# AechPro/rlgym-ppo

Measured on NVIDIA B200. Metric: learner_timesteps_per_sec, higher is better.
Workload: dtype bf16

## Files before the change

include/rlppo.h:

```cpp
#ifndef RLPPO_H_
#define RLPPO_H_

#include <stddef.h>
#include <stdint.h>

#ifdef __cplusplus
extern "C" {
#endif

#define RLPPO_OK 0
#define RLPPO_ERR_ARG (-1)
#define RLPPO_ERR_CUDA (-2)
#define RLPPO_ERR_DEVICE (-3)
#define RLPPO_ERR_WORKSPACE (-4)

int rlppo_version(void);
const char* rlppo_last_error(void);
int rlppo_device_check(void);

size_t rlppo_gae_workspace_bytes(int64_t n);
int rlppo_gae_f32(const float* rew, const float* done, const void* trunc, int trunc_is_f64,
                  const float* values, int64_t n, double gamma, double lambda, const float* ret_std,
                  float* adv, float* vtarget, float* ret, double* ret_head64, int64_t n_head,
                  const double* carry_in, void* ws, size_t ws_bytes, void* stream);
// ... 41 lines not shown
                         uint16_t* wt, int64_t wt_ld, int in_pad, void* stream);

int rlppo_linear_fwd(const uint16_t* x, int64_t ldx, const uint16_t* w, int64_t ldw, const float* bias,
                     uint16_t* y, int64_t ldy, int64_t M, int N, int K, int relu, void* stream);
int rlppo_linear_dgrad(const uint16_t* dy, int64_t lddy, const uint16_t* wt, int64_t ldwt,
                       const uint16_t* hprev, int64_t ldh, uint16_t* dx, int64_t lddx, int64_t M, int N,
                       int K, void* stream);
int rlppo_linear_dgrad_db(const uint16_t* dy, int64_t lddy, const uint16_t* wt, int64_t ldwt,
                          const uint16_t* hprev, int64_t ldh, uint16_t* dx, int64_t lddx, float* db_below,
                          int64_t M, int N, int K, void* stream);
int rlppo_linear_wgrad(const uint16_t* dy, int64_t lddy, const uint16_t* x, int64_t ldx, float* dw,
                       int64_t lddw, float* db, int64_t M, int N, int K, void* stream);

typedef struct rlppo_wgrad_item {
    const uint16_t* dy;
    int64_t lddy;
    const uint16_t* x;
    int64_t ldx;
    float* dw;
    int64_t lddw;
    int64_t M;
    int32_t N, K;
    float* db;
} rlppo_wgrad_item;
int rlppo_wgrad_multi(const rlppo_wgrad_item* h_items, int n_items, void* stream);

int rlppo_policy_head_sample(const uint16_t* h, int64_t ldh, const uint16_t* w, int64_t ldw,
                             const float* bias, int64_t M, int n_actions, int K, const float* u_inject,
                             uint64_t seed, uint64_t offset, int deterministic, float* actions_out,
                             int64_t* actions_i64_out, float* logp_out, float* probs_out, void* stream);

int rlppo_policy_head_train(const uint16_t* h, int64_t ldh, const uint16_t* w, int64_t ldw,
                            const float* bias, int64_t M, int n_actions, int K, const float* actions,
                            const float* old_logp, const float* adv, float inv_batch, float clip,
                            float ent_coef, uint16_t* dz, int64_t lddz, float* logp_out, float* metrics,
                            void* stream);

int rlppo_value_head(const uint16_t* h, int64_t ldh, const float* w, const float* bias, int64_t M, int K,
                     float* values_out, const float* targets, float inv_batch, uint16_t* dh, int64_t lddh,
                     float* dw, float* db, float* metrics, void* stream);

typedef struct rlppo_split {
    int32_t a_parts;
    int32_t b_parts;
    int32_t order;
    int32_t out_parts;
    int64_t a_pstride;
    int64_t b_pstride;
    int64_t out_pstride;
} rlppo_split;
int rlppo_rows_split_bf16(const float* src, int64_t src_ld, int64_t n_rows, int width, const float* mean,
                          const float* std, float clip, uint16_t* dst, int64_t dst_ld, int parts, int64_t pstride,
                          void* stream);
int rlppo_weight_split_bf16(const float* w, int out_f, int in_f, uint16_t* wq, int64_t wq_ld, int q_parts,
                            int64_t q_pstride, int out_rows, uint16_t* wt, int64_t wt_ld, int t_parts,
                            int64_t t_pstride, int in_rows, void* stream);
int rlppo_linear_fwd_split(const uint16_t* x, int64_t ldx, const uint16_t* w, int64_t ldw, const float* bias,
                           int bias_n, uint16_t* y, int64_t ldy, int64_t M, int N, int K, int relu,
                           const rlppo_split* sp, void* stream);
int rlppo_linear_dgrad_split(const uint16_t* dy, int64_t lddy, const uint16_t* wt, int64_t ldwt,
                             const uint16_t* hprev, int64_t ldh, uint16_t* dx, int64_t lddx, float* db_below,
                             int64_t M, int N, int K, const rlppo_split* sp, void* stream);
int rlppo_linear_wgrad_split(const uint16_t* dy, int64_t lddy, const uint16_t* x, int64_t ldx, float* dw,
                             int64_t lddw, float* db, int64_t M, int N, int K, const rlppo_split* sp, void* stream);
int rlppo_policy_head_sample_split(const uint16_t* h, int64_t ldh, const uint16_t* w, int64_t ldw,
                                   const float* bias, int64_t M, int n_actions, int K, const float* u_inject,
                                   uint64_t seed, uint64_t offset, int deterministic, float* actions_out,
                                   int64_t* actions_i64_out, float* logp_out, float* probs_out,
                                   const rlppo_split* sp, void* stream);
int rlppo_policy_head_train_split(const uint16_t* h, int64_t ldh, const uint16_t* w, int64_t ldw,
                                  const float* bias, int64_t M, int n_actions, int K, const float* actions,
                                  const float* old_logp, const float* adv, float inv_batch, float clip,
                                  float ent_coef, uint16_t* dz, int64_t lddz, float* logp_out, float* metrics,
                                  const rlppo_split* sp, void* stream);
int rlppo_value_head_split(const uint16_t* h, int64_t ldh, const float* w, const float* bias, int64_t M, int K,
                           float* values_out, const float* targets, float inv_batch, uint16_t* dh, int64_t lddh,
                           float* dw, float* db, float* metrics, int h_parts, int64_t h_pstride, int dh_parts,
                           int64_t dh_pstride, void* stream);

int rlppo_head_multi_discrete_train(const uint16_t* z, int64_t ldz, int z_parts, int64_t z_pstride, int64_t M,
                                    const float* actions, int64_t ld_act, const float* old_logp, const float* adv,
                                    float inv_batch, float clip, float ent_coef, uint16_t* dz, int64_t lddz,
                                    int dz_parts, int64_t dz_pstride, int dz_cols, float* logp_out, float* metrics,
                                    void* stream);
int rlppo_head_multi_discrete_sample(const uint16_t* z, int64_t ldz, int z_parts, int64_t z_pstride, int64_t M,
                                     const float* u_inject, uint64_t seed, uint64_t offset, int deterministic,
                                     float* actions_out, int64_t ld_aout, float* logp_out, void* stream);
int rlppo_head_continuous_train(const uint16_t* z, int64_t ldz, int z_parts, int64_t z_pstride, int64_t M, int n_act,
                                float var_min, float var_max, const float* actions, int64_t ld_act,
                                const float* old_logp, const float* adv, float inv_batch, float clip, float ent_coef,
                                uint16_t* dz, int64_t lddz, int dz_parts, int64_t dz_pstride, int dz_cols,
                                float* logp_out, float* metrics, void* stream);
int rlppo_head_continuous_sample(const uint16_t* z, int64_t ldz, int z_parts, int64_t z_pstride, int64_t M, int n_act,
                                 float var_min, float var_max, const float* n_inject, uint64_t seed, uint64_t offset,
                                 int deterministic, float* actions_out, int64_t ld_aout, float* logp_out, void* stream);

int rlppo_policy_head_backward(const uint16_t* h, int64_t ldh, const uint16_t* w, int64_t ldw, const float* bias,
                               int64_t M, int n_actions, int K, const float* actions, const float* d_logp,
                               const float* d_ent, const float* d_probs, uint16_t* dz, int64_t lddz, void* stream);
int rlppo_policy_head_backward_split(const uint16_t* h, int64_t ldh, const uint16_t* w, int64_t ldw, const float* bias,
                                     int64_t M, int n_actions, int K, const float* actions, const float* d_logp,
                                     const float* d_ent, const float* d_probs, uint16_t* dz, int64_t lddz,
                                     const rlppo_split* sp, void* stream);
int rlppo_head_multi_discrete_backward(const uint16_t* z, int64_t ldz, int z_parts, int64_t z_pstride, int64_t M,
                                       const float* actions, int64_t ld_act, const float* d_logp, const float* d_ent,
                                       uint16_t* dz, int64_t lddz, int dz_parts, int64_t dz_pstride, int dz_cols,
                                       void* stream);
int rlppo_head_continuous_backward(const uint16_t* z, int64_t ldz, int z_parts, int64_t z_pstride, int64_t M, int n_act,
                                   float var_min, float var_max, const float* actions, int64_t ld_act,
                                   const float* d_logp, const float* d_ent, const float* d_mean, const float* d_std,
                                   uint16_t* dz, int64_t lddz, int dz_parts, int64_t dz_pstride, int dz_cols,
                                   void* stream);
int rlppo_value_head_backward(const uint16_t* h, int64_t ldh, const float* w, int64_t M, int K,
                              const float* d_values, uint16_t* dh, int64_t lddh, float* dw, float* db, void* stream);
int rlppo_value_head_backward_split(const uint16_t* h, int64_t ldh, const float* w, int64_t M, int K,
                                    const float* d_values, uint16_t* dh, int64_t lddh, float* dw, float* db,
                                    int h_parts, int64_t h_pstride, int dh_parts, int64_t dh_pstride, void* stream);

typedef struct rlppo_fused_net {
    int n_hidden;
    int in_dim;
    int64_t in_ld;
    int hidden[4];
    const uint16_t* wq[5];
    int64_t wq_ld[5];
    const uint16_t* wt[5];
    int64_t wt_ld[5];
    const float* bias[5];
    float* gbias[5];
    uint16_t* h[4];
    int64_t h_ld[4];
    uint16_t* dh[4];
    int64_t dh_ld[4];
    uint16_t* dz;
    int64_t dz_ld;
} rlppo_fused_net;

int rlppo_policy_train_fused(const rlppo_fused_net* net, const uint16_t* x, int64_t M, int n_actions,
                             const float* actions, const float* old_logp, const float* adv, float inv_batch,
                             float clip, float ent_coef, float* logp_out, float* metrics, void* stream);
int rlppo_policy_infer_fused(const rlppo_fused_net* net, const uint16_t* x, int64_t M, int n_actions,
                             const float* u_inject, uint64_t seed, uint64_t offset, const uint64_t* d_offset,
                             int deterministic, float* actions_out, int64_t* actions_i64_out, float* logp_out,
                             void* stream);
int rlppo_u64_add(uint64_t* d_counter, uint64_t inc, void* stream);
int rlppo_value_train_fused(const rlppo_fused_net* net, const uint16_t* x, int64_t M, const float* w_head,
                            const float* targets, float inv_batch, float* gw_head, float* values_out,
                            float* metrics, void* stream);
int rlppo_policy_value_train_fused(const rlppo_fused_net* policy_net, const rlppo_fused_net* value_net,
                                   const uint16_t* x, int64_t M, int n_actions, const float* actions,
                                   const float* old_logp, const float* adv, float inv_batch, float clip, float ent_coef,
                                   float* logp_out, const float* w_head, const float* targets, float* gw_head,
                                   float* values_out, float* metrics, void* stream);
int rlppo_value_infer_fused(const rlppo_fused_net* net, const uint16_t* x, int64_t M, const float* w_head,
                            float* values_out, void* stream);

int rlppo_grad_sqnorm(const float* grads, const int64_t* h_seg_off, int n_seg, float* sqnorm, void* stream);
typedef struct rlppo_bf16_view {
    int64_t offset;
    int32_t out_f, in_f;
    uint16_t* wq;
    int64_t wq_ld;
    uint16_t* wt;
    int64_t wt_ld;
} rlppo_bf16_view;
int rlppo_clip_adam(float* params, const float* grads, float* m, float* v, const int64_t* h_seg_off,
                    int n_seg, const float* sqnorm, const float* lr, int64_t* step_count, double max_norm,
                    double beta1, double beta2, double eps, const rlppo_bf16_view* h_views, int n_views,
                    void* stream);
size_t rlppo_norm_clip_adam_workspace_bytes(void);
int rlppo_norm_clip_adam(float* params, const float* grads, float* m, float* v, const int64_t* h_seg_off,
                         int n_seg, float* sqnorm_out, const float* lr, int64_t* step_count, double max_norm,
                         double beta1, double beta2, double eps, const rlppo_bf16_view* h_views, int n_views,
                         void* ws, size_t ws_bytes, void* stream);
size_t rlppo_peer_flag_bytes(void);
int rlppo_norm_clip_adam_peers(float* params, const float* const* h_peer_grads, void* const* h_peer_flags, int rank,
                               int world, float* gsum, float* m, float* v, const int64_t* h_seg_off, int n_seg,
                               float* sqnorm_out, const float* lr, int64_t* step_count, double max_norm, double beta1,
                               double beta2, double eps, const rlppo_bf16_view* h_views, int n_views, void* ws,
                               size_t ws_bytes, void* stream);
int rlppo_norm_clip_adam_peers2(float* params, const float* const* h_peer_grads, void* const* h_peer_flags,
                                const float* const* h_peer_red, int rank, int world, float* m, float* v,
                                const int64_t* h_seg_off, int n_seg, float* sqnorm_out, const float* lr,
                                int64_t* step_count, double max_norm, double beta1, double beta2, double eps,
                                const rlppo_bf16_view* h_views, int n_views, void* ws, size_t ws_bytes, void* stream);
int rlppo_sqdiff(const float* a, const float* b, const int64_t* h_seg_off, int n_seg, float* out,
                 void* stream);

#ifdef __cplusplus
}
#endif
#endif
```

rlgym_ppo_b200/_lib.py:

```python
import ctypes
import os

import torch

_HERE = os.path.dirname(os.path.abspath(__file__))
LIB_PATH = os.environ.get("RLPPO_LIB_PATH") or os.path.join(_HERE, "librlppo_b200.so")

if not os.path.exists(LIB_PATH):
    raise ImportError(
        f"{LIB_PATH} is missing: build it with `python -m rlgym_ppo_b200.build` (nvcc, sm_100a). "
        "rlgym_ppo_b200 has no CPU or PyTorch fallback for its kernels."
    )

_lib = ctypes.CDLL(LIB_PATH)

_P = ctypes.c_void_p
_I = ctypes.c_int
_L = ctypes.c_int64
_D = ctypes.c_double
_F = ctypes.c_float
_U64 = ctypes.c_uint64
_SZ = ctypes.c_size_t

_SIGS = {
    "rlppo_version": ([], _I),
    "rlppo_last_error": ([], ctypes.c_char_p),
    "rlppo_device_check": ([], _I),
    "rlppo_gae_workspace_bytes": ([_L], _SZ),
    "rlppo_gae_f32": ([_P, _P, _P, _I, _P, _L, _D, _D, _P, _P, _P, _P, _P, _L, _P, _P, _SZ, _P], _I),
    "rlppo_gae_chunk_summary": ([_P, _P, _P, _I, _P, _L, _D, _D, _P, _P, _P, _SZ, _P], _I),
    "rlppo_gae_compose_carry": ([_P, _I, _I, _P, _P], _I),
    "rlppo_welford_update": ([_P, _P, _P, _P, _I, _L, _I, _P, _P, _P], _I),
    "rlppo_ring_append": ([_P, _L, _P, _L, _L, _L, _P, _I, _L, _L, _I, _P], _I),
    "rlppo_ring_append_fields": ([_P, _I, _L, _L, _L, _P], _I),
    "rlppo_ring_append_fields_dev": ([_P, _I, _L, _P, _L, _P], _I),
    "rlppo_gather_batch": ([_P, _P, _P, _P, _P, _L, _P, _L, _I, _L, _L, _P, _P, _L, _P, _P, _P, _P, _P, _P, _P], _I),
    "rlppo_host_permutation": ([_P, _P, _L, _P], _I),
    "rlppo_rows_to_bf16": ([_P, _L, _L, _I, _P, _L, _P], _I),
    "rlppo_rows_standardize_to_bf16": ([_P, _L, _L, _I, _P, _P, _F, _P, _L, _P, _L, _P], _I),
    "rlppo_weight_to_bf16": ([_P, _I, _I, _P, _L, _I, _P, _L, _I, _P], _I),
    "rlppo_linear_fwd": ([_P, _L, _P, _L, _P, _P, _L, _L, _I, _I, _I, _P], _I),
    "rlppo_linear_dgrad": ([_P, _L, _P, _L, _P, _L, _P, _L, _L, _I, _I, _P], _I),
    "rlppo_linear_dgrad_db": ([_P, _L, _P, _L, _P, _L, _P, _L, _P, _L, _I, _I, _P], _I),
    "rlppo_linear_wgrad": ([_P, _L, _P, _L, _P, _L, _P, _L, _I, _I, _P], _I),
    "rlppo_wgrad_multi": ([_P, _I, _P], _I),
    "rlppo_policy_head_sample": ([_P, _L, _P, _L, _P, _L, _I, _I, _P, _U64, _U64, _I, _P, _P, _P, _P, _P], _I),
    "rlppo_policy_head_train": ([_P, _L, _P, _L, _P, _L, _I, _I, _P, _P, _P, _F, _F, _F, _P, _L, _P, _P, _P], _I),
    "rlppo_value_head": ([_P, _L, _P, _P, _L, _I, _P, _P, _F, _P, _L, _P, _P, _P, _P], _I),
    "rlppo_rows_split_bf16": ([_P, _L, _L, _I, _P, _P, _F, _P, _L, _I, _L, _P], _I),
    "rlppo_weight_split_bf16": ([_P, _I, _I, _P, _L, _I, _L, _I, _P, _L, _I, _L, _I, _P], _I),
    "rlppo_linear_fwd_split": ([_P, _L, _P, _L, _P, _I, _P, _L, _L, _I, _I, _I, _P, _P], _I),
    "rlppo_linear_dgrad_split": ([_P, _L, _P, _L, _P, _L, _P, _L, _P, _L, _I, _I, _P, _P], _I),
    "rlppo_linear_wgrad_split": ([_P, _L, _P, _L, _P, _L, _P, _L, _I, _I, _P, _P], _I),
    "rlppo_policy_head_sample_split": ([_P, _L, _P, _L, _P, _L, _I, _I, _P, _U64, _U64, _I, _P, _P, _P, _P, _P, _P], _I),
    "rlppo_policy_head_train_split": ([_P, _L, _P, _L, _P, _L, _I, _I, _P, _P, _P, _F, _F, _F, _P, _L, _P, _P, _P, _P], _I),
    "rlppo_value_head_split": ([_P, _L, _P, _P, _L, _I, _P, _P, _F, _P, _L, _P, _P, _P, _I, _L, _I, _L, _P], _I),
    "rlppo_head_multi_discrete_train": ([_P, _L, _I, _L, _L, _P, _L, _P, _P, _F, _F, _F, _P, _L, _I, _L, _I, _P, _P, _P], _I),
    "rlppo_head_multi_discrete_sample": ([_P, _L, _I, _L, _L, _P, _U64, _U64, _I, _P, _L, _P, _P], _I),
    "rlppo_head_continuous_train": ([_P, _L, _I, _L, _L, _I, _F, _F, _P, _L, _P, _P, _F, _F, _F, _P, _L, _I, _L, _I, _P,
                                     _P, _P], _I),
    "rlppo_head_continuous_sample": ([_P, _L, _I, _L, _L, _I, _F, _F, _P, _U64, _U64, _I, _P, _L, _P, _P], _I),
    "rlppo_policy_head_backward": ([_P, _L, _P, _L, _P, _L, _I, _I, _P, _P, _P, _P, _P, _L, _P], _I),
    "rlppo_policy_head_backward_split": ([_P, _L, _P, _L, _P, _L, _I, _I, _P, _P, _P, _P, _P, _L, _P, _P], _I),
    "rlppo_head_multi_discrete_backward": ([_P, _L, _I, _L, _L, _P, _L, _P, _P, _P, _L, _I, _L, _I, _P], _I),
    "rlppo_head_continuous_backward": ([_P, _L, _I, _L, _L, _I, _F, _F, _P, _L, _P, _P, _P, _P, _P, _L, _I, _L, _I, _P],
                                       _I),
    "rlppo_value_head_backward": ([_P, _L, _P, _L, _I, _P, _P, _L, _P, _P, _P], _I),
    "rlppo_value_head_backward_split": ([_P, _L, _P, _L, _I, _P, _P, _L, _P, _P, _I, _L, _I, _L, _P], _I),
    "rlppo_policy_train_fused": ([_P, _P, _L, _I, _P, _P, _P, _F, _F, _F, _P, _P, _P], _I),
    "rlppo_policy_infer_fused": ([_P, _P, _L, _I, _P, _U64, _U64, _P, _I, _P, _P, _P, _P], _I),
    "rlppo_u64_add": ([_P, _U64, _P], _I),
    "rlppo_value_train_fused": ([_P, _P, _L, _P, _P, _F, _P, _P, _P, _P], _I),
    "rlppo_policy_value_train_fused": ([_P, _P, _P, _L, _I, _P, _P, _P, _F, _F, _F, _P, _P, _P, _P, _P, _P, _P], _I),
    "rlppo_value_infer_fused": ([_P, _P, _L, _P, _P, _P], _I),
    "rlppo_grad_sqnorm": ([_P, _P, _I, _P, _P], _I),
    "rlppo_clip_adam": ([_P, _P, _P, _P, _P, _I, _P, _P, _P, _D, _D, _D, _D, _P, _I, _P], _I),
    "rlppo_norm_clip_adam_workspace_bytes": ([], ctypes.c_size_t),
    "rlppo_norm_clip_adam": ([_P, _P, _P, _P, _P, _I, _P, _P, _P, _D, _D, _D, _D, _P, _I, _P, ctypes.c_size_t, _P], _I),
    "rlppo_peer_flag_bytes": ([], ctypes.c_size_t),
    "rlppo_norm_clip_adam_peers": ([_P, _P, _P, _I, _I, _P, _P, _P, _P, _I, _P, _P, _P, _D, _D, _D, _D, _P, _I, _P,
                                    ctypes.c_size_t, _P], _I),
    "rlppo_norm_clip_adam_peers2": ([_P, _P, _P, _P, _I, _I, _P, _P, _P, _I, _P, _P, _P, _D, _D, _D, _D, _P, _I, _P,
                                     ctypes.c_size_t, _P], _I),
    "rlppo_sqdiff": ([_P, _P, _P, _I, _P, _P], _I),
}

EXPORTED = tuple(_SIGS)


class AppendField(ctypes.Structure):
    _fields_ = [("ring", _P), ("ring_ld", _L), ("ring_bf16", _P), ("bf16_ld", _L), ("src", _P), ("src_ld", _L),
                ("src_is_f64", ctypes.c_int32), ("width", ctypes.c_int32)]


class Split(ctypes.Structure):
    _fields_ = [("a_parts", ctypes.c_int32), ("b_parts", ctypes.c_int32), ("order", ctypes.c_int32),
                ("out_parts", ctypes.c_int32), ("a_pstride", _L), ("b_pstride", _L), ("out_pstride", _L)]


class WgradItem(ctypes.Structure):
    _fields_ = [("dy", _P), ("lddy", _L), ("x", _P), ("ldx", _L), ("dw", _P), ("lddw", _L), ("M", _L),
                ("N", ctypes.c_int32), ("K", ctypes.c_int32), ("db", _P)]


class Bf16View(ctypes.Structure):
    _fields_ = [("offset", _L), ("out_f", ctypes.c_int32), ("in_f", ctypes.c_int32), ("wq", _P), ("wq_ld", _L),
                ("wt", _P), ("wt_ld", _L)]


class FusedNet(ctypes.Structure):
    _fields_ = [("n_hidden", _I), ("in_dim", _I), ("in_ld", _L), ("hidden", _I * 4),
                ("wq", _P * 5), ("wq_ld", _L * 5), ("wt", _P * 5), ("wt_ld", _L * 5),
                ("bias", _P * 5), ("gbias", _P * 5), ("h", _P * 4), ("h_ld", _L * 4),
                ("dh", _P * 4), ("dh_ld", _L * 4), ("dz", _P), ("dz_ld", _L)]

for _name, (_args, _res) in _SIGS.items():
    _fn = getattr(_lib, _name)
    _fn.argtypes = _args
    _fn.restype = _res


class RlppoError(RuntimeError):
    pass


def last_error():
    return _lib.rlppo_last_error().decode("utf-8", "replace")


def _check(rc, name):
    if rc != 0:
        raise RlppoError(f"{name} failed ({rc}): {last_error()}")


def ptr(t):
    if t is None:
        return None
    return ctypes.c_void_p(t.data_ptr())


def stream_ptr():
    return ctypes.c_void_p(torch.cuda.current_stream().cuda_stream)


CALLS = 0
_TIMING = None


def call(name, *args, work=None):
    global CALLS
    CALLS += 1
    if _TIMING is None:
        _check(getattr(_lib, name)(*args), name)
        return
    e0, e1 = torch.cuda.Event(enable_timing=True), torch.cuda.Event(enable_timing=True)
    torch.cuda._sleep(300_000)
    e0.record()
    rc = getattr(_lib, name)(*args)
    e1.record()
    _check(rc, name)
    _TIMING.append((name, work, e0, e1))


def timing_begin():
    global _TIMING
    _TIMING = []


def timing_end():
    global _TIMING
    rec, _TIMING = _TIMING, None
    torch.cuda.synchronize()
    out = {}
    for name, work, e0, e1 in rec:
        d = out.setdefault(name, {"calls": 0, "ms": 0.0, "flop": 0.0, "byte": 0.0})
        d["calls"] += 1
        d["ms"] += e0.elapsed_time(e1)
        if work is not None:
            for i in range(0, len(work), 2):
                d[work[i]] = d.get(work[i], 0.0) + float(work[i + 1])
    return out


def require_device():
    if not torch.cuda.is_available():
        raise RlppoError("rlgym_ppo_b200 needs a CUDA device (B200, sm_100); there is no CPU fallback")
    _check(_lib.rlppo_device_check(), "rlppo_device_check")


def version():
    return _lib.rlppo_version()


def gae_workspace_bytes(n):
    return int(_lib.rlppo_gae_workspace_bytes(int(n)))


def host_permutation_raw(key, pos, n, out=None):
    import numpy as np

    key = np.ascontiguousarray(key, dtype=np.uint32).copy()
    p = np.asarray([pos], dtype=np.int32)
    if out is None:
        out = np.empty(int(n), dtype=np.int64)
    rc = _lib.rlppo_host_permutation(key.ctypes.data_as(_P), p.ctypes.data_as(_P), int(n), out.ctypes.data_as(_P))
    _check(rc, "rlppo_host_permutation")
    return out, key, int(p[0])


def host_permutation(rng, n):
    import numpy as np

    st = rng.get_state()
    key = np.ascontiguousarray(st[1], dtype=np.uint32).copy()
    pos = np.asarray([st[2]], dtype=np.int32)
    out = np.empty(int(n), dtype=np.int64)
    rc = _lib.rlppo_host_permutation(key.ctypes.data_as(_P), pos.ctypes.data_as(_P), int(n), out.ctypes.data_as(_P))
    _check(rc, "rlppo_host_permutation")
    rng.set_state((st[0], key, int(pos[0]), st[3], st[4]))
    return out
```

rlgym_ppo_b200/csrc/common.cuh:

```cuda
#pragma once
#include <cuda_runtime.h>
#include <cuda_bf16.h>
#include <stdint.h>
#include <stdio.h>
#include <string.h>

#include "../../include/rlppo.h"

namespace rlppo {

void set_error(const char* fmt, ...);
int check_device();
int num_sms();

#define RLPPO_CHECK_ARG(cond, ...)                 \
    do {                                           \
        if (!(cond)) {                             \
            rlppo::set_error(__VA_ARGS__);         \
            return RLPPO_ERR_ARG;                  \
        }                                          \
    } while (0)

#define RLPPO_CUDA(expr)                                                                      \
    do {                                                                                      \
        cudaError_t _e = (expr);                                                              \
        if (_e != cudaSuccess) {                                                              \
            rlppo::set_error("%s failed: %s (%s:%d)", #expr, cudaGetErrorString(_e), __FILE__, \
                             __LINE__);                                                       \
            return RLPPO_ERR_CUDA;                                                            \
        }                                                                                     \
    } while (0)

#define RLPPO_REQUIRE_DEVICE()                    \
    do {                                          \
        int _d = rlppo::check_device();           \
        if (_d != RLPPO_OK) return _d;            \
    } while (0)

#define RLPPO_LAUNCH_CHECK() RLPPO_CUDA(cudaGetLastError())

__device__ __forceinline__ void pdl_wait() { asm volatile("griddepcontrol.wait;" ::: "memory"); }
__device__ __forceinline__ void pdl_trigger() { asm volatile("griddepcontrol.launch_dependents;" ::: "memory"); }
int pdl_mode();

template <class... KArgs, class... Args>
cudaError_t launch_pdl_cluster(void (*kernel)(KArgs...), dim3 grid, dim3 block, size_t smem, cudaStream_t s, int cluster_x,
                               Args&&... args) {
    cudaLaunchConfig_t cfg = {};
    cfg.gridDim = grid;
    cfg.blockDim = block;
    cfg.dynamicSmemBytes = smem;
    cfg.stream = s;
    cudaLaunchAttribute attr[2];
    int n = 0;
    if (pdl_mode()) {
        attr[n].id = cudaLaunchAttributeProgrammaticStreamSerialization;
        attr[n].val.programmaticStreamSerializationAllowed = 1;
        ++n;
    }
    if (cluster_x > 1) {
        attr[n].id = cudaLaunchAttributeClusterDimension;
        attr[n].val.clusterDim.x = (unsigned)cluster_x;
        attr[n].val.clusterDim.y = 1;
        attr[n].val.clusterDim.z = 1;
        ++n;
    }
    cfg.attrs = attr;
    cfg.numAttrs = n;
    return cudaLaunchKernelEx(&cfg, kernel, static_cast<KArgs>(args)...);
}
template <class... KArgs, class... Args>
cudaError_t launch_pdl(void (*kernel)(KArgs...), dim3 grid, dim3 block, size_t smem, cudaStream_t s, Args&&... args) {
    return launch_pdl_cluster(kernel, grid, block, smem, s, 1, static_cast<Args&&>(args)...);
}

__device__ __forceinline__ int ld_acquire_s32(const int* p) {
    int v;
    asm volatile("ld.acquire.gpu.global.s32 %0, [%1];" : "=r"(v) : "l"(p) : "memory");
    return v;
}
__device__ __forceinline__ void st_release_s32(int* p, int v) {
    asm volatile("st.release.gpu.global.s32 [%0], %1;" ::"l"(p), "r"(v) : "memory");
}

__device__ __forceinline__ float warp_sum(float v) {
#pragma unroll
    for (int o = 16; o > 0; o >>= 1) v += __shfl_xor_sync(0xffffffffu, v, o);
    return v;
}
__device__ __forceinline__ double warp_sum(double v) {
#pragma unroll
    for (int o = 16; o > 0; o >>= 1) v += __shfl_xor_sync(0xffffffffu, v, o);
    return v;
}

__device__ __forceinline__ uint16_t f32_to_bf16_bits(float f) {
    return __bfloat16_as_ushort(__float2bfloat16_rn(f));
}
__device__ __forceinline__ float bf16_bits_to_f32(uint16_t b) { return __uint_as_float(((uint32_t)b) << 16); }
__device__ __forceinline__ uint32_t pack_bf16x2(float lo, float hi) {
    return (uint32_t)f32_to_bf16_bits(lo) | ((uint32_t)f32_to_bf16_bits(hi) << 16);
}

}
```

rlgym_ppo_b200/csrc/mlp_fused.cu:

```cuda
#include <type_traits>
#include <math.h>
#include <stdlib.h>

#include "tc_common.cuh"

namespace {

using namespace rlppo;
using namespace rlppo::tc;

constexpr int MAXL = 4;
constexpr int TILE_M = 128;
constexpr int KBLK = 64;
constexpr uint32_t KB_BYTES = TILE_M * KBLK * 2;
constexpr uint32_t ACT_BYTES = 4 * KB_BYTES;
constexpr uint32_t WST_BYTES = 256 * KBLK * 2;
constexpr uint32_t MN_CHUNK = 64 * KBLK * 2;
constexpr int MAX_NWST = 6;
constexpr int kThreads = 352;
constexpr int kEpiThreads = 256;
constexpr int MAXPH = 2 * MAXL + 1;

constexpr uint32_t OFF_ACT = 0;
constexpr uint32_t OFF_XST = ACT_BYTES;
constexpr uint32_t BIAS_FLOATS = (MAXL + 1) * 256;
constexpr uint32_t MISC_BIAS = 0;
constexpr uint32_t MISC_ROWX = MISC_BIAS + 2 * BIAS_FLOATS * 4;
constexpr uint32_t ROWX_FLOATS = 1280;
constexpr uint32_t MISC_DB = MISC_ROWX + ROWX_FLOATS * 4;
constexpr uint32_t MISC_MASK = MISC_DB + 256 * 4;
constexpr uint32_t MISC_BARS = MISC_MASK + MAXL * 4 * kEpiThreads * 4;
constexpr uint32_t MISC_BYTES = MISC_BARS + 384;
constexpr uint32_t SMEM_LIMIT = 232448;
static_assert(ACT_BYTES + 2 * KB_BYTES + MISC_BYTES + 1024 + 3 * WST_BYTES <= SMEM_LIMIT,
              "an observation of <= 128 columns must leave room for a 3-stage weight ring (2 stages starve the MMA)");

enum { PH_FWD = 0, PH_FWD_VALUE = 1, PH_HEAD = 2, PH_DGRAD = 3, PH_VALUE_BWD = 4 };
constexpr uint8_t NO_STORE = 0xFF;

struct alignas(16) PhaseDesc {
    uint8_t kind;
    uint8_t layer;
    uint8_t n_kb;
    uint8_t wmap;
    uint16_t N;
    uint8_t out;
    uint8_t smem;
    uint8_t wait_kb;
    uint8_t rel_kb;
    uint8_t b_mn;
};

constexpr int MAXNET = 2;

struct alignas(64) Maps {
    CUtensorMap x;
    CUtensorMap w[MAXNET][MAXPH];
    CUtensorMap out[MAXNET][MAXPH];
};

struct NetP {
    int policy;
    int n_ph, L;
    int H[MAXL];
    PhaseDesc ph[MAXPH];
    int tail_rel_kb;
    const float* bias[MAXL + 1];
    float* gbias[MAXL + 1];
    int n_actions, out_kb;
    const float *actions, *old_logp, *adv;
    float inv_batch, clip, ent_coef;
    const float* u_inject;
    uint64_t seed, offset;
    const unsigned long long* d_offset;
    int deterministic;
    float* actions_out;
    int64_t* actions_i64_out;
    float* logp_out;
    const float* w_head;
    const float* targets;
    float* gw_head;
    float* values_out;
    float* metrics;
};

struct Params {
    int64_t M;
    int num_tiles, in_kb, nwst;
    int pair;
    int n_units;
    uint32_t wst_bytes;
    int n_nets;
    NetP net[MAXNET];
    unsigned int* sched;
    uint32_t* mask_scratch;
    int dbg_nostore;
    int dbg;
    unsigned long long* trace;
};

__device__ __forceinline__ void tma_store_2d(const CUtensorMap* m, const void* smem_src, int c0, int c1) {
    asm volatile("cp.async.bulk.tensor.2d.global.shared::cta.bulk_group [%0, {%2, %3}], [%1];" ::"l"(
                     reinterpret_cast<uint64_t>(m)),
                 "r"(smem_u32(smem_src)), "r"(c0), "r"(c1)
                 : "memory");
}
__device__ __forceinline__ void bulk_commit() { asm volatile("cp.async.bulk.commit_group;" ::: "memory"); }
__device__ __forceinline__ void bulk_wait_read_all() { asm volatile("cp.async.bulk.wait_group.read 0;" ::: "memory"); }
__device__ __forceinline__ void epi_bar_sync() { asm volatile("bar.sync 1, 256;" ::: "memory"); }

__device__ __forceinline__ uint4 philox4x32_10(uint4 c, uint2 k) {
#pragma unroll
    for (int i = 0; i < 10; ++i) {
        const uint32_t hi0 = __umulhi(0xD2511F53u, c.x), lo0 = 0xD2511F53u * c.x;
        const uint32_t hi1 = __umulhi(0xCD9E8D57u, c.z), lo1 = 0xCD9E8D57u * c.z;
        c = make_uint4(hi1 ^ c.y ^ k.x, lo1, hi0 ^ c.w ^ k.y, lo0);
        k.x += 0x9E3779B9u;
        k.y += 0xBB67AE85u;
    }
    return c;
}

__device__ __forceinline__ float warp_colsum32(float (&v)[32], int lane) {
#pragma unroll
    for (int w = 16; w >= 1; w >>= 1) {
        const bool up = (lane & w) != 0;
#pragma unroll
        for (int i = 0; i < w; ++i) {
            const float send = up ? v[i] : v[i + w];
            const float keep = up ? v[i + w] : v[i];
            v[i] = keep + __shfl_xor_sync(0xffffffffu, send, w);
        }
    }
    return v[0];
}

__device__ __forceinline__ float warp_colsum16(float (&v)[16], int lane) {
#pragma unroll
    for (int w = 8; w >= 1; w >>= 1) {
        const bool up = (lane & w) != 0;
#pragma unroll
        for (int i = 0; i < w; ++i) {
            const float send = up ? v[i] : v[i + w];
            const float keep = up ? v[i + w] : v[i];
            v[i] = keep + __shfl_xor_sync(0xffffffffu, send, w);
        }
    }
    return v[0] + __shfl_xor_sync(0xffffffffu, v[0], 16);
}

__device__ __forceinline__ float bf16_round(float x) { return bf16_bits_to_f32(f32_to_bf16_bits(x)); }
__device__ __forceinline__ uint32_t cvt_bf16x2(float lo, float hi) {
    uint32_t r;
    asm("cvt.rn.bf16x2.f32 %0, %1, %2;" : "=r"(r) : "f"(hi), "f"(lo));
    return r;
}

__device__ __forceinline__ uint32_t cvt_relu_bf16x2(float lo, float hi) {
    uint32_t r;
    asm("cvt.rn.relu.bf16x2.f32 %0, %1, %2;" : "=r"(r) : "f"(hi), "f"(lo));
    return r;
}

__device__ __forceinline__ void pack32(const float (&v)[32], uint32_t (&w)[16]) {
#pragma unroll
    for (int i = 0; i < 16; ++i) w[i] = cvt_bf16x2(v[2 * i], v[2 * i + 1]);
}
__device__ __forceinline__ void pack32_relu(const float (&v)[32], uint32_t (&w)[16]) {
#pragma unroll
    for (int i = 0; i < 16; ++i) w[i] = cvt_relu_bf16x2(v[2 * i], v[2 * i + 1]);
}
__device__ __forceinline__ uint32_t prmt_b32(uint32_t a, uint32_t b, uint32_t sel) {
    uint32_t r;
    asm("prmt.b32 %0, %1, %2, %3;" : "=r"(r) : "r"(a), "r"(b), "r"(sel));
    return r;
}
__device__ __forceinline__ uint32_t relu_mask32(const uint32_t (&w)[16]) {
    uint32_t m[4] = {0u, 0u, 0u, 0u};
#pragma unroll
    for (int q = 0; q < 8; ++q) {
        uint32_t f0, f1;
        asm("set.gt.u32.bf16x2 %0, %1, %2;" : "=r"(f0) : "r"(w[2 * q]), "r"(0u));
        asm("set.gt.u32.bf16x2 %0, %1, %2;" : "=r"(f1) : "r"(w[2 * q + 1]), "r"(0u));
        m[q & 3] |= prmt_b32(f0, f1, 0x7531u) & (0x80808080u >> q);
    }
    return (m[0] | m[1]) | (m[2] | m[3]);
}
__device__ __forceinline__ void apply_relu_mask32(uint32_t (&w)[16], uint32_t bits) {
#pragma unroll
    for (int q = 0; q < 8; ++q) {
        const uint32_t t = bits << q;
        w[2 * q] &= prmt_b32(t, 0u, 0x9988u);
        w[2 * q + 1] &= prmt_b32(t, 0u, 0xBBAAu);
    }
}
__device__ __forceinline__ constexpr int relu_mask_bit(int i) { return 8 * (i & 3) + 7 - (i >> 2); }
__device__ __forceinline__ void sts_chunk_sw128(uint8_t* buf, int row, int chunk32, const uint32_t (&w)[16]) {
    uint8_t* kb = buf + (chunk32 >> 1) * KB_BYTES + row * 128;
    const int base16 = (chunk32 & 1) * 4;
#pragma unroll
    for (int t = 0; t < 4; ++t)
        *reinterpret_cast<uint4*>(kb + (((base16 + t) ^ (row & 7)) << 4)) = make_uint4(w[4 * t], w[4 * t + 1], w[4 * t + 2], w[4 * t + 3]);
}
__device__ __forceinline__ void sts_chunk16_sw128(uint8_t* buf, int row, int chunk16, const uint32_t (&w)[8]) {
    uint8_t* kb = buf + (chunk16 >> 2) * KB_BYTES + row * 128;
    const int base16 = (chunk16 & 3) * 2;
#pragma unroll
    for (int t = 0; t < 2; ++t)
        *reinterpret_cast<uint4*>(kb + (((base16 + t) ^ (row & 7)) << 4)) = make_uint4(w[4 * t], w[4 * t + 1], w[4 * t + 2], w[4 * t + 3]);
}

#define RLPPO_TRACE(role, idx)                                                                  \
    do {                                                                                        \
        const int _i = (idx);                                                                   \
        if (p.trace != nullptr && blockIdx.x == 0 && _i < 512) p.trace[(role) * 512 + _i] = clock64(); \
    } while (0)

#ifdef RLPPO_FINE_TRACE
#define EPI_T()                                                                                  \
    do {                                                                                         \
        if (p.trace != nullptr && blockIdx.x == 0 && it == 0 && warp == 2 && lane == 0 && tr5 < 500) p.trace[5 * 512 + tr5++] = clock64(); \
    } while (0)
#else
#define EPI_T() do { } while (0)
#endif

struct EpiCtx {
    uint8_t* act;
    float* s_bias;
    float* s_rowx;
    uint32_t* s_mask;
    uint64_t* a_ready;
    uint64_t* a_mma;
    uint32_t rank;
    int lane, quarter, half, row_in_tile;
};

template <bool PAIR>
__device__ __forceinline__ void release_kb(const EpiCtx& e, int kb) {
    tc_fence_before();
    fence_proxy_async();
    __syncwarp();
    if (e.lane == 0) {
        mbar_arrive(e.a_ready + kb);
        if (PAIR) mbar_arrive_cta(e.a_mma + kb, 0);
    }
}

template <bool TRAIN, bool PAIR>
__global__ void __launch_bounds__(kThreads, 1) fused_mlp_kernel(const __grid_constant__ Maps maps, const Params p) {
    extern __shared__ uint8_t smem_raw[];
    uint8_t* smem = smem_raw + ((1024u - (smem_u32(smem_raw) & 1023u)) & 1023u);
    uint8_t* act = smem + OFF_ACT;
    uint8_t* xst = smem + OFF_XST;
    uint8_t* wring = xst + p.in_kb * KB_BYTES;
    uint8_t* misc = wring + p.nwst * p.wst_bytes;
    const uint32_t rank = PAIR ? cluster_ctarank() : 0u;
    const bool leader = rank == 0;
    float* s_bias = reinterpret_cast<float*>(misc + MISC_BIAS);
    float* s_rowx = reinterpret_cast<float*>(misc + MISC_ROWX);
    float* s_db = reinterpret_cast<float*>(misc + MISC_DB);
// ... 455 lines not shown
            mbar_init(&a_done[s], 16);
            mbar_init(&acc_full[s], 1);
            mbar_init(&st_done[s], 1);
        }
        fence_barrier_init();
    }
    if (warp == 1) tmem_alloc_pair(tmem_slot, 512);
    pdl_wait();
    pdl_trigger();
    if (p.trace != nullptr && threadIdx.x == 0) {
        unsigned long long t;
        asm volatile("mov.u64 %0, %%globaltimer;" : "=l"(t));
        p.trace[2048 + 2 * blockIdx.x] = t;
    }
    for (int i = threadIdx.x; i < p.n_nets * (int)BIAS_FLOATS; i += kThreads) {
        const int ni = i >= (int)BIAS_FLOATS ? 1 : 0;
        const NetP& np = p.net[ni];
        const int j = i - ni * (int)BIAS_FLOATS;
        const int l = j >> 8, c = j & 255;
        float b = 0.f;
        if (l < np.L) {
            if (c < np.H[l]) b = __ldg(np.bias[l] + c);
        } else if (l == MAXL) {
            if (np.policy) b = c < np.n_actions ? (np.bias[MAXL] != nullptr ? __ldg(np.bias[MAXL] + c) : 0.f) : -1e30f;
            else if (c < np.H[np.L - 1]) b = __ldg(np.w_head + c);
        }
        s_bias[i] = b;
    }
    for (int i = threadIdx.x; i < 256; i += kThreads) s_db[i] = 0.f;
    for (int i = threadIdx.x; i < p.n_nets * MAXPH; i += kThreads)
        const_cast<PhaseDesc*>(s_ph)[i] = p.net[i / MAXPH].ph[i % MAXPH];
    tc_fence_before();
    __syncthreads();
    cluster_sync_all();
    tc_fence_after();
    const uint32_t tmem_base = *tmem_slot;

    const int cluster_id = (int)(blockIdx.x >> 1), n_clusters = (int)(gridDim.x >> 1);
    const int total_items = p.n_nets * p.n_units;
    const int nph_net0 = p.net[0].n_ph, nph_net1 = p.net[1].n_ph;
    auto next_item = [&](DuoWalk& w, int s) -> bool {
        const int q = cluster_id + (w.fetches++) * n_clusters;
        if (q >= total_items) {
            DUO_SET(w, alive, s, false);
            return false;
        }
        const int ni = q >= p.n_units ? 1 : 0;
        DUO_SET(w, ni, s, ni);
        DUO_SET(w, tile, s, 2 * (q - ni * p.n_units) + (int)rank);
        DUO_SET(w, ph, s, 0);
        DUO_SET(w, nph, s, ni ? nph_net1 : nph_net0);
        DUO_SET(w, items, s, DUO_SEL(w, items, s) + 1);
        return true;
    };
#define DUO_WALK_BEGIN(w, traced)                                             \
    for (int n = 0;; ++n) {                                                   \
        const int s = n & 1;                                                  \
        if ((traced) && warp == 2 && lane == 0) RLPPO_TRACE(3, 4 * n);        \
        if (!DUO_SEL(w, alive, s)) {                                          \
            if (!DUO_SEL(w, alive, s ^ 1)) break;                             \
            continue;                                                         \
        }                                                                     \
        if (DUO_SEL(w, ph, s) == DUO_SEL(w, nph, s) && !next_item(w, s)) {    \
            if (!DUO_SEL(w, alive, s ^ 1)) break;                             \
            continue;                                                         \
        }                                                                     \
        const int ph = DUO_SEL(w, ph, s);                                     \
        DUO_SET(w, ph, s, ph + 1);                                            \
        const int ni = DUO_SEL(w, ni, s);                                     \
        const int tile_s = DUO_SEL(w, tile, s);                               \
        const int items_s = DUO_SEL(w, items, s);                             \
        const bool last_ph = ph + 1 == DUO_SEL(w, nph, s);                    \
        const NetP& np = p.net[ni];                                           \
        const PhaseDesc d = s_ph[ni * MAXPH + ph];                            \
        (void)d; (void)np; (void)tile_s; (void)items_s; (void)last_ph;
#define DUO_WALK_END }

    if (warp == 0) {
        if (lane == 0) {
            DuoWalk w;
            uint32_t ws = 0, wpar = 0;
            DUO_WALK_BEGIN(w, false)
                if (ph == 0) {
                    mbar_wait(&x_free[s], (uint32_t)(items_s & 1));
                    if (leader) mbar_expect_tx(&x_full[s], 2u * p.in_kb * KB_BYTES);
                    for (int kb = 0; kb < p.in_kb; ++kb)
                        tma_load_2d_leaderbar(&maps.x, &x_full[s], smem + s * ACT_BYTES + kb * KB_BYTES, kb * KBLK, tile_s * TILE_M);
                }
                const int nh = d.N >> 1;
                for (int kb = 0; kb < d.n_kb; ++kb) {
                    mbar_wait(&wempty[ws], wpar ^ 1);
                    if (leader) mbar_expect_tx(&wfull[ws], (uint32_t)d.N * 128u);
                    uint8_t* dst = ring + ws * DUO_STAGE;
                    if (d.b_mn) {
                        for (int c = 0; c < (nh >> 6); ++c)
                            tma_load_2d_leaderbar(&maps.w[ni][d.wmap], &wfull[ws], dst + c * MN_CHUNK, (int)rank * nh + c * 64,
                                                  kb * KBLK);
                    } else {
                        tma_load_2d_leaderbar(&maps.w[ni][d.wmap], &wfull[ws], dst, kb * KBLK, (int)rank * nh);
                    }
                    if (++ws == DUO_NST) {
                        ws = 0;
                        wpar ^= 1;
                    }
                }
            DUO_WALK_END
        }
    } else if (warp == 1) {
        if (lane == 0 && leader) {
            DuoWalk w;
            uint32_t ws = 0, wpar = 0;
            uint32_t epi_cnt[2] = {0u, 0u};
            int tr0 = 0;
            DUO_WALK_BEGIN(w, false)
                RLPPO_TRACE(0, tr0++);
                const uint32_t d_tmem = tmem_base + (uint32_t)s * 256u;
                uint8_t* act = smem + s * ACT_BYTES;
                if (epi_cnt[s] > 0u) mbar_wait(&a_done[s], (epi_cnt[s] - 1u) & 1u);
                if (ph == 0) mbar_wait(&x_full[s], (items_s - 1) & 1);
                tc_fence_after();
                if (d.n_kb > 0) {
                    const uint32_t idesc = umma_idesc_bf16(2 * TILE_M, d.N, 0, d.b_mn);
                    for (int kb = 0; kb < d.n_kb; ++kb) {
                        mbar_wait(&wfull[ws], wpar);
                        tc_fence_after();
                        const uint32_t a_addr = smem_u32(act + kb * KB_BYTES);
                        const uint32_t b_addr = smem_u32(ring + ws * DUO_STAGE);
#pragma unroll
                        for (int k = 0; k < KBLK / 16; ++k) {
                            const uint64_t ad = umma_smem_desc(a_addr + k * 32, 16, 1024);
                            const uint64_t bd = d.b_mn ? umma_smem_desc(b_addr + k * (16 * 128), MN_CHUNK, 1024)
                                                       : umma_smem_desc(b_addr + k * 32, 16, 1024);
                            if (!(p.dbg & 1)) umma_bf16_pair(d_tmem, ad, bd, idesc, (kb | k) != 0 ? 1u : 0u);
                        }
                        umma_commit_pair(&wempty[ws]);
                        if (++ws == DUO_NST) {
                            ws = 0;
                            wpar ^= 1;
                        }
                    }
                    umma_commit_pair(&acc_full[s]);
                } else {
                    mbar_arrive(&acc_full[s]);
                    mbar_arrive_cta(&acc_full[s], 1);
                }
                ++epi_cnt[s];
                RLPPO_TRACE(0, tr0++);
            DUO_WALK_END
        }
    } else if (warp == 10) {
        if (lane == 0) {
            DuoWalk w;
            uint32_t kpar = 0;
            DUO_WALK_BEGIN(w, false)
                uint8_t* act = smem + s * ACT_BYTES;
                for (int kb = 0; kb < d.rel_kb; ++kb) {
                    const int b = 4 * s + kb;
                    mbar_wait(&a_kb[b], (kpar >> b) & 1u);
                    kpar ^= 1u << b;
                    if (d.out != NO_STORE) {
                        if (!p.dbg_nostore) tma_store_2d(&maps.out[ni][d.out], act + kb * KB_BYTES, kb * KBLK, tile_s * TILE_M);
                        bulk_commit();
                    }
                }
                if (d.out != NO_STORE && d.rel_kb > 0) bulk_wait_read_all();
                mbar_arrive(&st_done[s]);
                if (last_ph) mbar_arrive(&x_free[s]);
            DUO_WALK_END
            asm volatile("cp.async.bulk.wait_group 0;" ::: "memory");
        }
    } else {
        EpiCtx e;
        e.s_bias = s_bias;
        e.s_rowx = s_rowx;
        e.a_ready = nullptr;
        e.a_mma = nullptr;
        e.rank = rank;
        e.lane = lane;
        e.quarter = warp & 3;
        e.half = (warp - 2) >> 2;
        e.row_in_tile = e.quarter * 32 + lane;
        float dv_slot0 = 0.f, dv_slot1 = 0.f;
        float m0 = 0.f, m1 = 0.f, m2 = 0.f, m3 = 0.f, mrows = 0.f;
        float vm0 = 0.f, vm1 = 0.f, vrows = 0.f;
        auto db_add = [&](int c, float v) { atomicAdd(&s_db[c * 32 + e.lane], v); };
        uint32_t cnt[2] = {0u, 0u};
        uint32_t pend = 0, scnt = 0;
        uint32_t* mask_g = p.mask_scratch + (size_t)blockIdx.x * (2 * DUO_MAXL * 4 * kEpiThreads) + (threadIdx.x - 64);
        int tr1 = 0;
        DuoWalk w;
        DUO_WALK_BEGIN(w, true)
            uint8_t* act = smem + s * ACT_BYTES;
            e.act = act;
            e.s_mask = nullptr;
            const float* s_bias_n = s_bias + ni * (int)BIAS_FLOATS;
            const int64_t row = (int64_t)tile_s * TILE_M + e.row_in_tile;
            const bool row_ok = row < p.M;
            float dv_keep = s ? dv_slot1 : dv_slot0;
            if (warp == 2 && lane == 0) RLPPO_TRACE(2, tr1);
            uint32_t mpre0 = 0u, mpre1 = 0u, mpre2 = 0u, mpre3 = 0u;
            if (d.kind == PH_DGRAD || d.kind == PH_VALUE_BWD) {
                const uint32_t* mp = mask_g + (s * DUO_MAXL + d.layer) * 4 * kEpiThreads;
                mpre0 = __ldcg(mp);
                mpre1 = __ldcg(mp + kEpiThreads);
                mpre2 = __ldcg(mp + 2 * kEpiThreads);
                mpre3 = __ldcg(mp + 3 * kEpiThreads);
            }
            mbar_wait(&acc_full[s], cnt[s] & 1u);
            ++cnt[s];
            tc_fence_after();
            if (warp == 2 && lane == 0) RLPPO_TRACE(1, tr1++);
            if ((pend >> s) & 1u) {
                mbar_wait(&st_done[s], (scnt >> s) & 1u);
                scnt ^= 1u << s;
                pend &= ~(1u << s);
            }
            const uint32_t trow = tmem_base + ((uint32_t)(e.quarter * 32) << 16) + (uint32_t)s * 256u;
            uint8_t* dst = act;
            const int li = d.layer;
            const int it = 1;
            int tr5 = 0;
            (void)it;
            (void)tr5;
#define RLPPO_RELEASE_KB(j)                                                  \
    do {                                                                      \
        if (((j) & 1) || (j) + 1 >= (int)d.rel_kb) {                          \
            fence_proxy_async();                                              \
            __syncwarp();                                                     \
            if (lane == 0) {                                                  \
                if ((j) & 1) mbar_arrive(&a_kb[4 * s + (j) - 1]);             \
                mbar_arrive(&a_kb[4 * s + (j)]);                              \
            }                                                                 \
        }                                                                     \
    } while (0)
#define RLPPO_MASK_ST(l, kb, v) __stcg(mask_g + ((s * DUO_MAXL + (l)) * 4 + (kb)) * kEpiThreads, (v))
#define RLPPO_MASK_LD(l, kb) ((kb) == 0 ? mpre0 : (kb) == 1 ? mpre1 : (kb) == 2 ? mpre2 : mpre3)
#include "fused_epilogue.inc"
#undef RLPPO_MASK_ST
#undef RLPPO_MASK_LD
#undef RLPPO_RELEASE_KB
            if (s) dv_slot1 = dv_keep;
            else dv_slot0 = dv_keep;
            pend |= 1u << s;
            if (warp == 2 && lane == 0) RLPPO_TRACE(3, 4 * n + 1);
            tc_fence_before();
            __syncwarp();
            if (warp == 2 && lane == 0) RLPPO_TRACE(3, 4 * n + 2);
            if (lane == 0) {
                if (leader) mbar_arrive(&a_done[s]);
                else mbar_arrive_cta(&a_done[s], 0);
            }
            if (warp == 2 && lane == 0) RLPPO_TRACE(1, tr1++);
        DUO_WALK_END
        if (e.half == 0) {
            for (int ni = 0; ni < p.n_nets; ++ni) {
                const NetP& np = p.net[ni];
                if (np.metrics == nullptr) continue;
                if (np.policy) {
                    const float r0 = warp_sum(m0), r1 = warp_sum(m1), r2 = warp_sum(m2), r3 = warp_sum(m3),
                                rr = warp_sum(mrows);
                    if (e.lane == 0 && rr > 0.f) {
                        atomicAdd(np.metrics + 0, r0);
                        atomicAdd(np.metrics + 1, r1);
                        atomicAdd(np.metrics + 2, r2);
                        atomicAdd(np.metrics + 3, r3);
                        atomicAdd(np.metrics + 4, rr);
                    }
                } else {
                    const float r0 = warp_sum(vm0), r1 = warp_sum(vm1), rr = warp_sum(vrows);
                    if (e.lane == 0 && rr > 0.f) {
                        atomicAdd(np.metrics + 5, r0);
                        atomicAdd(np.metrics + 6, rr);
                        if (np.gbias[MAXL] != nullptr) atomicAdd(np.gbias[MAXL], r1);
                    }
                }
            }
        }
    }
#undef DUO_WALK_BEGIN
#undef DUO_WALK_END
#undef DUO_SEL
#undef DUO_SET
    tc_fence_before();
    __syncthreads();
    if (p.trace != nullptr && threadIdx.x == 0) {
        unsigned long long t;
        asm volatile("mov.u64 %0, %%globaltimer;" : "=l"(t));
        p.trace[2048 + 2 * blockIdx.x + 1] = t;
    }
    cluster_sync_all();
    if (warp == 1) {
        tc_fence_after();
        tmem_dealloc_pair(tmem_base, 512);
    }
    for (int ni = 0; ni < p.n_nets; ++ni) {
        const NetP& np = p.net[ni];
        if (np.policy || np.gw_head == nullptr) continue;
        for (int c = threadIdx.x; c < np.H[np.L - 1]; c += kThreads) atomicAdd(np.gw_head + c, s_db[c]);
    }
}

int check_net(const rlppo_fused_net* net) {
    RLPPO_CHECK_ARG(net != nullptr, "null net descriptor");
    RLPPO_CHECK_ARG(net->n_hidden >= 1 && net->n_hidden <= MAXL, "fused path: 1..%d hidden layers", MAXL);
    RLPPO_CHECK_ARG(net->in_dim >= 1 && net->in_dim <= 256 && net->in_ld % 8 == 0 && net->in_ld >= net->in_dim,
                    "fused path: input width <= 256, row stride a multiple of 8");
    for (int l = 0; l < net->n_hidden; ++l)
        RLPPO_CHECK_ARG(net->hidden[l] >= 64 && net->hidden[l] <= 256 && net->hidden[l] % 64 == 0,
                        "fused path: hidden widths must be 64, 128, 192 or 256 (got %d)", net->hidden[l]);
    return RLPPO_OK;
}

template <bool TRAIN>
int build_net(bool POLICY, const rlppo_fused_net* net, int64_t M, int ni, Maps& maps, NetP& p, bool pair) {
    int rc = check_net(net);
    if (rc) return rc;
    const int L = net->n_hidden;
    p.policy = POLICY ? 1 : 0;
    p.L = L;
    for (int l = 0; l < MAXL; ++l) p.H[l] = l < L ? net->hidden[l] : 0;
    for (int l = 0; l < L; ++l) {
        p.bias[l] = net->bias[l];
// ... 197 lines not shown
    }
    return true;
}

int launch_duo(const rlppo_fused_net* const* nets, const bool* is_policy, int n_nets, const uint16_t* x, int64_t M, Params& p,
               cudaStream_t s) {
    Maps maps;
    p.M = M;
    p.num_tiles = (int)((M + TILE_M - 1) / TILE_M);
    p.pair = 1;
    p.n_units = (p.num_tiles + 1) / 2;
    p.n_nets = n_nets;
    p.in_kb = (nets[0]->in_dim + KBLK - 1) / KBLK;
    p.nwst = DUO_NST;
    p.wst_bytes = DUO_STAGE;
    for (int ni = 0; ni < n_nets; ++ni) {
        RLPPO_CHECK_ARG(nets[ni]->in_dim == nets[0]->in_dim && nets[ni]->in_ld == nets[0]->in_ld,
                        "nets of one launch read the same x");
        int rc = build_net<true>(is_policy[ni], nets[ni], M, ni, maps, p.net[ni], true);
        if (rc) return rc;
    }
    int rc = make_tmap_bf16_2d(&maps.x, x, (uint64_t)M, (uint64_t)nets[0]->in_dim, (uint64_t)nets[0]->in_ld, TILE_M);
    if (rc) return rc;
    static bool configured = false;
    if (!configured) {
        RLPPO_CUDA(cudaFuncSetAttribute(fused_duo_kernel, cudaFuncAttributeMaxDynamicSharedMemorySize, (int)SMEM_LIMIT));
        configured = true;
    }
    const int items = p.n_units * n_nets;
    const int pairs = num_sms() / 2;
    const int want = (items + 1) / 2;
    const int grid = 2 * (want < pairs ? want : pairs);
    for (int ni = 0; ni < n_nets; ++ni)
        for (int i = 0; i < p.net[ni].n_ph; ++i)
            RLPPO_CHECK_ARG(p.net[ni].ph[i].rel_kb > 0, "duo kernel: every phase must release at least one k-block");
    p.sched = nullptr;
    {
        static uint32_t* d_mask[16] = {};
        static unsigned int next_area[16] = {};
        int dev = 0;
        RLPPO_CUDA(cudaGetDevice(&dev));
        const size_t area = (size_t)num_sms() * 2 * DUO_MAXL * 4 * kEpiThreads;
        if (d_mask[dev] == nullptr) RLPPO_CUDA(cudaMalloc(&d_mask[dev], 4 * area * sizeof(uint32_t)));
        p.mask_scratch = d_mask[dev] + (next_area[dev]++ % 4) * area;
    }
    p.dbg_nostore = getenv("RLPPO_FUSED_NOSTORE") != nullptr ? 1 : 0;
    p.dbg = getenv("RLPPO_DUO_DBG") != nullptr ? atoi(getenv("RLPPO_DUO_DBG")) : 0;
    static unsigned long long* d_trace = nullptr;
    const bool tracing = getenv("RLPPO_FUSED_TRACE") != nullptr;
    if (tracing) {
        if (d_trace == nullptr) RLPPO_CUDA(cudaMalloc(&d_trace, 3072 * sizeof(unsigned long long)));
        RLPPO_CUDA(cudaMemsetAsync(d_trace, 0, 3072 * sizeof(unsigned long long), s));
        p.trace = d_trace;
    }
    RLPPO_CUDA(launch_pdl_cluster(fused_duo_kernel, dim3(grid), dim3(kThreads), (size_t)DUO_SMEM, s, 2, maps, p));
    if (tracing) {
        static unsigned long long h[3072];
        RLPPO_CUDA(cudaMemcpyAsync(h, d_trace, sizeof(h), cudaMemcpyDeviceToHost, s));
        RLPPO_CUDA(cudaStreamSynchronize(s));
        const unsigned long long t0 = h[0];
        fprintf(stderr, "[duo trace] items=%d (steps alternate slots 0/1)\n", items);
        for (int i = 0; i + 1 < 100 && h[i + 1] != 0; i += 2)
            fprintf(stderr, "  mma  step %d start=%llu issued=+%llu\n", i / 2, h[i] - t0, h[i + 1] - h[i]);
        {
            unsigned long long g0 = ~0ull, g1 = 0;
            for (int b = 0; b < grid; ++b) {
                if (h[2048 + 2 * b] < g0) g0 = h[2048 + 2 * b];
                if (h[2048 + 2 * b + 1] > g1) g1 = h[2048 + 2 * b + 1];
            }
            fprintf(stderr, "  CTA spans (ns from the first start; start..end), kernel body %llu ns:\n", g1 - g0);
            for (int b = 0; b < grid; b += 2)
                fprintf(stderr, "   cluster %d: %llu..%llu%s", b / 2, h[2048 + 2 * b] - g0, h[2048 + 2 * b + 1] - g0, (b / 2) % 4 == 3 ? "\n" : "");
            fprintf(stderr, "\n");
        }
        for (int i = 0; i + 1 < 100 && h[512 + i] != 0; i += 2)
            fprintf(stderr, "  epi  step %d top=%llu arrive=%llu acc_full=%llu dur=%llu body_end=+%llu fences=+%llu arrives=+%llu\n", i / 2,
                    h[1536 + 2 * i] - t0, h[1024 + i] - t0, h[512 + i] - t0, h[512 + i + 1] - h[512 + i],
                    h[1536 + 2 * i + 1] - h[512 + i], h[1536 + 2 * i + 2] - h[1536 + 2 * i + 1], h[512 + i + 1] - h[1536 + 2 * i + 2]);
    }
    return RLPPO_OK;
}

template <bool TRAIN>
int launch_nets(const rlppo_fused_net* const* nets, const bool* is_policy, int n_nets, const uint16_t* x, int64_t M, Params& p,
                cudaStream_t s) {
    RLPPO_CHECK_ARG(n_nets >= 1 && n_nets <= MAXNET && nets[0] != nullptr, "1..%d nets per launch", MAXNET);
    RLPPO_CHECK_ARG(M >= 1 && M < (1ll << 30) - TILE_M, "bad row count");
    for (int ni = 0; ni < n_nets; ++ni) {
        int rc = check_net(nets[ni]);
        if (rc) return rc;
    }
    if (TRAIN && duo_ok(nets, n_nets)) return launch_duo(nets, is_policy, n_nets, x, M, p, s);
    if (TRAIN && pair_ok(nets, n_nets)) return launch_nets_t<TRAIN, TRAIN>(nets, is_policy, n_nets, x, M, p, s);
    return launch_nets_t<TRAIN, false>(nets, is_policy, n_nets, x, M, p, s);
}

void fill_policy_train(NetP& n, int n_actions, const float* actions, const float* old_logp, const float* adv,
                       float inv_batch, float clip, float ent_coef, float* logp_out, float* metrics) {
    n.n_actions = n_actions;
    n.actions = actions; n.old_logp = old_logp; n.adv = adv;
    n.inv_batch = inv_batch; n.clip = clip; n.ent_coef = ent_coef;
    n.logp_out = logp_out; n.metrics = metrics;
}
void fill_value_train(NetP& n, const float* w_head, const float* targets, float inv_batch, float* gw_head,
                      float* values_out, float* metrics) {
    n.w_head = w_head; n.targets = targets; n.inv_batch = inv_batch; n.gw_head = gw_head;
    n.values_out = values_out; n.metrics = metrics;
}

__global__ void u64_add_kernel(unsigned long long* ctr, unsigned long long inc) { *ctr += inc; }

}

extern "C" {

int rlppo_policy_train_fused(const rlppo_fused_net* net, const uint16_t* x, int64_t M, int n_actions,
                             const float* actions, const float* old_logp, const float* adv, float inv_batch, float clip,
                             float ent_coef, float* logp_out, float* metrics, void* stream) {
    RLPPO_REQUIRE_DEVICE();
    RLPPO_CHECK_ARG(x && actions && old_logp && adv, "null pointer");
    RLPPO_CHECK_ARG(n_actions >= 1 && n_actions <= 128, "fused path: n_actions must be in [1,128]");
    Params p{};
    fill_policy_train(p.net[0], n_actions, actions, old_logp, adv, inv_batch, clip, ent_coef, logp_out, metrics);
    const bool pol[1] = {true};
    return launch_nets<true>(&net, pol, 1, x, M, p, static_cast<cudaStream_t>(stream));
}

int rlppo_value_train_fused(const rlppo_fused_net* net, const uint16_t* x, int64_t M, const float* w_head,
                            const float* targets, float inv_batch, float* gw_head, float* values_out, float* metrics,
                            void* stream) {
    RLPPO_REQUIRE_DEVICE();
    RLPPO_CHECK_ARG(x && w_head && targets && gw_head, "null pointer");
    Params p{};
    fill_value_train(p.net[0], w_head, targets, inv_batch, gw_head, values_out, metrics);
    const bool pol[1] = {false};
    return launch_nets<true>(&net, pol, 1, x, M, p, static_cast<cudaStream_t>(stream));
}

int rlppo_policy_value_train_fused(const rlppo_fused_net* policy_net, const rlppo_fused_net* value_net, const uint16_t* x,
                                   int64_t M, int n_actions, const float* actions, const float* old_logp, const float* adv,
                                   float inv_batch, float clip, float ent_coef, float* logp_out, const float* w_head,
                                   const float* targets, float* gw_head, float* values_out, float* metrics, void* stream) {
    RLPPO_REQUIRE_DEVICE();
    RLPPO_CHECK_ARG(policy_net && value_net && x && actions && old_logp && adv && w_head && targets && gw_head, "null pointer");
    RLPPO_CHECK_ARG(n_actions >= 1 && n_actions <= 128, "fused path: n_actions must be in [1,128]");
    Params p{};
    fill_policy_train(p.net[0], n_actions, actions, old_logp, adv, inv_batch, clip, ent_coef, logp_out, metrics);
    fill_value_train(p.net[1], w_head, targets, inv_batch, gw_head, values_out, metrics);
    const rlppo_fused_net* nets[2] = {policy_net, value_net};
    const bool pol[2] = {true, false};
    return launch_nets<true>(nets, pol, 2, x, M, p, static_cast<cudaStream_t>(stream));
}

int rlppo_u64_add(uint64_t* d_counter, uint64_t inc, void* stream) {
    RLPPO_REQUIRE_DEVICE();
    RLPPO_CHECK_ARG(d_counter != nullptr, "null pointer");
    u64_add_kernel<<<1, 1, 0, static_cast<cudaStream_t>(stream)>>>(reinterpret_cast<unsigned long long*>(d_counter), inc);
    RLPPO_LAUNCH_CHECK();
    return RLPPO_OK;
}

int rlppo_policy_infer_fused(const rlppo_fused_net* net, const uint16_t* x, int64_t M, int n_actions,
                             const float* u_inject, uint64_t seed, uint64_t offset, const uint64_t* d_offset,
                             int deterministic, float* actions_out, int64_t* actions_i64_out, float* logp_out,
                             void* stream) {
    RLPPO_REQUIRE_DEVICE();
    RLPPO_CHECK_ARG(x != nullptr, "null pointer");
    RLPPO_CHECK_ARG(n_actions >= 1 && n_actions <= 128, "fused path: n_actions must be in [1,128]");
    Params p{};
    NetP& n = p.net[0];
    n.n_actions = n_actions;
    n.u_inject = u_inject; n.seed = seed; n.offset = offset; n.deterministic = deterministic;
    n.d_offset = reinterpret_cast<const unsigned long long*>(d_offset);
    n.actions_out = actions_out; n.actions_i64_out = actions_i64_out; n.logp_out = logp_out;
    const bool pol[1] = {true};
    return launch_nets<false>(&net, pol, 1, x, M, p, static_cast<cudaStream_t>(stream));
}

int rlppo_value_infer_fused(const rlppo_fused_net* net, const uint16_t* x, int64_t M, const float* w_head,
                            float* values_out, void* stream) {
    RLPPO_REQUIRE_DEVICE();
    RLPPO_CHECK_ARG(x && w_head && values_out, "null pointer");
    Params p{};
    p.net[0].w_head = w_head; p.net[0].values_out = values_out;
    const bool pol[1] = {false};
    return launch_nets<false>(&net, pol, 1, x, M, p, static_cast<cudaStream_t>(stream));
}
}
```

rlgym_ppo_b200/csrc/mlp_tcgen05.cu:

```cuda
#include <mutex>
#include <unordered_map>
#include <math.h>

#include <stdlib.h>

#include "tc_common.cuh"

namespace rlppo {
namespace tc {

typedef CUresult (*EncodeTiledFn)(CUtensorMap*, CUtensorMapDataType, cuuint32_t, void*, const cuuint64_t*,
                                  const cuuint64_t*, const cuuint32_t*, const cuuint32_t*, CUtensorMapInterleave,
                                  CUtensorMapSwizzle, CUtensorMapL2promotion, CUtensorMapFloatOOBfill);

static EncodeTiledFn get_encode_fn() {
    static EncodeTiledFn fn = nullptr;
    if (fn == nullptr) {
        void* p = nullptr;
        cudaDriverEntryPointQueryResult q;
        if (cudaGetDriverEntryPoint("cuTensorMapEncodeTiled", &p, cudaEnableDefault, &q) == cudaSuccess &&
            q == cudaDriverEntryPointSuccess)
            fn = reinterpret_cast<EncodeTiledFn>(p);
    }
    return fn;
}

int make_tmap_bf16_2d(CUtensorMap* out, const void* base, uint64_t rows, uint64_t cols, uint64_t ld,
                      uint32_t box_rows) {
    EncodeTiledFn fn = get_encode_fn();
    if (fn == nullptr) {
        set_error("cuTensorMapEncodeTiled not available from the driver");
        return RLPPO_ERR_CUDA;
    }
    RLPPO_CHECK_ARG((reinterpret_cast<uintptr_t>(base) & 15) == 0, "TMA operand must be 16-byte aligned");
    RLPPO_CHECK_ARG((ld * 2) % 16 == 0 && cols <= ld && cols >= 1 && rows >= 1, "TMA operand: ld must be a multiple of 8");
    RLPPO_CHECK_ARG(box_rows >= 1 && box_rows <= 256, "TMA box rows out of range");
    struct Key {
        const void* base;
        uint64_t rows, cols, ld;
        uint32_t box_rows;
        bool operator==(const Key& o) const {
            return base == o.base && rows == o.rows && cols == o.cols && ld == o.ld && box_rows == o.box_rows;
        }
    };
    struct KeyHash {
        size_t operator()(const Key& k) const {
            uint64_t h = reinterpret_cast<uintptr_t>(k.base) * 0x9E3779B97F4A7C15ull;
            h ^= (k.rows + 0x9E3779B97F4A7C15ull + (h << 6) + (h >> 2));
            h ^= (k.cols * 0xC2B2AE3D27D4EB4Full + (h << 6) + (h >> 2));
            h ^= (k.ld * 0x165667B19E3779F9ull + (h << 6) + (h >> 2));
            return (size_t)(h ^ k.box_rows);
        }
    };
    static std::mutex mu;
    static std::unordered_map<Key, CUtensorMap, KeyHash> cache;
    const Key key{base, rows, cols, ld, box_rows};
    {
        std::lock_guard<std::mutex> lock(mu);
        auto it = cache.find(key);
        if (it != cache.end()) {
            *out = it->second;
            return RLPPO_OK;
        }
    }
    cuuint64_t gdim[2] = {cols, rows};
    cuuint64_t gstride[1] = {ld * 2};
    cuuint32_t box[2] = {64, box_rows};
    cuuint32_t estr[2] = {1, 1};
    CUresult r = fn(out, CU_TENSOR_MAP_DATA_TYPE_BFLOAT16, 2, const_cast<void*>(base), gdim, gstride, box, estr,
                    CU_TENSOR_MAP_INTERLEAVE_NONE, CU_TENSOR_MAP_SWIZZLE_128B, CU_TENSOR_MAP_L2_PROMOTION_L2_256B,
                    CU_TENSOR_MAP_FLOAT_OOB_FILL_NONE);
    if (r != CUDA_SUCCESS) {
        set_error("cuTensorMapEncodeTiled failed with CUresult %d (rows=%llu cols=%llu ld=%llu box_rows=%u)", (int)r,
                  (unsigned long long)rows, (unsigned long long)cols, (unsigned long long)ld, box_rows);
        return RLPPO_ERR_CUDA;
    }
    {
        std::lock_guard<std::mutex> lock(mu);
        if (cache.size() >= 4096) cache.clear();
        cache.emplace(key, *out);
    }
    return RLPPO_OK;
}

}
}

namespace {

using namespace rlppo;
using namespace rlppo::tc;

constexpr int BLOCK_M = 128;
constexpr int BLOCK_K = 64;
constexpr int UMMA_K = 16;
constexpr int kStages = 4;
constexpr int kThreads = 192;
constexpr uint32_t A_BYTES = BLOCK_M * BLOCK_K * 2;

enum { EPI_BIAS_ACT = 0, EPI_RELU_MASK = 1, EPI_HEAD_SAMPLE = 2, EPI_HEAD_TRAIN = 3, EPI_HEAD_BWD = 4 };

constexpr int MAX_SCHED = 6;
struct KSched {
    int n;
    int kpp;
    int a_off[MAX_SCHED];
    int b_off[MAX_SCHED];
};

struct RowGemmParams {
    int64_t M;
    int N, K;
    int num_m_tiles, num_n_tiles, num_k_blocks;
    KSched sched;
    int out_parts;
    int64_t out_pstride;
    int out_cols;
    uint16_t* out;
    int64_t ldo;
    const float* bias;
    int bias_n;
    int relu;
    const uint16_t* mask;
    int64_t ldmask;
    float* colsum;
    int n_actions;
    const float* actions;
    const float* old_logp;
    const float* adv;
    float inv_batch, clip, ent_coef;
    float* logp_out;
    float* metrics;
    const float* u_inject;
    uint64_t seed, offset;
    int deterministic;
    float* actions_out;
    int64_t* actions_i64_out;
    float* probs_out;
    const float* d_logp;
    const float* d_ent;
    const float* d_probs;
};

__device__ __forceinline__ uint4 philox4x32_10(uint4 c, uint2 k) {
#pragma unroll
    for (int i = 0; i < 10; ++i) {
        const uint32_t hi0 = __umulhi(0xD2511F53u, c.x), lo0 = 0xD2511F53u * c.x;
        const uint32_t hi1 = __umulhi(0xCD9E8D57u, c.z), lo1 = 0xCD9E8D57u * c.z;
        c = make_uint4(hi1 ^ c.y ^ k.x, lo1, hi0 ^ c.w ^ k.y, lo0);
        k.x += 0x9E3779B9u;
        k.y += 0xBB67AE85u;
    }
// ... 509 lines not shown
            } else if (EPI == EPI_HEAD_SAMPLE) {
                epilogue_head_sample(p, trow, row, s_bias);
            } else {
                epilogue_head_train<EPI == EPI_HEAD_BWD>(p, trow, row, s_bias, lane);
            }
            tc_fence_before();
            __syncwarp();
            if (lane == 0) mbar_arrive(&tempty[acc]);
        }
    }
    tc_fence_before();
    __syncthreads();
    if (warp == 1) {
        tc_fence_after();
        tmem_dealloc(tmem_base, TMEM_COLS);
    }
}

struct WgradParams {
    int64_t M;
    int N, K;
    float* dw;
    int64_t lddw;
    int64_t m_per_split;
    int splits, n_tiles_n, n_tiles_k;
    int n_sched;
    int x_off[MAX_SCHED], dy_off[MAX_SCHED];
};

template <int BN>
__global__ void __launch_bounds__(kThreads, 1)
wgrad_kernel(const __grid_constant__ CUtensorMap tmX, const __grid_constant__ CUtensorMap tmDY, WgradParams p) {
    constexpr uint32_t CHUNK = 64 * BLOCK_K * 2;
    constexpr uint32_t XA_BYTES = 2 * CHUNK;
    constexpr uint32_t DY_BYTES = (BN / 64) * CHUNK;
    constexpr uint32_t STAGE = XA_BYTES + DY_BYTES;
    constexpr uint32_t TMEM_COLS = BN < 32 ? 32 : BN;
    static_assert(BN % 64 == 0 && BN <= 256, "wgrad n tile");

    extern __shared__ uint8_t smem_raw[];
    uint8_t* smem = smem_raw + ((1024u - (smem_u32(smem_raw) & 1023u)) & 1023u);
    uint64_t* full = reinterpret_cast<uint64_t*>(smem + kStages * STAGE);
    uint64_t* empty = full + kStages;
    uint64_t* tfull = empty + kStages;
    uint32_t* tmem_slot = reinterpret_cast<uint32_t*>(tfull + 1);

    const int warp = threadIdx.x >> 5, lane = threadIdx.x & 31;
    if (threadIdx.x == 0) {
        tma_prefetch_desc(&tmX);
        tma_prefetch_desc(&tmDY);
        for (int i = 0; i < kStages; ++i) {
            mbar_init(&full[i], 1);
            mbar_init(&empty[i], 1);
        }
        mbar_init(tfull, 1);
        fence_barrier_init();
    }
    if (warp == 1) tmem_alloc(tmem_slot, TMEM_COLS);
    tc_fence_before();
    __syncthreads();
    tc_fence_after();
    const uint32_t tmem_base = *tmem_slot;

    const int split = blockIdx.x % p.splits;
    const int tile = blockIdx.x / p.splits;
    const int k_tile = tile % p.n_tiles_k, n_tile = tile / p.n_tiles_k;
    const int64_t m0 = (int64_t)split * p.m_per_split;
    const int64_t m1 = min(p.M, m0 + p.m_per_split);
    const int nkb = m1 > m0 ? (int)((m1 - m0 + BLOCK_K - 1) / BLOCK_K) : 0;

    const int nsch = p.n_sched > 0 ? p.n_sched : 1;
    if (warp == 0) {
        if (lane == 0) {
            uint32_t stage = 0, phase = 0;
            for (int kb = 0; kb < nkb; ++kb) {
              const int mrow = (int)(m0 + (int64_t)kb * BLOCK_K);
              for (int se = 0; se < nsch; ++se) {
                mbar_wait(&empty[stage], phase ^ 1);
                mbar_expect_tx(&full[stage], STAGE);
                uint8_t* sx = smem + stage * STAGE;
                const int xo = p.n_sched > 0 ? p.x_off[se] : 0, yo = p.n_sched > 0 ? p.dy_off[se] : 0;
#pragma unroll
                for (int c = 0; c < 2; ++c)
                    tma_load_2d(&tmX, &full[stage], sx + c * CHUNK, xo + k_tile * 128 + c * 64, mrow);
#pragma unroll
                for (int c = 0; c < BN / 64; ++c)
                    tma_load_2d(&tmDY, &full[stage], sx + XA_BYTES + c * CHUNK, yo + n_tile * BN + c * 64, mrow);
                if (++stage == kStages) {
                    stage = 0;
                    phase ^= 1;
                }
              }
            }
        }
    } else if (warp == 1) {
        if (lane == 0 && nkb > 0) {
            constexpr uint32_t idesc = umma_idesc_bf16(128, BN, 1, 1);
            uint32_t stage = 0, phase = 0;
            for (int kb = 0; kb < nkb * nsch; ++kb) {
                mbar_wait(&full[stage], phase);
                tc_fence_after();
                const uint32_t a_addr = smem_u32(smem + stage * STAGE);
                const uint32_t b_addr = a_addr + XA_BYTES;
#pragma unroll
                for (int ks = 0; ks < BLOCK_K / UMMA_K; ++ks) {
                    const uint64_t ad = umma_smem_desc(a_addr + ks * (UMMA_K * 128), CHUNK, 1024);
                    const uint64_t bd = umma_smem_desc(b_addr + ks * (UMMA_K * 128), CHUNK, 1024);
                    umma_bf16(tmem_base, ad, bd, idesc, (kb | ks) != 0 ? 1u : 0u);
                }
                umma_commit(&empty[stage]);
                if (++stage == kStages) {
                    stage = 0;
                    phase ^= 1;
                }
            }
            umma_commit(tfull);
        }
    } else if (nkb > 0) {
        const int ew = warp & 3;
        mbar_wait(tfull, 0);
        tc_fence_after();
        const uint32_t trow = tmem_base + ((uint32_t)(ew * 32) << 16);
        const int k = k_tile * 128 + ew * 32 + lane;
        const int n0 = n_tile * BN;
        const int nch = (min(BN, p.N - n0) + 31) >> 5;
        for (int c = 0; c < nch; ++c) {
            float v[32];
            tmem_ld32(trow + c * 32, v);
            if (k < p.K) {
#pragma unroll
                for (int j = 0; j < 32; ++j) {
                    const int n = n0 + c * 32 + j;
                    if (n < p.N) atomicAdd(p.dw + (int64_t)n * p.lddw + k, v[j]);
                }
            }
        }
    }
    tc_fence_before();
    __syncthreads();
    if (warp == 1) {
        tc_fence_after();
        tmem_dealloc(tmem_base, TMEM_COLS);
    }
}

constexpr int MAXW = 8;
struct alignas(64) WMaps {
    CUtensorMap x[MAXW];
    CUtensorMap dy[MAXW];
};
struct WLayer {
    float* dw;
    float* db;
    int64_t lddw, M, m_per_split;
    int N, K, n_tiles_n, n_kpairs, splits, first_item;
};
struct WMultiParams {
    WLayer L[MAXW];
    int n_layers, total_items;
    int dbg_nodrain;
    int dbg_nomma;
};

__global__ void __launch_bounds__(kThreads, 1)
wgrad_multi_kernel(const __grid_constant__ WMaps maps, const WMultiParams p) {
    constexpr uint32_t CHUNK = 64 * BLOCK_K * 2;
    constexpr uint32_t STAGE = 8 * CHUNK;
    constexpr int NST = 3;

    extern __shared__ uint8_t smem_raw[];
    uint8_t* smem = smem_raw + ((1024u - (smem_u32(smem_raw) & 1023u)) & 1023u);
    uint64_t* full = reinterpret_cast<uint64_t*>(smem + NST * STAGE);
    uint64_t* empty = full + NST;
    uint64_t* tfull = empty + NST;
    uint64_t* tempty = tfull + 1;
    uint32_t* tmem_slot = reinterpret_cast<uint32_t*>(tempty + 1);

    const int warp = threadIdx.x >> 5, lane = threadIdx.x & 31;
    if (threadIdx.x == 0) {
        for (int i = 0; i < NST; ++i) {
            mbar_init(&full[i], 1);
            mbar_init(&empty[i], 1 + 4);
        }
        mbar_init(tfull, 1);
        mbar_init(tempty, 4);
        fence_barrier_init();
    }
    if (warp == 1) tmem_alloc(tmem_slot, 512);
    tc_fence_before();
    __syncthreads();
    tc_fence_after();
    const uint32_t tmem_base = *tmem_slot;
    pdl_wait();
    pdl_trigger();

    struct Item {
        int layer, n0, k0, nkb, n_x, n_y, bn;
        int64_t m0;
    };
    auto decode = [&](int w) {
        Item it;
        int l = 0;
        while (l + 1 < p.n_layers && w >= p.L[l + 1].first_item) ++l;
        const WLayer& L = p.L[l];
        const int local = w - L.first_item;
        const int split = local % L.splits, tile = local / L.splits;
        const int kp = tile % L.n_kpairs, nt = tile / L.n_kpairs;
        it.layer = l;
        it.n0 = nt * 256;
        it.k0 = kp * 256;
        it.m0 = (int64_t)split * L.m_per_split;
        const int64_t m1 = min(L.M, it.m0 + L.m_per_split);
        it.nkb = m1 > it.m0 ? (int)((m1 - it.m0 + BLOCK_K - 1) / BLOCK_K) : 0;
        it.n_x = (min(256, L.K - it.k0) + 63) / 64;
        it.n_y = (min(256, L.N - it.n0) + 63) / 64;
        it.bn = (min(256, L.N - it.n0) + 15) / 16 * 16;
        return it;
    };

    if (warp == 0) {
        if (lane == 0) {
            uint32_t stage = 0, phase = 0;
            for (int w = blockIdx.x; w < p.total_items; w += gridDim.x) {
                const Item it = decode(w);
                for (int kb = 0; kb < it.nkb; ++kb) {
                    mbar_wait(&empty[stage], phase ^ 1);
                    mbar_expect_tx(&full[stage], (uint32_t)(it.n_x + it.n_y) * CHUNK);
                    uint8_t* sx = smem + stage * STAGE;
                    const int mrow = (int)(it.m0 + (int64_t)kb * BLOCK_K);
                    for (int c = 0; c < it.n_x; ++c)
                        tma_load_2d_hint(&maps.x[it.layer], &full[stage], sx + c * CHUNK, it.k0 + c * 64, mrow, L2_EVICT_FIRST);
                    for (int c = 0; c < it.n_y; ++c)
                        tma_load_2d_hint(&maps.dy[it.layer], &full[stage], sx + (4 + c) * CHUNK, it.n0 + c * 64, mrow, L2_EVICT_FIRST);
                    if (++stage == NST) {
                        stage = 0;
                        phase ^= 1;
                    }
                }
            }
        }
    } else if (warp == 1) {
        if (lane == 0) {
            uint32_t stage = 0, phase = 0, n_done = 0;
            for (int w = blockIdx.x; w < p.total_items; w += gridDim.x) {
                const Item it = decode(w);
                if (it.nkb == 0) continue;
                mbar_wait(tempty, (n_done & 1) ^ 1);
                tc_fence_after();
                const uint32_t idesc = umma_idesc_bf16(128, it.bn, 1, 1);
                const int n_kt = (it.n_x + 1) / 2;
                for (int kb = 0; kb < it.nkb; ++kb) {
                    mbar_wait(&full[stage], phase);
                    tc_fence_after();
                    const uint32_t x_addr = smem_u32(smem + stage * STAGE);
                    const uint32_t b_addr = x_addr + 4 * CHUNK;
                    for (int kt = 0; kt < (p.dbg_nomma ? 0 : n_kt); ++kt) {
#pragma unroll
                        for (int ks = 0; ks < BLOCK_K / UMMA_K; ++ks) {
                            const uint64_t ad = umma_smem_desc(x_addr + kt * 2 * CHUNK + ks * (UMMA_K * 128), CHUNK, 1024);
                            const uint64_t bd = umma_smem_desc(b_addr + ks * (UMMA_K * 128), CHUNK, 1024);
                            umma_bf16(tmem_base + kt * 256, ad, bd, idesc, (kb | ks) != 0 ? 1u : 0u);
                        }
                    }
                    umma_commit(&empty[stage]);
                    if (++stage == NST) {
                        stage = 0;
                        phase ^= 1;
                    }
                }
                umma_commit(tfull);
                ++n_done;
            }
        }
    } else {
        const int ew = warp & 3;
        uint32_t n_done = 0, stage = 0, phase = 0;
        for (int w = blockIdx.x; w < p.total_items; w += gridDim.x) {
            const Item it = decode(w);
            if (it.nkb == 0) continue;
            const WLayer& L = p.L[it.layer];
            const bool want_db = L.db != nullptr && it.k0 == 0 && ew < it.n_y;
            float s0 = 0.f, s1 = 0.f, s2 = 0.f, s3 = 0.f;
            for (int kb = 0; kb < it.nkb; ++kb) {
                mbar_wait(&full[stage], phase);
                if (want_db) {
                    const uint8_t* tile = smem + stage * STAGE + (4 + ew) * CHUNK;
                    const uint32_t sub = (uint32_t)(lane & 3) * 4u, c16 = (uint32_t)lane >> 2;
#pragma unroll 8
                    for (int r = 0; r < BLOCK_K; r += 2) {
                        const uint32_t w0 = *reinterpret_cast<const uint32_t*>(tile + r * 128 + ((c16 ^ (uint32_t)(r & 7)) << 4) + sub);
                        const uint32_t w1 = *reinterpret_cast<const uint32_t*>(tile + (r + 1) * 128 + ((c16 ^ (uint32_t)((r + 1) & 7)) << 4) + sub);
                        s0 += __uint_as_float(w0 << 16);
                        s1 += __uint_as_float(w0 & 0xFFFF0000u);
                        s2 += __uint_as_float(w1 << 16);
                        s3 += __uint_as_float(w1 & 0xFFFF0000u);
                    }
                }
                __syncwarp();
                if (lane == 0) mbar_arrive(&empty[stage]);
                if (++stage == NST) {
                    stage = 0;
                    phase ^= 1;
                }
            }
            if (want_db && !p.dbg_nodrain) {
                const int n = it.n0 + ew * 64 + 2 * lane;
                if (n < L.N) atomicAdd(L.db + n, s0 + s2);
                if (n + 1 < L.N) atomicAdd(L.db + n + 1, s1 + s3);
            }
            mbar_wait(tfull, n_done & 1);
            tc_fence_after();
            const int n_kt = (it.n_x + 1) / 2;
            const int nch = (min(256, L.N - it.n0) + 31) >> 5;
            for (int kt = 0; kt < n_kt; ++kt) {
                const uint32_t trow = tmem_base + ((uint32_t)(ew * 32) << 16) + kt * 256;
                const int k = it.k0 + kt * 128 + ew * 32 + lane;
                for (int c = 0; c < nch; ++c) {
                    float v[32];
                    tmem_ld32(trow + c * 32, v);
                    if (k < L.K) {
#pragma unroll
                        for (int j = 0; j < 32; ++j) {
                            const int n = it.n0 + c * 32 + j;
                            if (n < L.N && !p.dbg_nodrain) atomicAdd(L.dw + (int64_t)n * L.lddw + k, v[j]);
                        }
                    }
                }
            }
            tc_fence_before();
            __syncwarp();
            if (lane == 0) mbar_arrive(tempty);
            ++n_done;
        }
    }
    tc_fence_before();
    __syncthreads();
    if (warp == 1) {
        tc_fence_after();
        tmem_dealloc(tmem_base, 512);
    }
}

__global__ void colsum_kernel(const uint16_t* __restrict__ dy, int64_t ld, int64_t M, int N, int n8,
                              float* __restrict__ db, int64_t rows_per_block) {
    extern __shared__ float s_acc[];
    for (int i = threadIdx.x; i < n8; i += blockDim.x) s_acc[i] = 0.f;
    __syncthreads();
    const int groups = n8 >> 3;
    const int g = threadIdx.x % groups;
    const int rlane = threadIdx.x / groups;
    const int rstride = blockDim.x / groups;
    const int64_t r0 = (int64_t)blockIdx.x * rows_per_block;
    const int64_t r1 = min(M, r0 + rows_per_block);
    float acc[8] = {0, 0, 0, 0, 0, 0, 0, 0};
    if (rlane < rstride) {
#pragma unroll 4
        for (int64_t r = r0 + rlane; r < r1; r += rstride) {
            const uint4 q = __ldg(reinterpret_cast<const uint4*>(dy + r * ld + g * 8));
            const uint32_t w[4] = {q.x, q.y, q.z, q.w};
#pragma unroll
            for (int j = 0; j < 4; ++j) {
                acc[2 * j] += __uint_as_float(w[j] << 16);
                acc[2 * j + 1] += __uint_as_float(w[j] & 0xFFFF0000u);
            }
        }
#pragma unroll
        for (int j = 0; j < 8; ++j) atomicAdd(&s_acc[g * 8 + j], acc[j]);
    }
    __syncthreads();
    for (int i = threadIdx.x; i < N; i += blockDim.x) atomicAdd(db + i, s_acc[i]);
}

template <int BLOCK_N, int EPI>
int launch_rowgemm_t(const CUtensorMap& tmA, const CUtensorMap& tmB, RowGemmParams& p, cudaStream_t s) {
    using L = SmemLayout<BLOCK_N>;
    static bool configured = false;
    auto kfn = rowgemm_kernel<BLOCK_N, EPI>;
    if (!configured) {
        RLPPO_CUDA(cudaFuncSetAttribute(kfn, cudaFuncAttributeMaxDynamicSharedMemorySize, (int)L::TOTAL));
        configured = true;
    }
    p.num_m_tiles = (int)((p.M + BLOCK_M - 1) / BLOCK_M);
    p.num_n_tiles = (p.N + BLOCK_N - 1) / BLOCK_N;
    p.num_k_blocks = (p.K + BLOCK_K - 1) / BLOCK_K * (p.sched.n > 0 ? p.sched.n : 1);
    const int tiles = p.num_m_tiles * p.num_n_tiles;
    const int grid = tiles < num_sms() ? tiles : num_sms();
    kfn<<<grid, kThreads, L::TOTAL, s>>>(tmA, tmB, p);
    RLPPO_LAUNCH_CHECK();
    return RLPPO_OK;
}

int fill_sched(const rlppo_split* sp, int K, int* n, int* a_off, int* b_off) {
    *n = 0;
    if (sp == nullptr) return RLPPO_OK;
    RLPPO_CHECK_ARG(sp->a_parts >= 1 && sp->a_parts <= 3 && sp->b_parts >= 1 && sp->b_parts <= 3 && sp->order >= 1 &&
                        sp->order <= 3 && sp->out_parts >= 1 && sp->out_parts <= 3,
                    "split: parts and order must be in [1,3]");
    const int Kp = (K + 63) / 64 * 64;
    RLPPO_CHECK_ARG((sp->a_parts == 1 || (sp->a_pstride % 64 == 0 && sp->a_pstride >= Kp)) &&
                        (sp->b_parts == 1 || (sp->b_pstride % 64 == 0 && sp->b_pstride >= Kp)),
                    "split: part strides must be multiples of 64 columns and cover the contraction width");
    for (int sum = sp->order - 1; sum >= 0; --sum)
        for (int i = 0; i < sp->a_parts; ++i) {
            const int j = sum - i;
            if (j < 0 || j >= sp->b_parts) continue;
            RLPPO_CHECK_ARG(*n < MAX_SCHED, "split: too many products");
            a_off[*n] = (int)(i * sp->a_pstride);
            b_off[*n] = (int)(j * sp->b_pstride);
            ++*n;
        }
    return RLPPO_OK;
}

template <int EPI>
int launch_rowgemm(const uint16_t* a, int64_t lda, const uint16_t* b, int64_t ldb, int64_t b_rows,
                   RowGemmParams& p, int min_block_n, const rlppo_split* sp, cudaStream_t s) {
    RLPPO_CHECK_ARG(p.M >= 1 && p.N >= 1 && p.K >= 1, "empty GEMM");
    RLPPO_CHECK_ARG(p.M < (1ll << 31), "M too large for TMA coordinates");
    int bn = p.N <= 64 ? 64 : (p.N <= 128 ? 128 : 256);
    if (bn < min_block_n) bn = min_block_n;
    int rc = fill_sched(sp, p.K, &p.sched.n, p.sched.a_off, p.sched.b_off);
    if (rc) return rc;
    p.sched.kpp = (p.K + BLOCK_K - 1) / BLOCK_K;
    p.out_parts = sp ? sp->out_parts : 1;
    p.out_pstride = sp ? sp->out_pstride : 0;
    RLPPO_CHECK_ARG(p.out_parts == 1 || p.out_pstride % 8 == 0, "split: output part stride must be a multiple of 8");
    const uint64_t a_cols = sp && sp->a_parts > 1 ? (uint64_t)lda : (uint64_t)p.K;
    const uint64_t b_cols = sp && sp->b_parts > 1 ? (uint64_t)ldb : (uint64_t)p.K;
    CUtensorMap tmA, tmB;
    rc = make_tmap_bf16_2d(&tmA, a, (uint64_t)p.M, a_cols, (uint64_t)lda, BLOCK_M);
    if (rc) return rc;
    rc = make_tmap_bf16_2d(&tmB, b, (uint64_t)b_rows, b_cols, (uint64_t)ldb, (uint32_t)bn);
    if (rc) return rc;
    if (EPI == EPI_HEAD_SAMPLE || EPI == EPI_HEAD_TRAIN || EPI == EPI_HEAD_BWD) {
        if (bn <= 128) return launch_rowgemm_t<128, EPI>(tmA, tmB, p, s);
        return launch_rowgemm_t<256, EPI>(tmA, tmB, p, s);
    }
    if (bn == 64) return launch_rowgemm_t<64, EPI>(tmA, tmB, p, s);
    if (bn == 128) return launch_rowgemm_t<128, EPI>(tmA, tmB, p, s);
    return launch_rowgemm_t<256, EPI>(tmA, tmB, p, s);
}

template <int BN>
int launch_wgrad_t(const CUtensorMap& tmX, const CUtensorMap& tmDY, const WgradParams& p, cudaStream_t s) {
    constexpr uint32_t SMEM = kStages * (2 * 8192 + (BN / 64) * 8192) + 256 + 1024;
    static bool configured = false;
    auto kfn = wgrad_kernel<BN>;
    if (!configured) {
        RLPPO_CUDA(cudaFuncSetAttribute(kfn, cudaFuncAttributeMaxDynamicSharedMemorySize, (int)SMEM));
        configured = true;
    }
    const int grid = p.n_tiles_n * p.n_tiles_k * p.splits;
    kfn<<<grid, kThreads, SMEM, s>>>(tmX, tmDY, p);
    RLPPO_LAUNCH_CHECK();
    return RLPPO_OK;
}

}

extern "C" {

int rlppo_linear_fwd_split(const uint16_t* x, int64_t ldx, const uint16_t* w, int64_t ldw, const float* bias,
                           int bias_n, uint16_t* y, int64_t ldy, int64_t M, int N, int K, int relu,
                           const rlppo_split* sp, void* stream) {
    RLPPO_REQUIRE_DEVICE();
    RLPPO_CHECK_ARG(x && w && y, "null pointer");
    RLPPO_CHECK_ARG(N % 8 == 0 && ldy >= N && ldy % 8 == 0, "N and ldy must be multiples of 8");
    RLPPO_CHECK_ARG(bias_n >= 0 && bias_n <= N, "bias_n must be in [0, N]");
    RowGemmParams p{};
    p.M = M; p.N = N; p.K = K;
    p.out = y; p.ldo = ldy; p.bias = bias; p.bias_n = bias_n > 0 ? bias_n : N; p.relu = relu;
    return launch_rowgemm<EPI_BIAS_ACT>(x, ldx, w, ldw, N, p, 0, sp, static_cast<cudaStream_t>(stream));
}

int rlppo_linear_fwd(const uint16_t* x, int64_t ldx, const uint16_t* w, int64_t ldw, const float* bias, uint16_t* y,
                     int64_t ldy, int64_t M, int N, int K, int relu, void* stream) {
    return rlppo_linear_fwd_split(x, ldx, w, ldw, bias, 0, y, ldy, M, N, K, relu, nullptr, stream);
}

int rlppo_linear_dgrad_split(const uint16_t* dy, int64_t lddy, const uint16_t* wt, int64_t ldwt, const uint16_t* hprev,
                             int64_t ldh, uint16_t* dx, int64_t lddx, float* db_below, int64_t M, int N, int K,
                             const rlppo_split* sp, void* stream) {
    RLPPO_REQUIRE_DEVICE();
    RLPPO_CHECK_ARG(dy && wt && dx, "null pointer");
    RLPPO_CHECK_ARG(K % 8 == 0 && lddx >= K && lddx % 8 == 0, "K and lddx must be multiples of 8");
    RLPPO_CHECK_ARG(!hprev || ldh % 8 == 0, "ldh must be a multiple of 8");
    RowGemmParams p{};
// ... 3 lines not shown
}

int rlppo_linear_dgrad(const uint16_t* dy, int64_t lddy, const uint16_t* wt, int64_t ldwt, const uint16_t* hprev,
                       int64_t ldh, uint16_t* dx, int64_t lddx, int64_t M, int N, int K, void* stream) {
    return rlppo_linear_dgrad_split(dy, lddy, wt, ldwt, hprev, ldh, dx, lddx, nullptr, M, N, K, nullptr, stream);
}

int rlppo_linear_dgrad_db(const uint16_t* dy, int64_t lddy, const uint16_t* wt, int64_t ldwt, const uint16_t* hprev,
                          int64_t ldh, uint16_t* dx, int64_t lddx, float* db_below, int64_t M, int N, int K,
                          void* stream) {
    return rlppo_linear_dgrad_split(dy, lddy, wt, ldwt, hprev, ldh, dx, lddx, db_below, M, N, K, nullptr, stream);
}

int rlppo_policy_head_sample_split(const uint16_t* h, int64_t ldh, const uint16_t* w, int64_t ldw, const float* bias,
                                   int64_t M, int n_actions, int K, const float* u_inject, uint64_t seed,
                                   uint64_t offset, int deterministic, float* actions_out, int64_t* actions_i64_out,
                                   float* logp_out, float* probs_out, const rlppo_split* sp, void* stream) {
    RLPPO_REQUIRE_DEVICE();
    RLPPO_CHECK_ARG(h && w, "null pointer");
    RLPPO_CHECK_ARG(n_actions >= 1 && n_actions <= 256, "n_actions must be in [1,256]");
    RowGemmParams p{};
    p.M = M; p.N = (n_actions + 7) / 8 * 8; p.K = K;
    p.bias = bias; p.n_actions = n_actions;
    p.u_inject = u_inject; p.seed = seed; p.offset = offset; p.deterministic = deterministic;
    p.actions_out = actions_out; p.actions_i64_out = actions_i64_out; p.logp_out = logp_out; p.probs_out = probs_out;
    return launch_rowgemm<EPI_HEAD_SAMPLE>(h, ldh, w, ldw, n_actions, p, 128, sp, static_cast<cudaStream_t>(stream));
}

int rlppo_policy_head_sample(const uint16_t* h, int64_t ldh, const uint16_t* w, int64_t ldw, const float* bias,
                             int64_t M, int n_actions, int K, const float* u_inject, uint64_t seed, uint64_t offset,
                             int deterministic, float* actions_out, int64_t* actions_i64_out, float* logp_out,
                             float* probs_out, void* stream) {
    return rlppo_policy_head_sample_split(h, ldh, w, ldw, bias, M, n_actions, K, u_inject, seed, offset, deterministic,
                                          actions_out, actions_i64_out, logp_out, probs_out, nullptr, stream);
}

int rlppo_policy_head_train_split(const uint16_t* h, int64_t ldh, const uint16_t* w, int64_t ldw, const float* bias,
                                  int64_t M, int n_actions, int K, const float* actions, const float* old_logp,
                                  const float* adv, float inv_batch, float clip, float ent_coef, uint16_t* dz,
                                  int64_t lddz, float* logp_out, float* metrics, const rlppo_split* sp, void* stream) {
    RLPPO_REQUIRE_DEVICE();
    RLPPO_CHECK_ARG(h && w && actions && old_logp && adv && dz, "null pointer");
    RLPPO_CHECK_ARG(n_actions >= 1 && n_actions <= 256, "n_actions must be in [1,256]");
    const int64_t cols = sp && sp->out_parts > 1 ? sp->out_pstride : lddz;
    RLPPO_CHECK_ARG(cols >= n_actions && cols % 8 == 0 && cols <= 256 && lddz >= cols && lddz % 8 == 0,
                    "d(logits) row width must be a multiple of 8 in [n_actions,256]");
    RowGemmParams p{};
    p.M = M; p.N = (n_actions + 7) / 8 * 8; p.K = K;
    p.bias = bias; p.n_actions = n_actions;
    p.actions = actions; p.old_logp = old_logp; p.adv = adv;
    p.inv_batch = inv_batch; p.clip = clip; p.ent_coef = ent_coef;
    p.out = dz; p.ldo = lddz; p.out_cols = (int)cols; p.logp_out = logp_out; p.metrics = metrics;
    const int min_bn = cols > 128 ? 256 : 128;
    return launch_rowgemm<EPI_HEAD_TRAIN>(h, ldh, w, ldw, n_actions, p, min_bn, sp, static_cast<cudaStream_t>(stream));
}

int rlppo_policy_head_train(const uint16_t* h, int64_t ldh, const uint16_t* w, int64_t ldw, const float* bias,
                            int64_t M, int n_actions, int K, const float* actions, const float* old_logp,
                            const float* adv, float inv_batch, float clip, float ent_coef, uint16_t* dz, int64_t lddz,
                            float* logp_out, float* metrics, void* stream) {
    return rlppo_policy_head_train_split(h, ldh, w, ldw, bias, M, n_actions, K, actions, old_logp, adv, inv_batch, clip,
                                         ent_coef, dz, lddz, logp_out, metrics, nullptr, stream);
}

int rlppo_policy_head_backward_split(const uint16_t* h, int64_t ldh, const uint16_t* w, int64_t ldw, const float* bias,
                                     int64_t M, int n_actions, int K, const float* actions, const float* d_logp,
                                     const float* d_ent, const float* d_probs, uint16_t* dz, int64_t lddz,
                                     const rlppo_split* sp, void* stream) {
    RLPPO_REQUIRE_DEVICE();
    RLPPO_CHECK_ARG(h && w && dz && (d_logp == nullptr || actions != nullptr), "null pointer");
    RLPPO_CHECK_ARG(n_actions >= 1 && n_actions <= 256, "n_actions must be in [1,256]");
    const int64_t cols = sp && sp->out_parts > 1 ? sp->out_pstride : lddz;
    RLPPO_CHECK_ARG(cols >= n_actions && cols % 8 == 0 && cols <= 256 && lddz >= cols && lddz % 8 == 0,
                    "d(logits) row width must be a multiple of 8 in [n_actions,256]");
    RowGemmParams p{};
    p.M = M; p.N = (n_actions + 7) / 8 * 8; p.K = K;
    p.bias = bias; p.n_actions = n_actions; p.actions = actions;
    p.d_logp = d_logp; p.d_ent = d_ent; p.d_probs = d_probs;
    p.out = dz; p.ldo = lddz; p.out_cols = (int)cols;
    const int min_bn = cols > 128 ? 256 : 128;
    return launch_rowgemm<EPI_HEAD_BWD>(h, ldh, w, ldw, n_actions, p, min_bn, sp, static_cast<cudaStream_t>(stream));
}

int rlppo_policy_head_backward(const uint16_t* h, int64_t ldh, const uint16_t* w, int64_t ldw, const float* bias,
                               int64_t M, int n_actions, int K, const float* actions, const float* d_logp,
                               const float* d_ent, const float* d_probs, uint16_t* dz, int64_t lddz, void* stream) {
    return rlppo_policy_head_backward_split(h, ldh, w, ldw, bias, M, n_actions, K, actions, d_logp, d_ent, d_probs, dz,
                                            lddz, nullptr, stream);
}

int rlppo_linear_wgrad_split(const uint16_t* dy, int64_t lddy, const uint16_t* x, int64_t ldx, float* dw, int64_t lddw,
                             float* db, int64_t M, int N, int K, const rlppo_split* sp, void* stream) {
    RLPPO_REQUIRE_DEVICE();
    RLPPO_CHECK_ARG(dy && x && dw && M >= 1 && N >= 1 && K >= 1, "bad argument");
    RLPPO_CHECK_ARG(M < (1ll << 31), "M too large for TMA coordinates");
    RLPPO_CHECK_ARG(lddy % 8 == 0 && ldx % 8 == 0, "lddy and ldx must be multiples of 8");
    cudaStream_t s = static_cast<cudaStream_t>(stream);
    const int bn = N <= 64 ? 64 : (N <= 128 ? 128 : 256);
    WgradParams p{};
    p.M = M; p.N = N; p.K = K; p.dw = dw; p.lddw = lddw;
    p.n_tiles_n = (N + bn - 1) / bn;
    p.n_tiles_k = (K + 127) / 128;
    if (sp != nullptr) {
        rlppo_split t = *sp;
        const int Np = (N + 63) / 64 * 64, Kp = (K + 63) / 64 * 64;
        RLPPO_CHECK_ARG((t.a_parts == 1 || t.a_pstride >= Np) && (t.b_parts == 1 || t.b_pstride >= Kp),
                        "split: part strides must cover the operand widths");
        int rc0 = fill_sched(&t, 1, &p.n_sched, p.dy_off, p.x_off);
        if (rc0) return rc0;
    }
    const int tiles = p.n_tiles_n * p.n_tiles_k;
    const int64_t kblocks = (M + BLOCK_K - 1) / BLOCK_K;
    int64_t splits = num_sms() / tiles;
    if (splits < 1) splits = 1;
    if (splits > kblocks) splits = kblocks;
    p.m_per_split = ((kblocks + splits - 1) / splits) * BLOCK_K;
    p.splits = (int)((M + p.m_per_split - 1) / p.m_per_split);
    const bool xs = sp && sp->b_parts > 1, ys = sp && sp->a_parts > 1;
    const uint64_t x_cols = xs ? (uint64_t)ldx : (uint64_t)min((int64_t)((K + 7) / 8 * 8), ldx);
    const uint64_t dy_cols = ys ? (uint64_t)lddy : (uint64_t)min((int64_t)((N + 7) / 8 * 8), lddy);
    CUtensorMap tmX, tmDY;
    int rc = make_tmap_bf16_2d(&tmX, x, (uint64_t)M, x_cols, (uint64_t)ldx, 64);
    if (rc) return rc;
    rc = make_tmap_bf16_2d(&tmDY, dy, (uint64_t)M, dy_cols, (uint64_t)lddy, 64);
    if (rc) return rc;
    if (bn == 64) rc = launch_wgrad_t<64>(tmX, tmDY, p, s);
    else if (bn == 128) rc = launch_wgrad_t<128>(tmX, tmDY, p, s);
    else rc = launch_wgrad_t<256>(tmX, tmDY, p, s);
    if (rc) return rc;
    if (db != nullptr) {
        const int n8 = (N + 7) / 8 * 8;
        RLPPO_CHECK_ARG(n8 <= lddy && n8 / 8 <= 256, "bias-gradient pass needs N padded to 8 within lddy");
        int64_t rows_per_block = (M + (int64_t)num_sms() * 8 - 1) / ((int64_t)num_sms() * 8);
        rows_per_block = (rows_per_block + 7) / 8 * 8;
        if (rows_per_block < 32) rows_per_block = 32;
        const unsigned blocks = (unsigned)((M + rows_per_block - 1) / rows_per_block);
        int threads = 256;
        if (threads < n8 / 8) threads = n8 / 8;
        const int dy_parts = sp ? sp->a_parts : 1;
        for (int q = 0; q < dy_parts; ++q) {
            colsum_kernel<<<blocks, threads, n8 * sizeof(float), s>>>(dy + (sp ? q * sp->a_pstride : 0), lddy, M, N, n8, db,
                                                                      rows_per_block);
            RLPPO_LAUNCH_CHECK();
        }
    }
    return RLPPO_OK;
}

int rlppo_linear_wgrad(const uint16_t* dy, int64_t lddy, const uint16_t* x, int64_t ldx, float* dw, int64_t lddw,
                       float* db, int64_t M, int N, int K, void* stream) {
    return rlppo_linear_wgrad_split(dy, lddy, x, ldx, dw, lddw, db, M, N, K, nullptr, stream);
}

int rlppo_wgrad_multi(const rlppo_wgrad_item* h_items, int n_items, void* stream) {
    RLPPO_REQUIRE_DEVICE();
    RLPPO_CHECK_ARG(h_items && n_items >= 1 && n_items <= MAXW, "1..%d weight-gradient items per launch", MAXW);
    WMaps maps;
    WMultiParams p{};
    p.n_layers = n_items;
    double bytes[MAXW], total_bytes = 0.0;
    for (int i = 0; i < n_items; ++i) {
        const rlppo_wgrad_item& it = h_items[i];
        RLPPO_CHECK_ARG(it.dy && it.x && it.dw && it.M >= 1 && it.N >= 1 && it.K >= 1, "bad item %d", i);
        RLPPO_CHECK_ARG(it.M < (1ll << 31) && it.lddy % 8 == 0 && it.ldx % 8 == 0, "item %d: ld must be a multiple of 8", i);
        WLayer& L = p.L[i];
        L.dw = it.dw; L.db = it.db; L.lddw = it.lddw; L.M = it.M; L.N = it.N; L.K = it.K;
        L.n_tiles_n = (it.N + 255) / 256;
        L.n_kpairs = (it.K + 255) / 256;
        const uint64_t x_cols = (uint64_t)min((int64_t)((it.K + 7) / 8 * 8), it.ldx);
        const uint64_t dy_cols = (uint64_t)min((int64_t)((it.N + 7) / 8 * 8), it.lddy);
        int rc = make_tmap_bf16_2d(&maps.x[i], it.x, (uint64_t)it.M, x_cols, (uint64_t)it.ldx, 64);
        if (rc) return rc;
        rc = make_tmap_bf16_2d(&maps.dy[i], it.dy, (uint64_t)it.M, dy_cols, (uint64_t)it.lddy, 64);
        if (rc) return rc;
        bytes[i] = (double)it.M * 2.0 * ((double)L.n_tiles_n * min(it.K, 256 * L.n_kpairs) + (double)L.n_kpairs * min(it.N, 256 * L.n_tiles_n));
        total_bytes += bytes[i];
    }
    const int ctas = num_sms();
    int64_t splits[MAXW], kblocks[MAXW];
    double ideal[MAXW];
    int used = 0;
    for (int i = 0; i < n_items; ++i) {
        const WLayer& L = p.L[i];
        const int tiles = L.n_tiles_n * L.n_kpairs;
        kblocks[i] = (L.M + BLOCK_K - 1) / BLOCK_K;
        ideal[i] = ctas * (bytes[i] / total_bytes) / tiles;
        splits[i] = (int64_t)ideal[i];
        if (splits[i] < 1) splits[i] = 1;
        if (splits[i] > kblocks[i]) splits[i] = kblocks[i];
        used += tiles * (int)splits[i];
    }
    for (;;) {
        int best = -1;
        double best_gap = 0.0;
        for (int i = 0; i < n_items; ++i) {
            const int tiles = p.L[i].n_tiles_n * p.L[i].n_kpairs;
            const double gap = ideal[i] - (double)splits[i];
            if (splits[i] < kblocks[i] && used + tiles <= ctas && gap > best_gap) {
                best = i;
                best_gap = gap;
            }
        }
        if (best < 0) break;
        ++splits[best];
        used += p.L[best].n_tiles_n * p.L[best].n_kpairs;
    }
    int first = 0;
    for (int i = 0; i < n_items; ++i) {
        WLayer& L = p.L[i];
        const int tiles = L.n_tiles_n * L.n_kpairs;
        L.m_per_split = ((kblocks[i] + splits[i] - 1) / splits[i]) * BLOCK_K;
        L.splits = (int)((L.M + L.m_per_split - 1) / L.m_per_split);
        L.first_item = first;
        first += tiles * L.splits;
    }
    p.total_items = first;
    static const bool nodrain = getenv("RLPPO_WGRAD_NODRAIN") != nullptr;
    p.dbg_nodrain = nodrain ? 1 : 0;
    static const bool nomma = getenv("RLPPO_WGRAD_NOMMA") != nullptr;
    p.dbg_nomma = nomma ? 1 : 0;
    constexpr uint32_t SMEM = 3 * 8 * 8192 + 256 + 1024;
    static bool configured = false;
    if (!configured) {
        RLPPO_CUDA(cudaFuncSetAttribute(wgrad_multi_kernel, cudaFuncAttributeMaxDynamicSharedMemorySize, (int)SMEM));
        configured = true;
    }
    const int grid = p.total_items < ctas ? p.total_items : ctas;
    RLPPO_CUDA(launch_pdl(wgrad_multi_kernel, dim3(grid), dim3(kThreads), SMEM, static_cast<cudaStream_t>(stream), maps, p));
    return RLPPO_OK;
}
}
```

rlgym_ppo_b200/ops.py:

```python
import ctypes

import numpy as np
import torch

from . import _lib
from ._lib import call, ptr, stream_ptr

BF16 = torch.bfloat16


def _cuda(t, dtype=None):
    assert t.is_cuda, "device tensor expected (no CPU fallback)"
    if dtype is not None:
        assert t.dtype == dtype, f"expected {dtype}, got {t.dtype}"
    return t


def pad8(n):
    return (int(n) + 7) // 8 * 8


_gae_ws = {}


# ... 53 lines not shown
    return out


def welford_update(mean, m2, count, samples, n, std_out=None, mean_out=None):
    dim = mean.numel()
    assert samples.dtype in (torch.float32, torch.float64) and count.dtype == torch.int64
    call("rlppo_welford_update", ptr(mean), ptr(m2), ptr(count), ptr(samples), int(samples.dtype == torch.float64),
         int(n), dim, ptr(std_out), ptr(mean_out), stream_ptr())


def ring_append(ring, phys_first, src, n_rows, ring_bf16=None):
    cap = ring.shape[0]
    width = 1 if ring.dim() == 1 else ring.shape[1]
    ring_ld = 1 if ring.dim() == 1 else ring.stride(0)
    src_ld = 1 if src.dim() == 1 else src.stride(0)
    assert src.dtype in (torch.float32, torch.float64)
    call("rlppo_ring_append", ptr(ring), ring_ld, ptr(ring_bf16), 0 if ring_bf16 is None else ring_bf16.stride(0),
         cap, int(phys_first), ptr(src), int(src.dtype == torch.float64), src_ld, int(n_rows), width, stream_ptr(),
         work=("byte", int(n_rows) * width * (src.element_size() + 4 + (2 if ring_bf16 is not None else 0))))


def ring_append_fields(fields, capacity, phys_first, n_rows, state_dev=None):
    arr = (_lib.AppendField * len(fields))()
    nbytes = 0
    for a, (ring, src, rb) in zip(arr, fields):
        assert src.dtype in (torch.float32, torch.float64) and src.is_cuda
        a.ring, a.ring_ld = ring.data_ptr(), (1 if ring.dim() == 1 else ring.stride(0))
        a.ring_bf16, a.bf16_ld = (None, 0) if rb is None else (rb.data_ptr(), rb.stride(0))
        a.src, a.src_ld = src.data_ptr(), (1 if src.dim() == 1 else src.stride(0))
        a.src_is_f64 = int(src.dtype == torch.float64)
        a.width = 1 if ring.dim() == 1 else ring.shape[1]
        nbytes += int(n_rows) * (a.width * (src.element_size() + 4) + (0 if rb is None else 2 * rb.stride(0)))
    if state_dev is not None:
        assert state_dev.dtype == torch.int64 and state_dev.numel() == 2 and state_dev.is_cuda
        call("rlppo_ring_append_fields_dev", ctypes.cast(arr, ctypes.c_void_p), len(fields), int(capacity),
             ptr(state_dev), int(n_rows), stream_ptr(), work=("byte", nbytes))
        return
    call("rlppo_ring_append_fields", ctypes.cast(arr, ctypes.c_void_p), len(fields), int(capacity), int(phys_first),
         int(n_rows), stream_ptr(), work=("byte", nbytes))


def gather_batch(buf, idx, out_actions=None, out_logp=None, out_values=None, out_adv=None, out_states=None,
                 out_states_bf16=None):
    B = idx.numel()
    sb = getattr(buf, "states_bf16", None)
    call("rlppo_gather_batch", ptr(buf.actions), ptr(buf.log_probs), ptr(buf.values), ptr(buf.advantages),
         ptr(buf.states), buf.states.stride(0) if buf.states is not None and buf.states.dim() == 2 else 1, ptr(sb),
         0 if sb is None else sb.stride(0), int(buf.obs_dim), int(buf.capacity), int(buf.start),
         ptr(getattr(buf, "start_dev", None)), ptr(idx), B,
         ptr(out_actions), ptr(out_logp), ptr(out_values), ptr(out_adv), ptr(out_states), ptr(out_states_bf16),
         stream_ptr(),
         work=("byte", 8 * B + 2 * B * (4 * sum(o is not None for o in (out_actions, out_logp, out_values, out_adv))
                                        + (4 * buf.obs_dim if out_states is not None else 0)
                                        + (2 * sb.stride(0) if out_states_bf16 is not None else 0))))


def rows_to_bf16(src, dst, mean=None, std=None, clip=5.0, dst_f32=None):
    n_rows, width = src.shape
    assert dst.dtype == BF16 and dst.shape[0] >= n_rows
    if mean is None:
        call("rlppo_rows_to_bf16", ptr(src), src.stride(0), n_rows, width, ptr(dst), dst.stride(0), stream_ptr(),
             work=("byte", n_rows * (4 * width + 2 * dst.stride(0))))
    else:
        call("rlppo_rows_standardize_to_bf16", ptr(src), src.stride(0), n_rows, width, ptr(mean), ptr(std),
             float(clip), ptr(dst), dst.stride(0), ptr(dst_f32), 0 if dst_f32 is None else dst_f32.stride(0),
             stream_ptr(), work=("byte", n_rows * (4 * width + 2 * dst.stride(0))))


def weight_to_bf16(w, wq, wt=None):
    out_f, in_f = w.shape
    assert w.is_contiguous() and wq.dtype == BF16
    call("rlppo_weight_to_bf16", ptr(w), out_f, in_f, ptr(wq), wq.stride(0), wq.shape[0], ptr(wt),
         0 if wt is None else wt.stride(0), 0 if wt is None else wt.shape[0], stream_ptr(),
         work=("byte", out_f * in_f * (4 + 2 + (2 if wt is not None else 0))))


def pad64(n):
    return (int(n) + 63) // 64 * 64


def make_split(a_parts, b_parts, order, out_parts, a_pstride, b_pstride, out_pstride=0):
    sp = _lib.Split()
    sp.a_parts, sp.b_parts, sp.order, sp.out_parts = int(a_parts), int(b_parts), int(order), int(out_parts)
    sp.a_pstride, sp.b_pstride, sp.out_pstride = int(a_pstride), int(b_pstride), int(out_pstride)
    return sp


def _n_products(sp):
    return sum(1 for i in range(sp.a_parts) for j in range(sp.b_parts) if i + j < sp.order)


def _sp(sp):
    return None if sp is None else ctypes.byref(sp)


def rows_split(src, dst, parts, pstride, mean=None, std=None, clip=5.0):
    n_rows, width = src.shape
    assert dst.dtype == BF16 and dst.shape[0] >= n_rows and src.dtype == torch.float32
    call("rlppo_rows_split_bf16", ptr(src), src.stride(0), n_rows, width, ptr(mean), ptr(std), float(clip), ptr(dst),
         dst.stride(0), int(parts), int(pstride), stream_ptr(), work=("byte", n_rows * (4 * width + 2 * parts * pstride)))


def weight_split(w, wq, q_parts, q_pstride, wt=None, t_parts=0, t_pstride=0):
    out_f, in_f = w.shape
    assert w.is_contiguous()
    call("rlppo_weight_split_bf16", ptr(w), out_f, in_f, ptr(wq), 0 if wq is None else wq.stride(0), int(q_parts),
         int(q_pstride), 0 if wq is None else wq.shape[0], ptr(wt), 0 if wt is None else wt.stride(0), int(t_parts),
         int(t_pstride), 0 if wt is None else wt.shape[0], stream_ptr(),
         work=("byte", out_f * in_f * (4 + 2 * q_parts + 2 * t_parts)))


def linear_fwd(x, wq, bias, y, N, K, relu, M=None, split=None, bias_n=0):
    M = x.shape[0] if M is None else M
    if split is not None:
        call("rlppo_linear_fwd_split", ptr(x), x.stride(0), ptr(wq), wq.stride(0), ptr(bias), int(bias_n), ptr(y),
             y.stride(0), int(M), int(N), int(K), int(bool(relu)), _sp(split), stream_ptr(),
             work=("flop", 2.0 * M * N * K, "mma_flop", 2.0 * M * N * K * _n_products(split),
                   "byte", 2.0 * (M * K * split.a_parts + N * K * split.b_parts + M * N * split.out_parts)))
        return
    call("rlppo_linear_fwd", ptr(x), x.stride(0), ptr(wq), wq.stride(0), ptr(bias), ptr(y), y.stride(0), int(M),
         int(N), int(K), int(bool(relu)), stream_ptr(),
         work=("flop", 2.0 * M * N * K, "byte", 2.0 * (M * K + N * K + M * N)))


def linear_dgrad(dy, wt, hprev, dx, N, K, M=None, db_below=None, split=None):
    M = dy.shape[0] if M is None else M
    work = ("flop", 2.0 * M * N * K, "byte", 2.0 * (M * N + N * K + M * K * (2 if hprev is not None else 1)))
    if split is not None:
        call("rlppo_linear_dgrad_split", ptr(dy), dy.stride(0), ptr(wt), wt.stride(0), ptr(hprev),
             0 if hprev is None else hprev.stride(0), ptr(dx), dx.stride(0), ptr(db_below), int(M), int(N), int(K),
             _sp(split), stream_ptr(), work=work)
        return
    if db_below is None:
        call("rlppo_linear_dgrad", ptr(dy), dy.stride(0), ptr(wt), wt.stride(0), ptr(hprev),
             0 if hprev is None else hprev.stride(0), ptr(dx), dx.stride(0), int(M), int(N), int(K), stream_ptr(),
             work=work)
    else:
        call("rlppo_linear_dgrad_db", ptr(dy), dy.stride(0), ptr(wt), wt.stride(0), ptr(hprev),
             0 if hprev is None else hprev.stride(0), ptr(dx), dx.stride(0), ptr(db_below), int(M), int(N), int(K),
             stream_ptr(), work=work)


def linear_wgrad(dy, x, dw, db, N, K, M=None, split=None):
    M = dy.shape[0] if M is None else M
    if split is not None:
        call("rlppo_linear_wgrad_split", ptr(dy), dy.stride(0), ptr(x), x.stride(0), ptr(dw), dw.stride(0), ptr(db),
             int(M), int(N), int(K), _sp(split), stream_ptr(),
             work=("flop", 2.0 * M * N * K, "byte", 2.0 * M * (N * split.a_parts + K * split.b_parts) + 4.0 * N * K))
        return
    call("rlppo_linear_wgrad", ptr(dy), dy.stride(0), ptr(x), x.stride(0), ptr(dw), dw.stride(0), ptr(db), int(M),
         int(N), int(K), stream_ptr(), work=("flop", 2.0 * M * N * K, "byte", 2.0 * M * (N + K) + 4.0 * N * K))


def wgrad_multi(items, M):
    for i0 in range(0, len(items), 8):
        part = items[i0:i0 + 8]
        arr = (_lib.WgradItem * len(part))()
        flop = nbytes = 0.0
        for a, item in zip(arr, part):
            dy, x, dw, N, K = item[:5]
            db = item[5] if len(item) > 5 else None
            a.dy, a.lddy, a.x, a.ldx = dy.data_ptr(), dy.stride(0), x.data_ptr(), x.stride(0)
            a.dw, a.lddw, a.M, a.N, a.K = dw.data_ptr(), dw.stride(0), int(M), int(N), int(K)
            a.db = db.data_ptr() if db is not None else None
            flop += 2.0 * M * N * K
            nbytes += 2.0 * M * (dy.stride(0) + x.stride(0)) + 4.0 * N * K
        call("rlppo_wgrad_multi", ctypes.cast(arr, ctypes.c_void_p), len(part), stream_ptr(),
             work=("flop", flop, "byte", nbytes))


def policy_head_sample(h, wq, bias, n_actions, K, M=None, u=None, seed=0, offset=0, deterministic=False,
                       actions_out=None, actions_i64_out=None, logp_out=None, probs_out=None, split=None):
    M = h.shape[0] if M is None else M
    if split is not None:
        call("rlppo_policy_head_sample_split", ptr(h), h.stride(0), ptr(wq), wq.stride(0), ptr(bias), int(M),
             int(n_actions), int(K), ptr(u), int(seed) & (2 ** 64 - 1), int(offset) & (2 ** 64 - 1),
             int(bool(deterministic)), ptr(actions_out), ptr(actions_i64_out), ptr(logp_out), ptr(probs_out),
             _sp(split), stream_ptr(), work=("flop", 2.0 * M * n_actions * K))
        return
    call("rlppo_policy_head_sample", ptr(h), h.stride(0), ptr(wq), wq.stride(0), ptr(bias), int(M), int(n_actions),
         int(K), ptr(u), int(seed) & (2 ** 64 - 1), int(offset) & (2 ** 64 - 1), int(bool(deterministic)),
         ptr(actions_out), ptr(actions_i64_out), ptr(logp_out), ptr(probs_out), stream_ptr(),
         work=("flop", 2.0 * M * n_actions * K))


def policy_head_train(h, wq, bias, n_actions, K, actions, old_logp, adv, inv_batch, clip, ent_coef, dz, metrics,
                      logp_out=None, M=None, split=None):
    M = h.shape[0] if M is None else M
    if split is not None:
        call("rlppo_policy_head_train_split", ptr(h), h.stride(0), ptr(wq), wq.stride(0), ptr(bias), int(M),
             int(n_actions), int(K), ptr(actions), ptr(old_logp), ptr(adv), float(inv_batch), float(clip),
             float(ent_coef), ptr(dz), dz.stride(0), ptr(logp_out), ptr(metrics), _sp(split), stream_ptr(),
             work=("flop", 2.0 * M * n_actions * K))
        return
    call("rlppo_policy_head_train", ptr(h), h.stride(0), ptr(wq), wq.stride(0), ptr(bias), int(M), int(n_actions),
         int(K), ptr(actions), ptr(old_logp), ptr(adv), float(inv_batch), float(clip), float(ent_coef), ptr(dz),
         dz.stride(0), ptr(logp_out), ptr(metrics), stream_ptr(), work=("flop", 2.0 * M * n_actions * K))


def value_head(h, w, bias, K, values_out=None, targets=None, inv_batch=0.0, dh=None, dw=None, db=None, metrics=None,
               M=None, h_parts=1, h_pstride=0, dh_parts=1, dh_pstride=0):
    M = h.shape[0] if M is None else M
    if h_parts > 1 or dh_parts > 1:
        call("rlppo_value_head_split", ptr(h), h.stride(0), ptr(w), ptr(bias), int(M), int(K), ptr(values_out),
             ptr(targets), float(inv_batch), ptr(dh), 0 if dh is None else dh.stride(0), ptr(dw), ptr(db), ptr(metrics),
             int(h_parts), int(h_pstride), int(dh_parts), int(dh_pstride), stream_ptr(),
             work=("byte", M * K * 2 * (h_parts + (dh_parts if targets is not None else 0)) + 8 * M))
        return
    call("rlppo_value_head", ptr(h), h.stride(0), ptr(w), ptr(bias), int(M), int(K), ptr(values_out), ptr(targets),
         float(inv_batch), ptr(dh), 0 if dh is None else dh.stride(0), ptr(dw), ptr(db), ptr(metrics), stream_ptr(),
         work=("byte", M * K * 2 * (2 if targets is not None else 1) + 4 * M * (2 if targets is not None else 1)))


def head_multi_discrete_train(z, z_parts, z_pstride, M, actions, old_logp, adv, inv_batch, clip, ent_coef, dz, dz_parts,
                              dz_pstride, dz_cols, metrics, logp_out=None):
    call("rlppo_head_multi_discrete_train", ptr(z), z.stride(0), int(z_parts), int(z_pstride), int(M), ptr(actions),
         actions.stride(0), ptr(old_logp), ptr(adv), float(inv_batch), float(clip), float(ent_coef), ptr(dz), dz.stride(0),
         int(dz_parts), int(dz_pstride), int(dz_cols), ptr(logp_out), ptr(metrics), stream_ptr(),
         work=("byte", M * (2 * 21 * z_parts + 2 * dz_cols * dz_parts + 4 * 11)))


def head_multi_discrete_sample(z, z_parts, z_pstride, M, actions_out, logp_out, u=None, seed=0, offset=0,
                               deterministic=False):
    call("rlppo_head_multi_discrete_sample", ptr(z), z.stride(0), int(z_parts), int(z_pstride), int(M), ptr(u),
         int(seed) & (2 ** 64 - 1), int(offset) & (2 ** 64 - 1), int(bool(deterministic)), ptr(actions_out),
         actions_out.stride(0), ptr(logp_out), stream_ptr(), work=("byte", M * (2 * 21 * z_parts + 4 * 9)))


def head_continuous_train(z, z_parts, z_pstride, M, n_act, var_min, var_max, actions, old_logp, adv, inv_batch, clip,
                          ent_coef, dz, dz_parts, dz_pstride, dz_cols, metrics, logp_out=None):
    call("rlppo_head_continuous_train", ptr(z), z.stride(0), int(z_parts), int(z_pstride), int(M), int(n_act),
         float(var_min), float(var_max), ptr(actions), actions.stride(0), ptr(old_logp), ptr(adv), float(inv_batch),
         float(clip), float(ent_coef), ptr(dz), dz.stride(0), int(dz_parts), int(dz_pstride), int(dz_cols), ptr(logp_out),
         ptr(metrics), stream_ptr(), work=("byte", M * (4 * n_act * z_parts + 2 * dz_cols * dz_parts + 4 * (n_act + 3))))


def head_continuous_sample(z, z_parts, z_pstride, M, n_act, var_min, var_max, actions_out, logp_out, normals=None, seed=0,
                           offset=0, deterministic=False):
    call("rlppo_head_continuous_sample", ptr(z), z.stride(0), int(z_parts), int(z_pstride), int(M), int(n_act),
         float(var_min), float(var_max), ptr(normals), int(seed) & (2 ** 64 - 1), int(offset) & (2 ** 64 - 1),
         int(bool(deterministic)), ptr(actions_out), actions_out.stride(0), ptr(logp_out), stream_ptr(),
         work=("byte", M * (4 * n_act * z_parts + 4 * (n_act + 1))))


def policy_head_backward(h, wq, bias, n_actions, K, actions, d_logp, d_ent, d_probs, dz, M=None, split=None):
    M = h.shape[0] if M is None else M
    args = (ptr(h), h.stride(0), ptr(wq), wq.stride(0), ptr(bias), int(M), int(n_actions), int(K), ptr(actions),
            ptr(d_logp), ptr(d_ent), ptr(d_probs), ptr(dz), dz.stride(0))
    if split is not None:
        call("rlppo_policy_head_backward_split", *args, _sp(split), stream_ptr(), work=("flop", 2.0 * M * n_actions * K))
        return
    call("rlppo_policy_head_backward", *args, stream_ptr(), work=("flop", 2.0 * M * n_actions * K))


def head_multi_discrete_backward(z, z_parts, z_pstride, M, actions, d_logp, d_ent, dz, dz_parts, dz_pstride, dz_cols):
    call("rlppo_head_multi_discrete_backward", ptr(z), z.stride(0), int(z_parts), int(z_pstride), int(M), ptr(actions),
         0 if actions is None else actions.stride(0), ptr(d_logp), ptr(d_ent), ptr(dz), dz.stride(0), int(dz_parts),
         int(dz_pstride), int(dz_cols), stream_ptr(), work=("byte", M * (2 * 21 * z_parts + 2 * dz_cols * dz_parts + 4 * 9)))


def head_continuous_backward(z, z_parts, z_pstride, M, n_act, var_min, var_max, actions, d_logp, d_ent, d_mean, d_std,
                             dz, dz_parts, dz_pstride, dz_cols):
    call("rlppo_head_continuous_backward", ptr(z), z.stride(0), int(z_parts), int(z_pstride), int(M), int(n_act),
         float(var_min), float(var_max), ptr(actions), 0 if actions is None else actions.stride(0), ptr(d_logp),
         ptr(d_ent), ptr(d_mean), ptr(d_std), ptr(dz), dz.stride(0), int(dz_parts), int(dz_pstride), int(dz_cols),
         stream_ptr(), work=("byte", M * (4 * n_act * z_parts + 2 * dz_cols * dz_parts + 4 * (3 * n_act + 1))))


def value_head_backward(h, w, K, d_values, dh, dw, db, M=None, h_parts=1, h_pstride=0, dh_parts=1, dh_pstride=0):
    M = h.shape[0] if M is None else M
    work = ("byte", M * K * 2 * (h_parts + dh_parts) + 4 * M)
    if h_parts > 1 or dh_parts > 1:
        call("rlppo_value_head_backward_split", ptr(h), h.stride(0), ptr(w), int(M), int(K), ptr(d_values), ptr(dh),
             dh.stride(0), ptr(dw), ptr(db), int(h_parts), int(h_pstride), int(dh_parts), int(dh_pstride), stream_ptr(),
             work=work)
        return
    call("rlppo_value_head_backward", ptr(h), h.stride(0), ptr(w), int(M), int(K), ptr(d_values), ptr(dh), dh.stride(0),
         ptr(dw), ptr(db), stream_ptr(), work=work)


def _net_flops(net, M, n_out, train):
    dims = [net.in_dim] + [net.hidden[i] for i in range(net.n_hidden)]
    f = sum(2.0 * M * dims[i] * dims[i + 1] for i in range(len(dims) - 1)) + 2.0 * M * dims[-1] * n_out
    if train:
        f += sum(2.0 * M * dims[i] * dims[i + 1] for i in range(1, len(dims) - 1)) + 2.0 * M * dims[-1] * n_out
    return f


def _net_bytes(net, M, n_out_pad, train, policy):
    hid = [net.hidden[i] for i in range(net.n_hidden)]
    b = 2.0 * M * ((net.in_dim + 7) // 8 * 8)
    if train:
        b += 2.0 * M * (2 * sum(hid) - (0 if policy else hid[-1])) + (2.0 * M * n_out_pad if policy else 0.0) + 16.0 * M
    else:
        b += 8.0 * M
    return b


def policy_train_fused(net, x, M, n_actions, actions, old_logp, adv, inv_batch, clip, ent_coef, metrics, logp_out=None):
    call("rlppo_policy_train_fused", ctypes.byref(net), ptr(x), int(M), int(n_actions), ptr(actions), ptr(old_logp),
         ptr(adv), float(inv_batch), float(clip), float(ent_coef), ptr(logp_out), ptr(metrics), stream_ptr(),
         work=("flop", _net_flops(net, M, n_actions, True), "byte", _net_bytes(net, M, (n_actions + 7) // 8 * 8, True, True)))


def policy_value_train_fused(pnet, vnet, x, M, n_actions, actions, old_logp, adv, inv_batch, clip, ent_coef, w_head, targets,
                             gw_head, metrics, logp_out=None, values_out=None):
    call("rlppo_policy_value_train_fused", ctypes.byref(pnet), ctypes.byref(vnet), ptr(x), int(M), int(n_actions),
         ptr(actions), ptr(old_logp), ptr(adv), float(inv_batch), float(clip), float(ent_coef), ptr(logp_out), ptr(w_head),
         ptr(targets), ptr(gw_head), ptr(values_out), ptr(metrics), stream_ptr(),
         work=("flop", _net_flops(pnet, M, n_actions, True) + _net_flops(vnet, M, 1, True),
               "byte", _net_bytes(pnet, M, (n_actions + 7) // 8 * 8, True, True) + _net_bytes(vnet, M, 0, True, False)))


def u64_add(counter, inc):
    call("rlppo_u64_add", ptr(counter), int(inc), stream_ptr())


def policy_infer_fused(net, x, M, n_actions, u=None, seed=0, offset=0, deterministic=False, actions_out=None,
                       actions_i64_out=None, logp_out=None, offset_dev=None):
    call("rlppo_policy_infer_fused", ctypes.byref(net), ptr(x), int(M), int(n_actions), ptr(u), int(seed) & (2 ** 64 - 1),
         int(offset) & (2 ** 64 - 1), ptr(offset_dev), int(bool(deterministic)), ptr(actions_out), ptr(actions_i64_out),
         ptr(logp_out),
         stream_ptr(), work=("flop", _net_flops(net, M, n_actions, False), "byte", _net_bytes(net, M, 0, False, True)))


def value_train_fused(net, x, M, w_head, targets, inv_batch, gw_head, metrics, values_out=None):
    call("rlppo_value_train_fused", ctypes.byref(net), ptr(x), int(M), ptr(w_head), ptr(targets), float(inv_batch),
         ptr(gw_head), ptr(values_out), ptr(metrics), stream_ptr(),
         work=("flop", _net_flops(net, M, 1, True), "byte", _net_bytes(net, M, 0, True, False)))


def value_infer_fused(net, x, M, w_head, values_out):
    call("rlppo_value_infer_fused", ctypes.byref(net), ptr(x), int(M), ptr(w_head), ptr(values_out), stream_ptr(),
         work=("flop", _net_flops(net, M, 1, False), "byte", _net_bytes(net, M, 0, False, False)))


def _seg(seg_off):
    return np.ascontiguousarray(seg_off, dtype=np.int64)


def grad_sqnorm(grads, seg_off, sqnorm):
    so = _seg(seg_off)
    call("rlppo_grad_sqnorm", ptr(grads), so.ctypes.data, len(so) - 1, ptr(sqnorm), stream_ptr(),
         work=("byte", 4 * int(so[-1])))


def clip_adam(params, grads, m, v, seg_off, sqnorm, lr, step_count, max_norm=0.5, beta1=0.9, beta2=0.999, eps=1e-8,
              views=None):
    so = _seg(seg_off)
    call("rlppo_clip_adam", ptr(params), ptr(grads), ptr(m), ptr(v), so.ctypes.data, len(so) - 1, ptr(sqnorm), ptr(lr),
         ptr(step_count), float(max_norm), float(beta1), float(beta2), float(eps),
         None if views is None else ctypes.cast(views, ctypes.c_void_p), 0 if views is None else len(views),
         stream_ptr(), work=("byte", 28 * int(so[-1])))


_nca_ws = {}


def norm_clip_adam(params, grads, m, v, seg_off, sqnorm_out, lr, step_count, max_norm=0.5, beta1=0.9, beta2=0.999,
                   eps=1e-8, views=None):
    so = _seg(seg_off)
    ws = _nca_ws.get(params.device)
    if ws is None:
        ws = torch.zeros(int(_lib._lib.rlppo_norm_clip_adam_workspace_bytes()), dtype=torch.uint8, device=params.device)
        _nca_ws[params.device] = ws
    call("rlppo_norm_clip_adam", ptr(params), ptr(grads), ptr(m), ptr(v), so.ctypes.data, len(so) - 1, ptr(sqnorm_out),
         ptr(lr), ptr(step_count), float(max_norm), float(beta1), float(beta2), float(eps),
         None if views is None else ctypes.cast(views, ctypes.c_void_p), 0 if views is None else len(views),
         ptr(ws), ws.numel(), stream_ptr(), work=("byte", 32 * int(so[-1])))


def norm_clip_adam_peers(params, peer_grad_ptrs, peer_flag_ptrs, rank, gsum, m, v, seg_off, sqnorm_out, lr, step_count,
                         max_norm=0.5, beta1=0.9, beta2=0.999, eps=1e-8, views=None):
    so = _seg(seg_off)
    ws = _nca_ws.get(params.device)
    if ws is None:
        ws = torch.zeros(int(_lib._lib.rlppo_norm_clip_adam_workspace_bytes()), dtype=torch.uint8, device=params.device)
        _nca_ws[params.device] = ws
    world = len(peer_grad_ptrs)
    gp = (ctypes.c_void_p * world)(*[int(x) for x in peer_grad_ptrs])
    fp = (ctypes.c_void_p * world)(*[int(x) for x in peer_flag_ptrs])
    call("rlppo_norm_clip_adam_peers", ptr(params), ctypes.cast(gp, ctypes.c_void_p), ctypes.cast(fp, ctypes.c_void_p),
         int(rank), world, ptr(gsum), ptr(m), ptr(v), so.ctypes.data, len(so) - 1, ptr(sqnorm_out), ptr(lr),
         ptr(step_count), float(max_norm), float(beta1), float(beta2), float(eps),
         None if views is None else ctypes.cast(views, ctypes.c_void_p), 0 if views is None else len(views),
         ptr(ws), ws.numel(), stream_ptr(), work=("byte", (32 + 4 * world) * int(so[-1])))


def norm_clip_adam_peers2(params, peer_grad_ptrs, peer_flag_ptrs, peer_red_ptrs, rank, m, v, seg_off, sqnorm_out, lr,
                          step_count, max_norm=0.5, beta1=0.9, beta2=0.999, eps=1e-8, views=None):
    so = _seg(seg_off)
    ws = _nca_ws.get(params.device)
    if ws is None:
        ws = torch.zeros(int(_lib._lib.rlppo_norm_clip_adam_workspace_bytes()), dtype=torch.uint8, device=params.device)
        _nca_ws[params.device] = ws
    world = len(peer_grad_ptrs)
    gp = (ctypes.c_void_p * world)(*[int(x) for x in peer_grad_ptrs])
    fp = (ctypes.c_void_p * world)(*[int(x) for x in peer_flag_ptrs])
    rp = (ctypes.c_void_p * world)(*[int(x) for x in peer_red_ptrs])
    call("rlppo_norm_clip_adam_peers2", ptr(params), ctypes.cast(gp, ctypes.c_void_p), ctypes.cast(fp, ctypes.c_void_p),
         ctypes.cast(rp, ctypes.c_void_p), int(rank), world, ptr(m), ptr(v), so.ctypes.data, len(so) - 1, ptr(sqnorm_out),
         ptr(lr), ptr(step_count), float(max_norm), float(beta1), float(beta2), float(eps),
         None if views is None else ctypes.cast(views, ctypes.c_void_p), 0 if views is None else len(views),
         ptr(ws), ws.numel(), stream_ptr(), work=("byte", 48 * int(so[-1])))


def sqdiff(a, b, seg_off, out):
    so = _seg(seg_off)
    call("rlppo_sqdiff", ptr(a), ptr(b), so.ctypes.data, len(so) - 1, ptr(out), stream_ptr(),
         work=("byte", 8 * int(so[-1])))
```

rlgym_ppo_b200/ppo/ppo_learner.py:

```python
import os
import sys
import time

import numpy as np
import torch

from .. import _lib, ops, parallel
from .continuous_policy import ContinuousPolicy
from .discrete_policy import DiscreteFF
from .fused_adam import FusedAdam
from .multi_discrete_policy import MultiDiscreteFF
from .value_estimator import ValueEstimator


class PPOLearner(object):
    def __init__(
        self,
        obs_space_size,
        act_space_size,
        policy_type,
        policy_layer_sizes,
        critic_layer_sizes,
        continuous_var_range,
        batch_size,
        n_epochs,
        policy_lr,
        critic_lr,
        clip_range,
        ent_coef,
        mini_batch_size,
        device,
        max_chunk_rows=131072,
        process_group=None,
        dp_mode="replicated",
        dp_collective=None,
        precision=None,
    ):
        _lib.require_device()
        if device in (None, "auto", "gpu"):
            device = "cuda:%d" % torch.cuda.current_device()
        if "cuda" not in str(device):
            raise _lib.RlppoError(f"PPOLearner device must be a CUDA device (got {device!r}); there is no CPU path")
        self.device = device
        dev = torch.device(device)

        assert (
            batch_size % mini_batch_size == 0
        ), "MINIBATCH SIZE MUST BE AN INTEGER MULTIPLE OF BATCH SIZE"
        obs_space_size = int(obs_space_size)
        self.policy_type = int(policy_type)
        if self.policy_type == 2:
            self.policy = ContinuousPolicy(obs_space_size, int(act_space_size) * 2, policy_layer_sizes, device,
                                           var_min=continuous_var_range[0], var_max=continuous_var_range[1],
                                           precision=precision)
        elif self.policy_type == 1:
            self.policy = MultiDiscreteFF(obs_space_size, policy_layer_sizes, device, precision=precision)
        else:
            self.policy = DiscreteFF(obs_space_size, act_space_size, policy_layer_sizes, device, precision)
        self._act_w = int(getattr(self.policy, "act_width", 1))
        self.value_net = ValueEstimator(obs_space_size, critic_layer_sizes, device, precision)
        self.precision = self.policy._stack.precision
        self.mini_batch_size = mini_batch_size

        ps, vs = self.policy._stack, self.value_net._stack
        n_p, n_v = ps.n_params, vs.n_params
        self._pg = process_group
        self.world_size, self.rank = parallel.world(process_group)
        n_x = 8 if self.world_size > 1 else 0
        self._n_net = n_p + n_v
        self._seg = np.asarray([0, n_p, n_p + n_v] + ([n_p + n_v + n_x] if n_x else []), dtype=np.int64)
        n_seg = len(self._seg) - 1
        self._params = torch.zeros(n_p + n_v + n_x, dtype=torch.float32, device=dev)
        self.dp_collective = "none"
        self._grads = None
        if self.world_size > 1:
            self.dp_collective = parallel.choose_collective(self.world_size, n_p + n_v, dp_collective,
                                                            os.environ.get("RLPPO_DP_COLLECTIVE"))
            if self.dp_collective in ("p2p", "p2p2"):
                import torch.distributed as dist
                err = None
                try:
                    self._setup_peers(dev, n_p + n_v + n_x)
                except Exception as e:
                    err = e
                ok = torch.tensor([0 if err is not None else 1], dtype=torch.int32, device=dev)
                dist.all_reduce(ok, op=dist.ReduceOp.MIN, group=self._pg)
                if int(ok.item()) == 0:
                    if dp_collective in ("p2p", "p2p2"):
                        raise _lib.RlppoError(f"dp_collective='p2p' requested but peer mappings are unavailable: {err}")
                    print(f"[rlgym_ppo_b200] rank {self.rank}: symmetric-memory peer mappings unavailable ({err}); "
                          "gradients go through NCCL all_reduce", file=sys.stderr, flush=True)
                    self.dp_collective = "nccl"
                    self._grads = None
        if self._grads is None:
            self._grads = torch.zeros_like(self._params)
        self._m = torch.zeros_like(self._params)
        self._v = torch.zeros_like(self._params)
        self._before = torch.zeros_like(self._params)
        ps.bind(self._params[:n_p], self._grads[:n_p])
        vs.bind(self._params[n_p:n_p + n_v], self._grads[n_p:n_p + n_v])
        self._steps = torch.zeros(n_seg, dtype=torch.int64, device=dev)
        self._lr_dev = torch.zeros(n_seg, dtype=torch.float32, device=dev)
        self._lr_host = None
        self._sqnorm = torch.zeros(n_seg, dtype=torch.float32, device=dev)
        self._tail = torch.zeros(12, dtype=torch.float32, device=dev)
        self._tail_host = torch.zeros(12, dtype=torch.float32).pin_memory()

        self.policy_optimizer = FusedAdam(ps, policy_lr, self._m[:n_p], self._v[:n_p], self._steps[0:1])
        self.value_optimizer = FusedAdam(vs, critic_lr, self._m[n_p:n_p + n_v], self._v[n_p:n_p + n_v], self._steps[1:2])

        policy_params_count, critic_params_count = n_p, n_v
        total_parameters = policy_params_count + critic_params_count
        print("Trainable Parameters:")
        print(f"{'Component':<10} {'Count':<10}")
        print("-" * 20)
        print(f"{'Policy':<10} {policy_params_count:<10}")
        print(f"{'Critic':<10} {critic_params_count:<10}")
        print("-" * 20)
        print(f"{'Total':<10} {total_parameters:<10}")
        print(f"Current Policy Learning Rate: {policy_lr}")
        print(f"Current Critic Learning Rate: {critic_lr}")

        self.n_epochs = n_epochs
        self.batch_size = batch_size
        self.clip_range = clip_range
        self.ent_coef = ent_coef
        self.cumulative_model_updates = 0
        self.max_chunk_rows = int(os.environ.get("RLPPO_MAX_CHUNK_ROWS", max_chunk_rows))

        assert dp_mode in ("replicated", "sharded")
        self.dp_mode = dp_mode
        if dp_mode == "replicated":
            assert batch_size % self.world_size == 0, "batch_size must be a multiple of the number of ranks"
        self._mb = None
        self.launches = 0
        self._views_sig = None
        self._sync_operand_views()
        self.use_cuda_graph = True
        self._nb_final = None
        self._graphs = {}
        self.max_graphs = 16
        self._graph_warm = set()
        self._idx_cur = None
        self._perm_dev = None
        self.graph_collectives = os.environ.get("RLPPO_GRAPH_COLLECTIVES", "0") == "1"
        self.two_streams = os.environ.get("RLPPO_TWO_STREAMS", "1") == "1"
        self.one_launch = os.environ.get("RLPPO_ONE_LAUNCH", "1") == "1"
        self._side_stream = None
        self.gather_prefetch = os.environ.get("RLPPO_GATHER_PREFETCH", "0") == "1"
        self._gather_stream = None
        self._mb_alt = None

    def _setup_peers(self, dev, n):
        import torch.distributed as dist
        import torch.distributed._symmetric_memory as symm_mem
        group = self._pg if self._pg is not None else dist.group.WORLD
        grads = symm_mem.empty(n, dtype=torch.float32, device=dev)
        grads.zero_()
        gh = symm_mem.rendezvous(grads, group)
        flags = symm_mem.empty(int(_lib._lib.rlppo_peer_flag_bytes()) // 4, dtype=torch.int32, device=dev)
        flags.zero_()
        fh = symm_mem.rendezvous(flags, group)
        torch.cuda.synchronize(dev)
        dist.barrier(group)
        self._grads = grads
        self._peer_grad_ptrs = [int(x) for x in gh.buffer_ptrs]
        self._peer_flag_ptrs = [int(x) for x in fh.buffer_ptrs]
        self._symm = (grads, gh, flags, fh)
        slots = symm_mem.empty(4, dtype=torch.float32, device=dev)
        slots.fill_(1.0)
        sh = symm_mem.rendezvous(slots, group)
        self._std_slots_local = slots
        self._std_slots_rank0 = sh.get_buffer(0, (4,), torch.float32) if self.rank != 0 else slots
        self._symm += (slots, sh)
        torch.cuda.synchronize(dev)
        dist.barrier(group)
        if self.dp_collective == "p2p2":
            gsum = symm_mem.empty(n, dtype=torch.float32, device=dev)
            gsum.zero_()
            rh = symm_mem.rendezvous(gsum, group)
            torch.cuda.synchronize(dev)
            dist.barrier(group)
            self._gsum = gsum
            self._peer_red_ptrs = [int(x) for x in rh.buffer_ptrs]
            self._symm += (gsum, rh)
        else:
            self._gsum = torch.zeros(n, dtype=torch.float32, device=dev)

    def _minibatch_buffers(self, rows, slot=0):
        cur = self._mb if slot == 0 else self._mb_alt
        if cur is None or cur["rows"] < rows:
            dev = self._params.device
            f = lambda: torch.empty(rows, dtype=torch.float32, device=dev)
            self._mb_gen = getattr(self, "_mb_gen", 0) + 1
            ps = self.policy._stack
            cur = {"rows": rows, "actions": f(), "old_logp": f(), "targets": f(), "adv": f()}
            if self._act_w > 1:
                cur["actions"] = torch.empty((rows, self._act_w), dtype=torch.float32, device=dev)
            if ps.exact:
                cur["x32"] = torch.empty((rows, ps.in_dim), dtype=torch.float32, device=dev)
                cur["x"] = torch.zeros((rows, 3 * ps.in_ps), dtype=torch.bfloat16, device=dev)
            else:
                cur["x"] = torch.zeros((rows, ps.in_pad), dtype=torch.bfloat16, device=dev)
            if slot == 0:
                self._mb = cur
            else:
                self._mb_alt = cur
        return cur

    def _gather(self, exp, idx, M, mb):
        if self.policy._stack.exact:
            exp.gather(idx, out_actions=mb["actions"], out_logp=mb["old_logp"], out_values=mb["targets"],
                       out_adv=mb["adv"], out_states=mb["x32"])
            self.policy._stack.stage_rows(mb["x32"][:M], mb["x"])
            self.launches += 1
        else:
            exp.gather(idx, out_actions=mb["actions"], out_logp=mb["old_logp"], out_values=mb["targets"],
                       out_adv=mb["adv"], out_states_bf16=mb["x"])

    def _sync_lr(self):
        lr = (float(self.policy_optimizer.param_groups[0]["lr"]), float(self.value_optimizer.param_groups[0]["lr"]))
        if lr != self._lr_host:
            pad = (0.0,) * (self._lr_dev.numel() - 2)
            self._lr_dev.copy_(torch.tensor(lr + pad, dtype=torch.float32))
            self._lr_host = lr

    def _sync_operand_views(self):
        ps, vs = self.policy._stack, self.value_net._stack
        sig = (ps.fused_ok and self.policy_type == 0, vs.fused_ok)
        if sig == self._views_sig:
            return
        for st, fused in zip((ps, vs), sig):
            was = st.need_wt
            st.need_wt = not fused
            if st.need_wt and not was and st.params is not None:
                st.refresh_operands(force=True)
        views = ps.bf16_views(0) + vs.bf16_views(ps.n_params)
        self._views = (_lib.Bf16View * len(views))(*views)
        self._views_sig = sig

    def _train_chunk(self, exp, idx, M, mb=None, after_fused=None):
        self._sync_operand_views()
        if mb is None:
            mb = self._minibatch_buffers(M)
            self._gather(exp, idx, M, mb)
        x = mb["x"]
        inv_b = 1.0 / float(parallel.samples_per_step(self.batch_size, self.world_size, self.dp_mode))
        metrics = self._step_metrics()
        n = 1
        both_fused = self.policy_type == 0 and self.policy._stack.fused_ok and self.value_net._stack.fused_ok
        if both_fused and self.one_launch:
            ps, vs = self.policy._stack, self.value_net._stack
            wp, wv = ps.workspace(M), vs.workspace(M)
            ops.policy_value_train_fused(ps.fused_net(x.stride(0), wp, policy_head=True), vs.fused_net(x.stride(0), wv), x, M,
                                         self.policy.n_actions, mb["actions"], mb["old_logp"], mb["adv"], inv_b,
                                         float(self.clip_range), float(self.ent_coef), vs.w[-1], mb["targets"], vs.gw[-1],
                                         metrics)
            if after_fused is not None:
                after_fused()
            ops.wgrad_multi(ps.fused_wgrad_items(x, wp, head_dy=wp["dz"]) + vs.fused_wgrad_items(x, wv), M)
            self.launches += 3
            return
        if after_fused is not None:
            after_fused()
        if both_fused and self.two_streams and _lib._TIMING is None:
            main = torch.cuda.current_stream()
            if self._side_stream is None:
                self._side_stream = torch.cuda.Stream(device=self._params.device)
            side = self._side_stream
            fork, join = torch.cuda.Event(), torch.cuda.Event()
            fork.record(main)
            side.wait_event(fork)
            with torch.cuda.stream(side):
                st = self.value_net._stack
                ws = st.workspace(M)
                ops.value_train_fused(st.fused_net(x.stride(0), ws), x, M, st.w[-1], mb["targets"], inv_b, st.gw[-1], metrics)
                ops.wgrad_multi(st.fused_wgrad_items(x, ws), M)
                join.record(side)
            st = self.policy._stack
            ws = st.workspace(M)
            ops.policy_train_fused(st.fused_net(x.stride(0), ws, policy_head=True), x, M, self.policy.n_actions,
                                   mb["actions"], mb["old_logp"], mb["adv"], inv_b, float(self.clip_range),
                                   float(self.ent_coef), metrics)
            ops.wgrad_multi(st.fused_wgrad_items(x, ws, head_dy=ws["dz"]), M)
            main.wait_event(join)
            self.launches += 5
            return
        wg_items = []
        for net, is_policy in ((self.policy, True), (self.value_net, False)):
            st = net._stack
            ws = st.workspace(M)
            if st.fused_ok and (not is_policy or self.policy_type == 0):
                if is_policy:
                    fnet = st.fused_net(x.stride(0), ws, policy_head=True)
                    ops.policy_train_fused(fnet, x, M, net.n_actions, mb["actions"], mb["old_logp"], mb["adv"], inv_b,
                                           float(self.clip_range), float(self.ent_coef), metrics)
                    wg_items += st.fused_wgrad_items(x, ws, head_dy=ws["dz"])
                else:
                    fnet = st.fused_net(x.stride(0), ws)
                    ops.value_train_fused(fnet, x, M, st.w[-1], mb["targets"], inv_b, st.gw[-1], metrics)
                    wg_items += st.fused_wgrad_items(x, ws)
                n += 1
                continue
            h = st.forward_hidden(x, M, ws)
            if is_policy and self.policy_type != 0:
                dh = net.train_head(h, M, ws, mb["actions"], mb["old_logp"], mb["adv"], inv_b, float(self.clip_range),
                                    float(self.ent_coef), metrics)
                n += 5 + (1 if st.exact else 0)
            elif is_policy:
                dh = st.policy_head_train(h, M, ws, net.n_actions, mb["actions"], mb["old_logp"], mb["adv"], inv_b,
                                          float(self.clip_range), float(self.ent_coef), metrics)
                n += 4 + (1 if st.exact else 0)
            else:
                dh = st.value_head_train(h, M, ws, mb["targets"], inv_b, metrics)
                n += 1
            st.backward_hidden(x, M, ws, dh)
            L = len(st.hidden)
            n += L + 2 * L + (L - 1)
        if wg_items:
            ops.wgrad_multi(wg_items, M)
            n += (len(wg_items) + 7) // 8
        self.launches += n

    def _step_metrics(self):
        if self.world_size > 1:
            return self._grads[self._n_net:self._n_net + 8]
        return self._tail[0:8]

    def _collect_step_metrics(self, summed):
        if self.world_size > 1:
            self._tail[0:8].add_(summed[self._n_net:self._n_net + 8])

    def _optimizer_step(self):
        if self.dp_collective == "p2p2":
            ops.norm_clip_adam_peers2(self._params, self._peer_grad_ptrs, self._peer_flag_ptrs, self._peer_red_ptrs,
                                      self.rank, self._m, self._v, self._seg, self._sqnorm, self._lr_dev, self._steps,
                                      max_norm=0.5, views=self._views if len(self._views) else None)
            self._collect_step_metrics(self._gsum)
            self._operands_after_step()
            self.launches += 1
            return
        if self.dp_collective == "p2p":
            ops.norm_clip_adam_peers(self._params, self._peer_grad_ptrs, self._peer_flag_ptrs, self.rank, self._gsum,
                                     self._m, self._v, self._seg, self._sqnorm, self._lr_dev, self._steps, max_norm=0.5,
                                     views=self._views if len(self._views) else None)
            self._collect_step_metrics(self._gsum)
            self._operands_after_step()
            self.launches += 1
            return
        parallel.allreduce_sum_(self._grads, self._pg)
        self._apply_step()

    def _operands_after_step(self):
        for st in (self.policy._stack, self.value_net._stack):
            if st.exact:
                st.refresh_operands(force=True)
                self.launches += len(st.linears)
            else:
                st.mark_operands_fresh()

    def _apply_step(self):
        ops.norm_clip_adam(self._params, self._grads, self._m, self._v, self._seg, self._sqnorm, self._lr_dev,
                           self._steps, max_norm=0.5, views=self._views if len(self._views) else None)
        self._collect_step_metrics(self._grads)
        self._operands_after_step()
        self.launches += 1

    def _backward_body(self, exp, idx, local, chunk):
        self._grads.zero_()
        for c0 in range(0, local, chunk):
            rows = min(chunk, local - c0)
            self._train_chunk(exp, idx[c0:c0 + rows], rows)

    def _batch_body(self, exp, idx, local, chunk):
        self._backward_body(exp, idx, local, chunk)
        self._optimizer_step()

    def _captured(self, key, fn):
        entry = self._graphs.get(key)
        if entry is None:
            if key not in self._graph_warm:
                self._graph_warm.add(key)
                return False
            calls0, launches0 = _lib.CALLS, self.launches
            graph = torch.cuda.CUDAGraph()
            with torch.cuda.graph(graph):
                fn()
            entry = (graph, _lib.CALLS - calls0, self.launches - launches0)
            self.launches = launches0
            _lib.CALLS = calls0
            while len(self._graphs) >= self.max_graphs:
                old = next(iter(self._graphs))
                del self._graphs[old]
                self._graph_warm.discard(old)
            self._graphs[key] = entry
        graph, n_calls, n_launch = entry
        graph.replay()
        _lib.CALLS += n_calls
        self.launches += n_launch
        return True

    def _batch_step(self, exp, idx, local, chunk):
        if not self.use_cuda_graph or _lib._TIMING is not None:
            self._batch_body(exp, idx, local, chunk)
            return
        if self._idx_cur is None or self._idx_cur.numel() < local:
            self._idx_cur = torch.empty(local, dtype=torch.int64, device=self._params.device)
        cur = self._idx_cur[:local]
        cur.copy_(idx)
        key = self._graph_key(exp, local, chunk) + (self._idx_cur.data_ptr(),)
        if self.world_size == 1 or self.dp_collective in ("p2p", "p2p2"):
            if not self._captured(("step",) + key, lambda: self._batch_body(exp, cur, local, chunk)):
                self._batch_body(exp, cur, local, chunk)
        else:
            if not self._captured(("bwd",) + key, lambda: self._backward_body(exp, cur, local, chunk)):
                self._backward_body(exp, cur, local, chunk)
            parallel.allreduce_sum_(self._grads, self._pg)
            if not self._captured(("opt",) + key, self._apply_step):
                self._apply_step()
        self.policy._stack.mark_operands_fresh()
        self.value_net._stack.mark_operands_fresh()

    def _graph_key(self, exp, local, chunk):
        return (exp.uid, local, chunk, float(self.clip_range), float(self.ent_coef), self.batch_size, self.world_size,
                self.dp_mode, self.dp_collective, self.precision, self.policy_type, self.policy._stack.fused_ok, self.value_net._stack.fused_ok, getattr(self, "_mb_gen", 0),
                self.gather_prefetch,
                getattr(self.policy._stack, "ws_gen", 0), getattr(self.value_net._stack, "ws_gen", 0))

    def _learn_body(self, exp, n_batches, local, chunk, tail=True):
        B, R = self.batch_size, self.world_size
        self._before.copy_(self._params)
        self._tail.zero_()
        steps = [(epoch, parallel.rank_rows(k, B, self.rank, R, self.dp_mode)[0])
                 for epoch in range(self.n_epochs) for k in range(n_batches)]
        idx_of = lambda i: self._perm_dev[steps[i][0], steps[i][1]:steps[i][1] + local]
        if self.gather_prefetch and chunk == local and len(steps) > 1:
            main = torch.cuda.current_stream()
            if self._gather_stream is None:
                self._gather_stream = torch.cuda.Stream(device=self._params.device)
            side = self._gather_stream
            sets = (self._minibatch_buffers(local, 0), self._minibatch_buffers(local, 1))
            self._gather(exp, idx_of(0), local, sets[0])
            for i in range(len(steps)):
                joins = []

                def prefetch(i=i, joins=joins):
                    fork, join = torch.cuda.Event(), torch.cuda.Event()
                    fork.record(main)
                    side.wait_event(fork)
                    with torch.cuda.stream(side):
                        self._gather(exp, idx_of(i + 1), local, sets[(i + 1) & 1])
                        join.record(side)
                    joins.append(join)

                self._grads.zero_()
                self._train_chunk(exp, None, local, mb=sets[i & 1], after_fused=prefetch if i + 1 < len(steps) else None)
                self._optimizer_step()
                for join in joins:
                    main.wait_event(join)
        else:
            for i in range(len(steps)):
                self._batch_body(exp, idx_of(i), local, chunk)
        ops.sqdiff(self._before, self._params, self._seg, self._tail[8:8 + len(self._seg) - 1])
        if tail:
            self._tail_host.copy_(self._tail, non_blocking=True)

    def learn(self, exp):
        self.launches = 0
        self.policy._stack.refresh_operands()
        self.value_net._stack.refresh_operands()
        self._sync_lr()

        t1 = time.time()
        B, R, E = self.batch_size, self.world_size, self.n_epochs
        local = parallel.rank_rows(0, B, self.rank, R, self.dp_mode)[1]
        chunk = min(local, self.max_chunk_rows)
        total = len(exp)
        n_batches = total // B
        if R > 1 and self.dp_mode == "sharded":
            full = int(total >= getattr(exp, "max_size", total + 1))
            if not (self._nb_final is not None and full):
                nb = torch.tensor([n_batches, full], dtype=torch.int64, device=self._params.device)
                torch.distributed.all_reduce(nb, op=torch.distributed.ReduceOp.MIN)
                n_batches = int(nb[0].item())
                self._nb_final = n_batches if int(nb[1].item()) == 1 else None
            else:
                n_batches = self._nb_final
        fresh = self._perm_dev is None or self._perm_dev.shape[0] != E or self._perm_dev.shape[1] < total
        if fresh:
            self._perm_dev = torch.empty((E, max(total, 1)), dtype=torch.int64, device=self._params.device)
        for epoch in range(E):
            exp.next_permutation_into(self._perm_dev[epoch, :total], fresh_alloc=fresh)
        n_iterations = E * n_batches

        p2p = R > 1 and self.dp_collective in ("p2p", "p2p2")
        whole = (self.use_cuda_graph and _lib._TIMING is None and n_batches > 0
                 and (R == 1 or p2p or self.graph_collectives))
        if whole:
            tail = True
            key = ("learn", total, E, n_batches, tail, self._perm_dev.data_ptr()) + self._graph_key(exp, local, chunk)
            if not self._captured(key, lambda: self._learn_body(exp, n_batches, local, chunk, tail)):
                self._learn_body(exp, n_batches, local, chunk, tail)
            self.policy._stack.mark_operands_fresh()
            self.value_net._stack.mark_operands_fresh()
        else:
            self._before.copy_(self._params)
            self._tail.zero_()
            for epoch in range(E):
                for k in range(n_batches):
                    base = parallel.rank_rows(k, B, self.rank, R, self.dp_mode)[0]
                    self._batch_step(exp, self._perm_dev[epoch, base:base + local], local, chunk)
            ops.sqdiff(self._before, self._params, self._seg, self._tail[8:8 + len(self._seg) - 1])
            self._tail_host.copy_(self._tail, non_blocking=True)
        torch.cuda.current_stream().synchronize()
        t = self._tail_host.double().numpy()
        avg = parallel.report_from_sums(t[0:8])

        if n_iterations == 0:
            n_iterations = 1
        self.cumulative_model_updates += n_iterations

        report = {
            "PPO Batch Consumption Time": (time.time() - t1) / n_iterations,
            "Cumulative Model Updates": self.cumulative_model_updates,
            "Policy Entropy": avg["Policy Entropy"],
            "Mean KL Divergence": avg["Mean KL Divergence"],
            "Value Function Loss": avg["Value Function Loss"],
            "SB3 Clip Fraction": avg["SB3 Clip Fraction"],
            "Policy Update Magnitude": float(np.sqrt(t[8])),
            "Value Function Update Magnitude": float(np.sqrt(t[9])),
        }
        return report

    def save_to(self, folder_path):
        os.makedirs(folder_path, exist_ok=True)
        cpu = lambda sd: {k: v.detach().cpu().clone() for k, v in sd.items()}
        torch.save(cpu(self.policy.state_dict()), os.path.join(folder_path, "PPO_POLICY.pt"))
        torch.save(cpu(self.value_net.state_dict()), os.path.join(folder_path, "PPO_VALUE_NET.pt"))
        torch.save(_optim_to_cpu(self.policy_optimizer.state_dict()),
                   os.path.join(folder_path, "PPO_POLICY_OPTIMIZER.pt"))
        torch.save(_optim_to_cpu(self.value_optimizer.state_dict()),
                   os.path.join(folder_path, "PPO_VALUE_NET_OPTIMIZER.pt"))

    def load_from(self, folder_path):
        assert os.path.exists(folder_path), "PPO LEARNER CANNOT FIND FOLDER {}".format(folder_path)
        dev = self._params.device
        self.policy.load_state_dict(torch.load(os.path.join(folder_path, "PPO_POLICY.pt"), map_location=dev))
        self.value_net.load_state_dict(torch.load(os.path.join(folder_path, "PPO_VALUE_NET.pt"), map_location=dev))
        self.policy_optimizer.load_state_dict(
            torch.load(os.path.join(folder_path, "PPO_POLICY_OPTIMIZER.pt"), map_location=dev))
        self.value_optimizer.load_state_dict(
            torch.load(os.path.join(folder_path, "PPO_VALUE_NET_OPTIMIZER.pt"), map_location=dev))
        self._lr_host = None


def _optim_to_cpu(sd):
    state = {i: {k: (v.detach().cpu() if isinstance(v, torch.Tensor) else v) for k, v in s.items()}
             for i, s in sd["state"].items()}
    return {"state": state, "param_groups": sd["param_groups"]}
```

Measured before the change: 55.88 million.

## Start weight-gradient kernel early using per-tile readiness flags from fused train kernel

The fused policy/value train kernel now publishes a release flag per row tile once its activations and gradients are stored. The weight-gradient multi kernel skips the PDL wait at entry and instead polls these flags before loading each 128-row block, so it overlaps with the tail of the fused kernel. Work items get a ticket-based order sorted by when their rows become ready, and late-running CTAs get shorter splits. This adds spin-wait polling and extra zeroing of the readiness words, and it risks deadlock if the consumer CTAs are not co-resident with the producer.

```diff
diff --git a/include/rlppo.h b/include/rlppo.h
--- a/include/rlppo.h
+++ b/include/rlppo.h
@@ -217,6 +217,15 @@
                                    const float* old_logp, const float* adv, float inv_batch, float clip, float ent_coef,
                                    float* logp_out, const float* w_head, const float* targets, float* gw_head,
                                    float* values_out, float* metrics, void* stream);
+int64_t rlppo_ready_words_per_net(int64_t M);
+int rlppo_policy_value_train_fused_ready(const rlppo_fused_net* policy_net, const rlppo_fused_net* value_net,
+                                         const uint16_t* x, int64_t M, int n_actions, const float* actions,
+                                         const float* old_logp, const float* adv, float inv_batch, float clip,
+                                         float ent_coef, float* logp_out, const float* w_head, const float* targets,
+                                         float* gw_head, float* values_out, float* metrics, uint32_t* ready,
+                                         int64_t ready_words, uint32_t ready_val, void* stream);
+int rlppo_wgrad_multi_ready(const rlppo_wgrad_item* h_items, int n_items, const int32_t* h_item_net,
+                            const uint32_t* ready, uint32_t ready_val, uint32_t* ticket, void* stream);
 int rlppo_value_infer_fused(const rlppo_fused_net* net, const uint16_t* x, int64_t M, const float* w_head,
                             float* values_out, void* stream);
 
diff --git a/rlgym_ppo_b200/_lib.py b/rlgym_ppo_b200/_lib.py
--- a/rlgym_ppo_b200/_lib.py
+++ b/rlgym_ppo_b200/_lib.py
@@ -72,6 +72,10 @@
     "rlppo_u64_add": ([_P, _U64, _P], _I),
     "rlppo_value_train_fused": ([_P, _P, _L, _P, _P, _F, _P, _P, _P, _P], _I),
     "rlppo_policy_value_train_fused": ([_P, _P, _P, _L, _I, _P, _P, _P, _F, _F, _F, _P, _P, _P, _P, _P, _P, _P], _I),
+    "rlppo_policy_value_train_fused_ready": ([_P, _P, _P, _L, _I, _P, _P, _P, _F, _F, _F, _P, _P, _P, _P, _P, _P, _P, _L,
+                                              ctypes.c_uint32, _P], _I),
+    "rlppo_ready_words_per_net": ([_L], _L),
+    "rlppo_wgrad_multi_ready": ([_P, _I, _P, _P, ctypes.c_uint32, _P, _P], _I),
     "rlppo_value_infer_fused": ([_P, _P, _L, _P, _P, _P], _I),
     "rlppo_grad_sqnorm": ([_P, _P, _I, _P, _P], _I),
     "rlppo_clip_adam": ([_P, _P, _P, _P, _P, _I, _P, _P, _P, _D, _D, _D, _D, _P, _I, _P], _I),
diff --git a/rlgym_ppo_b200/csrc/common.cuh b/rlgym_ppo_b200/csrc/common.cuh
--- a/rlgym_ppo_b200/csrc/common.cuh
+++ b/rlgym_ppo_b200/csrc/common.cuh
@@ -42,6 +42,20 @@
 __device__ __forceinline__ void pdl_wait() { asm volatile("griddepcontrol.wait;" ::: "memory"); }
 __device__ __forceinline__ void pdl_trigger() { asm volatile("griddepcontrol.launch_dependents;" ::: "memory"); }
 int pdl_mode();
+
+__device__ __forceinline__ void ready_publish(uint32_t* w, uint32_t v) {
+    asm volatile("fence.proxy.async.global;" ::: "memory");
+    asm volatile("st.release.gpu.global.u32 [%0], %1;" ::"l"(w), "r"(v) : "memory");
+}
+__device__ __forceinline__ void ready_wait(const uint32_t* w, uint32_t v) {
+    for (;;) {
+        uint32_t got;
+        asm volatile("ld.acquire.gpu.global.u32 %0, [%1];" : "=r"(got) : "l"(w) : "memory");
+        if (got >= v) break;
+        __nanosleep(64);
+    }
+    asm volatile("fence.proxy.async.global;" ::: "memory");
+}
 
 template <class... KArgs, class... Args>
 cudaError_t launch_pdl_cluster(void (*kernel)(KArgs...), dim3 grid, dim3 block, size_t smem, cudaStream_t s, int cluster_x,
diff --git a/rlgym_ppo_b200/csrc/mlp_fused.cu b/rlgym_ppo_b200/csrc/mlp_fused.cu
--- a/rlgym_ppo_b200/csrc/mlp_fused.cu
+++ b/rlgym_ppo_b200/csrc/mlp_fused.cu
@@ -94,6 +94,9 @@
     NetP net[MAXNET];
     unsigned int* sched;
     uint32_t* mask_scratch;
+    uint32_t* ready;
+    uint32_t ready_val;
+    int ready_wpn;
     int dbg_nostore;
     int dbg;
     unsigned long long* trace;
@@ -107,6 +110,15 @@
 }
 __device__ __forceinline__ void bulk_commit() { asm volatile("cp.async.bulk.commit_group;" ::: "memory"); }
 __device__ __forceinline__ void bulk_wait_read_all() { asm volatile("cp.async.bulk.wait_group.read 0;" ::: "memory"); }
+__device__ __forceinline__ void bulk_wait_all_but(int n) {
+    switch (n) {
+        case 0: asm volatile("cp.async.bulk.wait_group 0;" ::: "memory"); break;
+        case 1: asm volatile("cp.async.bulk.wait_group 1;" ::: "memory"); break;
+        case 2: asm volatile("cp.async.bulk.wait_group 2;" ::: "memory"); break;
+        case 3: asm volatile("cp.async.bulk.wait_group 3;" ::: "memory"); break;
+        default: asm volatile("cp.async.bulk.wait_group 4;" ::: "memory"); break;
+    }
+}
 __device__ __forceinline__ void epi_bar_sync() { asm volatile("bar.sync 1, 256;" ::: "memory"); }
 
 __device__ __forceinline__ uint4 philox4x32_10(uint4 c, uint2 k) {
@@ -868,6 +880,7 @@
         if (lane == 0) {
             DuoWalk w;
             uint32_t kpar = 0;
+            int pub = -1;
             DUO_WALK_BEGIN(w, false)
                 uint8_t* act = smem + s * ACT_BYTES;
                 for (int kb = 0; kb < d.rel_kb; ++kb) {
@@ -882,8 +895,17 @@
                 if (d.out != NO_STORE && d.rel_kb > 0) bulk_wait_read_all();
                 mbar_arrive(&st_done[s]);
                 if (last_ph) mbar_arrive(&x_free[s]);
+                if (p.ready != nullptr) {
+                    if (pub >= 0) {
+                        bulk_wait_all_but(d.out != NO_STORE ? d.rel_kb : 0);
+                        ready_publish(p.ready + pub, p.ready_val);
+                        pub = -1;
+                    }
+                    if (last_ph) pub = ni * p.ready_wpn + tile_s;
+                }
             DUO_WALK_END
             asm volatile("cp.async.bulk.wait_group 0;" ::: "memory");
+            if (pub >= 0) ready_publish(p.ready + pub, p.ready_val);
         }
     } else {
         EpiCtx e;
@@ -1387,6 +1409,33 @@
     return launch_nets<true>(nets, pol, 2, x, M, p, static_cast<cudaStream_t>(stream));
 }
 
+int rlppo_policy_value_train_fused_ready(const rlppo_fused_net* policy_net, const rlppo_fused_net* value_net,
+                                         const uint16_t* x, int64_t M, int n_actions, const float* actions,
+                                         const float* old_logp, const float* adv, float inv_batch, float clip,
+                                         float ent_coef, float* logp_out, const float* w_head, const float* targets,
+                                         float* gw_head, float* values_out, float* metrics, uint32_t* ready,
+                                         int64_t ready_words, uint32_t ready_val, void* stream) {
+    RLPPO_REQUIRE_DEVICE();
+    RLPPO_CHECK_ARG(policy_net && value_net && x && actions && old_logp && adv && w_head && targets && gw_head && ready,
+                    "null pointer");
+    RLPPO_CHECK_ARG(n_actions >= 1 && n_actions <= 128, "fused path: n_actions must be in [1,128]");
+    RLPPO_CHECK_ARG(M >= 1 && ready_val >= 1, "bad row count / ready value");
+    const int64_t wpn = rlppo_ready_words_per_net(M);
+    RLPPO_CHECK_ARG(ready_words >= 2 * wpn, "readiness words: %lld needed", (long long)(2 * wpn));
+    const rlppo_fused_net* nets[2] = {policy_net, value_net};
+    RLPPO_CHECK_ARG(duo_ok(nets, 2), "readiness words need the two-tile cluster form (fused_duo_kernel)");
+    Params p{};
+    fill_policy_train(p.net[0], n_actions, actions, old_logp, adv, inv_batch, clip, ent_coef, logp_out, metrics);
+    fill_value_train(p.net[1], w_head, targets, inv_batch, gw_head, values_out, metrics);
+    p.ready = ready;
+    p.ready_val = ready_val;
+    p.ready_wpn = (int)wpn;
+    const bool pol[2] = {true, false};
+    return launch_nets<true>(nets, pol, 2, x, M, p, static_cast<cudaStream_t>(stream));
+}
+
+int64_t rlppo_ready_words_per_net(int64_t M) { return 2 * (((M + TILE_M - 1) / TILE_M + 1) / 2); }
+
 int rlppo_u64_add(uint64_t* d_counter, uint64_t inc, void* stream) {
     RLPPO_REQUIRE_DEVICE();
     RLPPO_CHECK_ARG(d_counter != nullptr, "null pointer");
diff --git a/rlgym_ppo_b200/csrc/mlp_tcgen05.cu b/rlgym_ppo_b200/csrc/mlp_tcgen05.cu
--- a/rlgym_ppo_b200/csrc/mlp_tcgen05.cu
+++ b/rlgym_ppo_b200/csrc/mlp_tcgen05.cu
@@ -1,3 +1,4 @@
+#include <algorithm>
 #include <mutex>
 #include <unordered_map>
 #include <math.h>
@@ -813,12 +814,19 @@
 struct WLayer {
     float* dw;
     float* db;
+    const uint32_t* ready;
     int64_t lddw, M, m_per_split;
-    int N, K, n_tiles_n, n_kpairs, splits, first_item;
+    int64_t m_short;
+    int N, K, n_tiles_n, n_kpairs, splits, n_long, first_item;
 };
+constexpr int WMAX_ORDER = 256;
 struct WMultiParams {
     WLayer L[MAXW];
     int n_layers, total_items;
+    int early;
+    uint32_t ready_val;
+    uint32_t* ticket;
+    uint16_t order[WMAX_ORDER];
     int dbg_nodrain;
     int dbg_nomma;
 };
@@ -836,6 +844,7 @@
     uint64_t* tfull = empty + NST;
     uint64_t* tempty = tfull + 1;
     uint32_t* tmem_slot = reinterpret_cast<uint32_t*>(tempty + 1);
+    uint32_t* s_first = tmem_slot + 1;
 
     const int warp = threadIdx.x >> 5, lane = threadIdx.x & 31;
     if (threadIdx.x == 0) {
@@ -846,13 +855,15 @@
         mbar_init(tfull, 1);
         mbar_init(tempty, 4);
         fence_barrier_init();
+        *s_first = p.ticket != nullptr ? atomicAdd(p.ticket, 1u) : blockIdx.x;
     }
     if (warp == 1) tmem_alloc(tmem_slot, 512);
     tc_fence_before();
     __syncthreads();
     tc_fence_after();
     const uint32_t tmem_base = *tmem_slot;
-    pdl_wait();
+    const int first = (int)*s_first;
+    if (!p.early) pdl_wait();
     pdl_trigger();
 
     struct Item {
@@ -860,6 +871,7 @@
         int64_t m0;
     };
     auto decode = [&](int w) {
+        if (p.ticket != nullptr) w = p.order[w];
         Item it;
         int l = 0;
         while (l + 1 < p.n_layers && w >= p.L[l + 1].first_item) ++l;
@@ -870,8 +882,10 @@
         it.layer = l;
         it.n0 = nt * 256;
         it.k0 = kp * 256;
-        it.m0 = (int64_t)split * L.m_per_split;
-        const int64_t m1 = min(L.M, it.m0 + L.m_per_split);
+        const bool longer = split < L.n_long;
+        it.m0 = longer ? (int64_t)split * L.m_per_split
+                       : (int64_t)L.n_long * L.m_per_split + (int64_t)(split - L.n_long) * L.m_short;
+        const int64_t m1 = min(L.M, it.m0 + (longer ? L.m_per_split : L.m_short));
         it.nkb = m1 > it.m0 ? (int)((m1 - it.m0 + BLOCK_K - 1) / BLOCK_K) : 0;
         it.n_x = (min(256, L.K - it.k0) + 63) / 64;
         it.n_y = (min(256, L.N - it.n0) + 63) / 64;
@@ -882,13 +896,15 @@
     if (warp == 0) {
         if (lane == 0) {
             uint32_t stage = 0, phase = 0;
-            for (int w = blockIdx.x; w < p.total_items; w += gridDim.x) {
+            for (int w = first; w < p.total_items; w += gridDim.x) {
                 const Item it = decode(w);
+                const uint32_t* ready = p.L[it.layer].ready;
                 for (int kb = 0; kb < it.nkb; ++kb) {
+                    const int mrow = (int)(it.m0 + (int64_t)kb * BLOCK_K);
+                    if (ready != nullptr && (kb == 0 || (mrow & 127) == 0)) ready_wait(ready + (mrow >> 7), p.ready_val);
                     mbar_wait(&empty[stage], phase ^ 1);
                     mbar_expect_tx(&full[stage], (uint32_t)(it.n_x + it.n_y) * CHUNK);
                     uint8_t* sx = smem + stage * STAGE;
-                    const int mrow = (int)(it.m0 + (int64_t)kb * BLOCK_K);
                     for (int c = 0; c < it.n_x; ++c)
                         tma_load_2d_hint(&maps.x[it.layer], &full[stage], sx + c * CHUNK, it.k0 + c * 64, mrow, L2_EVICT_FIRST);
                     for (int c = 0; c < it.n_y; ++c)
@@ -903,7 +919,7 @@
     } else if (warp == 1) {
         if (lane == 0) {
             uint32_t stage = 0, phase = 0, n_done = 0;
-            for (int w = blockIdx.x; w < p.total_items; w += gridDim.x) {
+            for (int w = first; w < p.total_items; w += gridDim.x) {
                 const Item it = decode(w);
                 if (it.nkb == 0) continue;
                 mbar_wait(tempty, (n_done & 1) ^ 1);
@@ -936,7 +952,7 @@
     } else {
         const int ew = warp & 3;
         uint32_t n_done = 0, stage = 0, phase = 0;
-        for (int w = blockIdx.x; w < p.total_items; w += gridDim.x) {
+        for (int w = first; w < p.total_items; w += gridDim.x) {
             const Item it = decode(w);
             if (it.nkb == 0) continue;
             const WLayer& L = p.L[it.layer];
@@ -994,6 +1010,7 @@
             ++n_done;
         }
     }
+    if (p.early) pdl_wait();
     tc_fence_before();
     __syncthreads();
     if (warp == 1) {
@@ -1303,12 +1320,25 @@
     return rlppo_linear_wgrad_split(dy, lddy, x, ldx, dw, lddw, db, M, N, K, nullptr, stream);
 }
 
-int rlppo_wgrad_multi(const rlppo_wgrad_item* h_items, int n_items, void* stream) {
+static int wgrad_multi_launch(const rlppo_wgrad_item* h_items, int n_items, const int32_t* h_item_net,
+                              const uint32_t* ready, uint32_t ready_val, uint32_t* ticket, void* stream) {
     RLPPO_REQUIRE_DEVICE();
     RLPPO_CHECK_ARG(h_items && n_items >= 1 && n_items <= MAXW, "1..%d weight-gradient items per launch", MAXW);
     WMaps maps;
     WMultiParams p{};
     p.n_layers = n_items;
+    const bool early = ready != nullptr;
+    if (early) {
+        RLPPO_CHECK_ARG(h_item_net && ticket && ready_val >= 1, "early start: item nets, ticket and ready value needed");
+        const int64_t wpn = rlppo_ready_words_per_net(h_items[0].M);
+        for (int i = 0; i < n_items; ++i) {
+            RLPPO_CHECK_ARG(h_items[i].M == h_items[0].M && (h_item_net[i] == 0 || h_item_net[i] == 1),
+                            "early start: item %d: one M, nets 0 / 1", i);
+            p.L[i].ready = ready + h_item_net[i] * wpn;
+        }
+        p.early = 1;
+        p.ready_val = ready_val;
+    }
     double bytes[MAXW], total_bytes = 0.0;
     for (int i = 0; i < n_items; ++i) {
         const rlppo_wgrad_item& it = h_items[i];
@@ -1362,10 +1392,65 @@
         const int tiles = L.n_tiles_n * L.n_kpairs;
         L.m_per_split = ((kblocks[i] + splits[i] - 1) / splits[i]) * BLOCK_K;
         L.splits = (int)((L.M + L.m_per_split - 1) / L.m_per_split);
+        L.n_long = L.splits;
+        L.m_short = L.m_per_split;
         L.first_item = first;
         first += tiles * L.splits;
     }
     p.total_items = first;
+    if (early && p.total_items <= ctas && p.total_items <= WMAX_ORDER) {
+        const int64_t units = ((h_items[0].M + 127) / 128 + 1) / 2;
+        const int64_t n_clusters = std::min<int64_t>(units, ctas / 2);
+        constexpr double kLateShare = 0.8;
+        const int64_t rem = (2 * units) % n_clusters;
+        const int late = rem != 0 ? std::max(0, ctas - (int)(2 * (n_clusters - rem))) : 0;
+        int q_of[MAXW] = {}, n_short = 0;
+        for (int i = 0; i < n_items && late > 0; ++i) {
+            q_of[i] = std::min(p.L[i].splits - 1, (int)((int64_t)p.L[i].splits * late / p.total_items));
+            n_short += q_of[i] * p.L[i].n_tiles_n * p.L[i].n_kpairs;
+        }
+        while (late > 0 && n_short < late) {
+            int best = -1;
+            double best_frac = -1.0;
+            for (int i = 0; i < n_items; ++i) {
+                const double frac = (double)p.L[i].splits * late / p.total_items - q_of[i];
+                if (q_of[i] < p.L[i].splits - 1 && frac > best_frac) {
+                    best = i;
+                    best_frac = frac;
+                }
+            }
+            if (best < 0) break;
+            ++q_of[best];
+            n_short += p.L[best].n_tiles_n * p.L[best].n_kpairs;
+        }
+        for (int i = 0; i < n_items && late > 0; ++i) {
+            WLayer& L = p.L[i];
+            const int q = q_of[i];
+            if (q <= 0) continue;
+            const double denom = (double)(L.splits - q) + kLateShare * q;
+            const int64_t a = (int64_t)std::ceil((double)kblocks[i] / denom);
+            const int64_t b = std::max<int64_t>(1, (int64_t)std::ceil(kLateShare * (double)a));
+            L.n_long = L.splits - q;
+            L.m_per_split = a * BLOCK_K;
+            L.m_short = b * BLOCK_K;
+        }
+        int64_t key[WMAX_ORDER];
+        for (int w = 0; w < p.total_items; ++w) {
+            int l = 0;
+            while (l + 1 < p.n_layers && w >= p.L[l + 1].first_item) ++l;
+            const WLayer& L = p.L[l];
+            const int split = (w - L.first_item) % L.splits;
+            const int64_t end = split < L.n_long ? (int64_t)(split + 1) * L.m_per_split
+                                                 : (int64_t)L.n_long * L.m_per_split + (int64_t)(split + 1 - L.n_long) * L.m_short;
+            const int64_t last_row = std::max<int64_t>(0, std::min(L.M, end) - 1);
+            key[w] = (split >= L.n_long ? (int64_t)1 << 40 : 0) + (h_item_net[l] * units + last_row / 256) / n_clusters;
+            p.order[w] = (uint16_t)w;
+        }
+        std::stable_sort(p.order, p.order + p.total_items, [&](uint16_t a, uint16_t b) { return key[a] < key[b]; });
+        p.ticket = ticket;
+    } else if (early) {
+        p.ticket = nullptr;
+    }
     static const bool nodrain = getenv("RLPPO_WGRAD_NODRAIN") != nullptr;
     p.dbg_nodrain = nodrain ? 1 : 0;
     static const bool nomma = getenv("RLPPO_WGRAD_NOMMA") != nullptr;
@@ -1380,4 +1465,14 @@
     RLPPO_CUDA(launch_pdl(wgrad_multi_kernel, dim3(grid), dim3(kThreads), SMEM, static_cast<cudaStream_t>(stream), maps, p));
     return RLPPO_OK;
 }
-}
+
+int rlppo_wgrad_multi(const rlppo_wgrad_item* h_items, int n_items, void* stream) {
+    return wgrad_multi_launch(h_items, n_items, nullptr, nullptr, 0u, nullptr, stream);
+}
+
+int rlppo_wgrad_multi_ready(const rlppo_wgrad_item* h_items, int n_items, const int32_t* h_item_net,
+                            const uint32_t* ready, uint32_t ready_val, uint32_t* ticket, void* stream) {
+    RLPPO_CHECK_ARG(ready != nullptr, "null pointer");
+    return wgrad_multi_launch(h_items, n_items, h_item_net, ready, ready_val, ticket, stream);
+}
+}
diff --git a/rlgym_ppo_b200/ops.py b/rlgym_ppo_b200/ops.py
--- a/rlgym_ppo_b200/ops.py
+++ b/rlgym_ppo_b200/ops.py
@@ -229,7 +229,9 @@
          int(N), int(K), stream_ptr(), work=("flop", 2.0 * M * N * K, "byte", 2.0 * M * (N + K) + 4.0 * N * K))
 
 
-def wgrad_multi(items, M):
+def wgrad_multi(items, M, ready=None):
+    if ready is not None and len(items) > 8:
+        raise ValueError("wgrad_multi: early start takes at most 8 items")
     for i0 in range(0, len(items), 8):
         part = items[i0:i0 + 8]
         arr = (_lib.WgradItem * len(part))()
@@ -242,8 +244,18 @@
             a.db = db.data_ptr() if db is not None else None
             flop += 2.0 * M * N * K
             nbytes += 2.0 * M * (dy.stride(0) + x.stride(0)) + 4.0 * N * K
+        if ready is not None:
+            words, value, nets = ready
+            nets_arr = (ctypes.c_int32 * len(part))(*[int(n) for n in nets])
+            call("rlppo_wgrad_multi_ready", ctypes.cast(arr, ctypes.c_void_p), len(part), nets_arr, ptr(words), int(value),
+                 ptr(words[-1:]), stream_ptr(), work=("flop", flop, "byte", nbytes))
+            continue
         call("rlppo_wgrad_multi", ctypes.cast(arr, ctypes.c_void_p), len(part), stream_ptr(),
              work=("flop", flop, "byte", nbytes))
+
+
+def ready_words_per_net(M):
+    return int(_lib._lib.rlppo_ready_words_per_net(int(M)))
 
 
 def policy_head_sample(h, wq, bias, n_actions, K, M=None, u=None, seed=0, offset=0, deterministic=False,
@@ -381,7 +393,16 @@
 
 
 def policy_value_train_fused(pnet, vnet, x, M, n_actions, actions, old_logp, adv, inv_batch, clip, ent_coef, w_head, targets,
-                             gw_head, metrics, logp_out=None, values_out=None):
+                             gw_head, metrics, logp_out=None, values_out=None, ready=None):
+    if ready is not None:
+        words, value = ready
+        call("rlppo_policy_value_train_fused_ready", ctypes.byref(pnet), ctypes.byref(vnet), ptr(x), int(M), int(n_actions),
+             ptr(actions), ptr(old_logp), ptr(adv), float(inv_batch), float(clip), float(ent_coef), ptr(logp_out),
+             ptr(w_head), ptr(targets), ptr(gw_head), ptr(values_out), ptr(metrics), ptr(words), int(words.numel()) - 1,
+             int(value), stream_ptr(),
+             work=("flop", _net_flops(pnet, M, n_actions, True) + _net_flops(vnet, M, 1, True),
+                   "byte", _net_bytes(pnet, M, (n_actions + 7) // 8 * 8, True, True) + _net_bytes(vnet, M, 0, True, False)))
+        return
     call("rlppo_policy_value_train_fused", ctypes.byref(pnet), ctypes.byref(vnet), ptr(x), int(M), int(n_actions),
          ptr(actions), ptr(old_logp), ptr(adv), float(inv_batch), float(clip), float(ent_coef), ptr(logp_out), ptr(w_head),
          ptr(targets), ptr(gw_head), ptr(values_out), ptr(metrics), stream_ptr(),
diff --git a/rlgym_ppo_b200/ppo/ppo_learner.py b/rlgym_ppo_b200/ppo/ppo_learner.py
--- a/rlgym_ppo_b200/ppo/ppo_learner.py
+++ b/rlgym_ppo_b200/ppo/ppo_learner.py
@@ -73,6 +73,8 @@
         self._params = torch.zeros(n_p + n_v + n_x, dtype=torch.float32, device=dev)
         self.dp_collective = "none"
         self._grads = None
+        self.wgrad_early = os.environ.get("RLPPO_WGRAD_EARLY", "1") == "1"
+        self._n_ready = 2 * ops.ready_words_per_net(int(os.environ.get("RLPPO_MAX_CHUNK_ROWS", max_chunk_rows))) + 1
         if self.world_size > 1:
             self.dp_collective = parallel.choose_collective(self.world_size, n_p + n_v, dp_collective,
                                                             os.environ.get("RLPPO_DP_COLLECTIVE"))
@@ -93,7 +95,9 @@
                     self.dp_collective = "nccl"
                     self._grads = None
         if self._grads is None:
-            self._grads = torch.zeros_like(self._params)
+            self._gstore = torch.zeros(self._params.numel() + self._n_ready, dtype=torch.float32, device=dev)
+            self._grads = self._gstore[:self._params.numel()]
+        self._ready = self._gstore[self._params.numel():].view(torch.int32)
         self._m = torch.zeros_like(self._params)
         self._v = torch.zeros_like(self._params)
         self._before = torch.zeros_like(self._params)
@@ -155,7 +159,7 @@
         import torch.distributed as dist
         import torch.distributed._symmetric_memory as symm_mem
         group = self._pg if self._pg is not None else dist.group.WORLD
-        grads = symm_mem.empty(n, dtype=torch.float32, device=dev)
+        grads = symm_mem.empty(n + self._n_ready, dtype=torch.float32, device=dev)
         grads.zero_()
         gh = symm_mem.rendezvous(grads, group)
         flags = symm_mem.empty(int(_lib._lib.rlppo_peer_flag_bytes()) // 4, dtype=torch.int32, device=dev)
@@ -163,7 +167,8 @@
         fh = symm_mem.rendezvous(flags, group)
         torch.cuda.synchronize(dev)
         dist.barrier(group)
-        self._grads = grads
+        self._gstore = grads
+        self._grads = grads[:n]
         self._peer_grad_ptrs = [int(x) for x in gh.buffer_ptrs]
         self._peer_flag_ptrs = [int(x) for x in fh.buffer_ptrs]
         self._symm = (grads, gh, flags, fh)
@@ -239,7 +244,7 @@
         self._views = (_lib.Bf16View * len(views))(*views)
         self._views_sig = sig
 
-    def _train_chunk(self, exp, idx, M, mb=None, after_fused=None):
+    def _train_chunk(self, exp, idx, M, mb=None, after_fused=None, ready_cleared=False):
         self._sync_operand_views()
         if mb is None:
             mb = self._minibatch_buffers(M)
@@ -252,13 +257,17 @@
         if both_fused and self.one_launch:
             ps, vs = self.policy._stack, self.value_net._stack
             wp, wv = ps.workspace(M), vs.workspace(M)
+            items_p, items_v = ps.fused_wgrad_items(x, wp, head_dy=wp["dz"]), vs.fused_wgrad_items(x, wv)
+            early = (self.wgrad_early and ready_cleared and _lib._TIMING is None and len(items_p) + len(items_v) <= 8
+                     and 2 * ops.ready_words_per_net(M) + 1 <= self._n_ready and _duo_form(ps) and _duo_form(vs))
             ops.policy_value_train_fused(ps.fused_net(x.stride(0), wp, policy_head=True), vs.fused_net(x.stride(0), wv), x, M,
                                          self.policy.n_actions, mb["actions"], mb["old_logp"], mb["adv"], inv_b,
                                          float(self.clip_range), float(self.ent_coef), vs.w[-1], mb["targets"], vs.gw[-1],
-                                         metrics)
+                                         metrics, ready=(self._ready, 1) if early else None)
             if after_fused is not None:
                 after_fused()
-            ops.wgrad_multi(ps.fused_wgrad_items(x, wp, head_dy=wp["dz"]) + vs.fused_wgrad_items(x, wv), M)
+            nets = [0] * len(items_p) + [1] * len(items_v)
+            ops.wgrad_multi(items_p + items_v, M, ready=(self._ready, 1, nets) if early else None)
             self.launches += 3
             return
         if after_fused is not None:
@@ -367,10 +376,10 @@
         self.launches += 1
 
     def _backward_body(self, exp, idx, local, chunk):
-        self._grads.zero_()
+        self._gstore.zero_()
         for c0 in range(0, local, chunk):
             rows = min(chunk, local - c0)
-            self._train_chunk(exp, idx[c0:c0 + rows], rows)
+            self._train_chunk(exp, idx[c0:c0 + rows], rows, ready_cleared=rows == local)
 
     def _batch_body(self, exp, idx, local, chunk):
         self._backward_body(exp, idx, local, chunk)
@@ -453,8 +462,9 @@
                         join.record(side)
                     joins.append(join)
 
-                self._grads.zero_()
-                self._train_chunk(exp, None, local, mb=sets[i & 1], after_fused=prefetch if i + 1 < len(steps) else None)
+                self._gstore.zero_()
+                self._train_chunk(exp, None, local, mb=sets[i & 1], after_fused=prefetch if i + 1 < len(steps) else None,
+                                  ready_cleared=True)
                 self._optimizer_step()
                 for join in joins:
                     main.wait_event(join)
@@ -554,6 +564,11 @@
         self._lr_host = None
 
 
+def _duo_form(st):
+    return (os.environ.get("RLPPO_FUSED_DUO", "1")[:1] != "0" and len(st.hidden) <= 3
+            and all(h in (128, 256) for h in st.hidden))
+
+
 def _optim_to_cpu(sd):
     state = {i: {k: (v.detach().cpu() if isinstance(v, torch.Tensor) else v) for k, v in s.items()}
              for i, s in sd["state"].items()}
```

New measurement: 55.88 million, median of 6. No clear change (+0.0%).
